# amplab/snap

Measured on AMD Instinct MI355X. Metric: aligned reads/sec (whole node), 150 bp single-end vs synthetic 3100 Mb genome (GRCh38 unavailable), seed=20, maxDist=8, higher is better.
Workload: dtype u8 bases / int32 DP / f64 match probability

## Files before the change

snap_amd/csrc/align_single.h:

```cpp
#pragma once
#include "dev_common.h"
#include "probe.h"
#include "lv.h"
#include "ag_win.h"
#include "se_help.h"
#include "adjust.h"
#include <stddef.h>
#include "../../include/snapgpu.h"

#define BUCKET 48
#define SENT_MIN 0xFC00u
#define WIN_PAD 128

struct AlignCfg {
    uint32_t max_hits, max_k, num_seeds, min_weight, extra_depth, use_ag;
    int32_t  match_reward, sub_penalty, gap_open, gap_extend, five_bonus, three_bonus;
    uint32_t alt_aware, emit_alt;
    int32_t  max_gap_alt;
    double   seed_coverage;
    uint32_t num_weight_lists;
    uint32_t RL;
    uint32_t kmax;
    uint32_t pool_size;
    uint32_t ht_size;
    uint64_t scratch_stride;
    uint32_t lds_per_wave;
    uint32_t ag_numvec_max;
    uint32_t ag_buffers;
    uint32_t ag_lds;
    uint32_t se_items_cap; uint64_t se_off;
    uint32_t stop_on_first_hit, explore_popular_seeds;
};

struct __attribute__((aligned(16))) Elem {
    uint64_t used;
    uint64_t scored;
    int64_t  base;
    int64_t  best_loc;
    double   match_prob;
    uint32_t weight;
    uint32_t lps;
    uint32_t best_score;
    int32_t  ag_score;
    int32_t  clip_before, clip_after, seed_offset;
    uint16_t wnext, wprev, hnext;
    uint8_t  dir;
    uint8_t  flags;
    uint32_t pad0;
    uint16_t cand_seed_offset[BUCKET];
};
static_assert(sizeof(Elem) == 176, "Elem layout");

struct ScoreSet {
    int32_t  best_score;
    int64_t  best_loc, best_orig_loc;
    int32_t  dir;
    int32_t  used_ag, clip_before, clip_after, ag_score, seed_offset;
    double   best_match_prob;
    double   p_all, p_best;
    __device__ __forceinline__ void init() {
        best_score = SNAPGPU_UnusedScoreValue; best_loc = SNAPGPU_InvalidGenomeLocation32;
        best_orig_loc = SNAPGPU_InvalidGenomeLocation32; dir = 0; used_ag = 0; clip_before = 0;
        clip_after = 0; ag_score = -1; seed_offset = 0; best_match_prob = 0.0; p_all = 0.0; p_best = 0.0;
    }
};

struct WaveCounters {
    uint64_t lookups, slots, hits, overflow_lists, lv, ag, lv_ref_bytes;
    uint64_t cyc_lookup, cyc_hits, cyc_lv, cyc_ag, cyc_total;
};
static __device__ __forceinline__ uint64_t wave_clock() { return __builtin_amdgcn_s_memtime(); }

static __device__ __forceinline__ int compute_mapq(const DevTables *tab, double p_all, double p_best, int popular_skipped) {
    if (p_all < p_best) p_all = p_best;
    double correctness = p_best / p_all;
    int base_mapq;
    if (correctness >= 1) {
        base_mapq = 70;
    } else {
        double x = 1 - correctness;
        int lo = 0, hi = 70;
        while (lo < hi) {
            int mid = (lo + hi + 1) >> 1;
            if (x <= tab->mapq_threshold[mid]) lo = mid; else hi = mid - 1;
        }
        base_mapq = lo;
    }
    int pen = popular_skipped - 10; if (pen < 0) pen = 0;
    base_mapq -= pen / 2;
    if (base_mapq < 0) base_mapq = 0;
    return (int)first_u32((uint32_t)base_mapq);
}

struct WaveShared {
    ScoreSet all, non_alt;
    ScoreSet ag_all, ag_non_alt;
    snapgpu_single_result primary, first_alt;
    WaveCounters cnt;
};

struct SecCfg {
    int32_t  om;
    int32_t  mpc;
    int64_t  omax;
    uint32_t cap;
    uint32_t adjust;
    uint64_t adj_off;
};

struct AlignerDirState { uint32_t dirkey; };
struct AlignerNoDirState {};
template <bool REGDIR> struct AlignerDirBase { using type = AlignerNoDirState; };
template <> struct AlignerDirBase<true> { using type = AlignerDirState; };

template <int AGC, bool SEC = false, bool EXACT = false, bool TIMED = false, bool PLANES = false, bool REGDIR = false>
struct Aligner : AlignerDirBase<REGDIR>::type {
    const DevIndex ix;
    GP<const DevTables> tab;
    const AlignCfg cfg;
    LP<uint8_t>  rd[2];
    LP<uint8_t>  ql[2];
    LP<uint8_t>  gw;
    LP<uint32_t> seed_used;
    LP<uint16_t> wl_next, wl_prev;
    LP<uint16_t> lv_tri;
    LP<int16_t>  ag_rows;
    LP<unsigned long long> rp;
    LP<unsigned long long> tp;
    int tp_org;
    LP<unsigned long long> lvp;
    uint32_t rd_plain;
    GP<uint16_t> heads;
    GP<Elem>     pool;
    GP<uint8_t>  ag_scratch;
    uint8_t  *ag_persist0, *ag_persist1;
    uint32_t ag_hw0, ag_hw1;
    uint32_t ag_epoch, ag_tag;
    struct LaneId { __device__ __forceinline__ operator int() const { return lane_id(); } };
    LaneId lane;
    int read_len;
    uint32_t n_used;
    uint32_t highest_used_weight_list;
    uint32_t wrap_count;
    uint32_t lps_unseen[2];
    uint32_t cur_round_lps[2];
    uint32_t n_seeds_applied[2];
    uint32_t popular_seeds_skipped;
    uint32_t ag_stale;
    uint32_t ag_replay;
    uint32_t ag_obj_used0, ag_obj_used1;
    uint32_t max_k;
    uint32_t ag_calls_unit;
    SEHelpSlot *se_slots; uint32_t se_n_slots; SESpec *se_spec; uint32_t se_spec_cap;
    uint32_t *se_ctl;
    uint32_t se_eager;
    uint32_t *se_items, *se_first;
    unsigned long long *se_diag;
    int se_slot; uint32_t se_n, se_tried, cur_read; SESpec *se_mine;
    GP<snapgpu_single_result> agc;
    uint32_t agc_cap, n_agc, agc_overflow;
    SecCfg sec_cfg;
    snapgpu_single_result *sec;
    uint32_t *sec_key, *sec_ord;
    uint32_t n_sec, n_sec_raw, sec_overflow;
    uint8_t *adj_scratch;
    LDS_AS WaveShared *ws_;
    __device__ __forceinline__ ScoreSet &all() const { return *(ScoreSet *)&ws_->all; }
    __device__ __forceinline__ ScoreSet &non_alt() const { return *(ScoreSet *)&ws_->non_alt; }
    __device__ __forceinline__ snapgpu_single_result &primary() const { return *(snapgpu_single_result *)&ws_->primary; }
    __device__ __forceinline__ snapgpu_single_result &first_alt() const { return *(snapgpu_single_result *)&ws_->first_alt; }
    __device__ __forceinline__ WaveCounters &cnt() const { return *(WaveCounters *)&ws_->cnt; }

    __device__ __forceinline__ Aligner(const DevIndex &ix_, const DevTables *tab_, const AlignCfg &cfg_, WaveShared *ws)
        : ix(ix_), tab(tab_), cfg(cfg_), tp_org(0), rd_plain(0), ag_hw0(0), ag_hw1(0), ag_epoch(0), ag_tag(0), read_len(0), popular_seeds_skipped(0),
          ag_stale(0), ag_replay(0), ag_obj_used0(0), ag_obj_used1(0), max_k(cfg_.max_k), ag_calls_unit(0),
          agc(nullptr), agc_cap(0), n_agc(0), agc_overflow(0), n_sec(0), n_sec_raw(0), sec_overflow(0),
          ws_((LDS_AS WaveShared *)ws) {}

    static __device__ __forceinline__ uint64_t clk() { if constexpr (TIMED) return wave_clock(); else return 0; }

    __device__ __forceinline__ void note_ag_call(int obj, uint32_t stale_steps) {
        ag_stale += stale_steps;
        const uint32_t used = obj == 0 ? ag_obj_used0 : ag_obj_used1;
        if (EXACT || used) ag_replay += stale_steps;
        if (obj == 0) ag_obj_used0 = 1; else ag_obj_used1 = 1;
    }

    __device__ __forceinline__ void new_read_images() {
        if constexpr (EXACT) {
            if (++ag_epoch == 16u) {
                if (ag_hw0) wave_zero16(ag_persist0, ((size_t)ag_hw0 + 15) & ~(size_t)15);
                if (ag_hw1) wave_zero16(ag_persist1, ((size_t)ag_hw1 + 15) & ~(size_t)15);
                ag_hw0 = ag_hw1 = 0; ag_epoch = 1u;
                WAVE_SYNC();
            }
            ag_tag = bt_tag_bits(ag_epoch);
        }
    }

    __device__ __forceinline__ void note_ag_extent(int obj, bool banded, int plen, int w, int tlen) {
        if constexpr (EXACT) {
            int nv, sl, ns;
            ag_dims(banded, plen, w > 126 ? 126 : (w < 0 ? 0 : w), &nv, &sl, &ns);
            uint32_t ext = (w >= 0 && tlen > 0) ? (uint32_t)tlen * (uint32_t)(ns * sl) : 0u;
            const uint32_t image = (uint32_t)ag_scratch_bytes(cfg.RL);
            if (ext > image) ext = image;
            if (obj == 0) ag_hw0 = ext > ag_hw0 ? ext : ag_hw0; else ag_hw1 = ext > ag_hw1 ? ext : ag_hw1;
        }
    }

    __device__ __forceinline__ bool is_alt(int64_t loc) const { return (uint64_t)loc >= ix.first_alt_location && loc >= 0; }

    __device__ __forceinline__ int score_limit(bool for_alt) const {
        int64_t inner;
        if (for_alt) {
            int64_t g = cfg.max_gap_alt < non_alt().best_score ? cfg.max_gap_alt : non_alt().best_score;
            int64_t b = (int64_t)non_alt().best_score - g;
            inner = all().best_score < b ? all().best_score : b;
        } else {
            int64_t a = (int64_t)all().best_score + cfg.max_gap_alt;
            inner = a < non_alt().best_score ? a : non_alt().best_score;
        }
        int64_t m = (int64_t)max_k < inner ? (int64_t)max_k : inner;
        int64_t v = (int64_t)cfg.extra_depth + m;
        return (int)(v < 126 ? v : 126);
    }

    __device__ __forceinline__ bool substring_ok(int64_t loc, int64_t len) const {
        if (!substring_in_range(loc, len)) return false;
        return substring_ok_known(loc, len, first_u32(((const G(uint8_t) *)ix.genome)[loc]) == 'n');
    }
    __device__ __forceinline__ bool substring_in_range(int64_t loc, int64_t len) const {
        int64_t nb = (int64_t)ix.n_bases;
        if (loc > nb || loc + len > nb + 1000) return false;
        if (loc < -(int64_t)ix.genome_pad + WIN_PAD) return false;
        return true;
    }
    __device__ __forceinline__ bool substring_ok_known(int64_t loc, int64_t len, bool first_is_pad) const {
        int64_t nb = (int64_t)ix.n_bases;
        if (len <= (int64_t)ix.chromosome_padding && !first_is_pad) return true;
        if (len == 0) return true;
        int lo = 0, hi = (int)ix.n_contigs - 1, found = -1;
        while (lo <= hi) {
            int mid = (lo + hi) >> 1;
            uint64_t b = first_u64(((const G(uint64_t) *)ix.contig_begin)[mid]);
            if ((int64_t)b <= loc) { found = mid; lo = mid + 1; } else { hi = mid - 1; }
        }
        if (found < 0) return false;
        int64_t cbeg = (int64_t)first_u64(((const G(uint64_t) *)ix.contig_begin)[found]);
        int64_t cend = found == (int)ix.n_contigs - 1 ? nb : (int64_t)first_u64(((const G(uint64_t) *)ix.contig_begin)[found + 1]);
        if (cend <= loc + len) return false;
        (void)cbeg;
        return true;
    }

    __device__ __forceinline__ uint16_t sent(uint32_t w) const { return (uint16_t)(0xFFFFu - w); }
    __device__ __forceinline__ uint16_t get_next(uint16_t i) const {
        return i >= SENT_MIN ? wl_next[0xFFFFu - i] : (uint16_t)first_u32(pool[i].wnext);
    }
    __device__ __forceinline__ uint16_t get_prev(uint16_t i) const {
        return i >= SENT_MIN ? wl_prev[0xFFFFu - i] : (uint16_t)first_u32(pool[i].wprev);
    }
    __device__ __forceinline__ void set_next(uint16_t i, uint16_t v) {
        if (lane == 0) { if (i >= SENT_MIN) wl_next[0xFFFFu - i] = v; else pool[i].wnext = v; }
        WAVE_SYNC();
    }
    __device__ __forceinline__ void set_prev(uint16_t i, uint16_t v) {
        if (lane == 0) { if (i >= SENT_MIN) wl_prev[0xFFFFu - i] = v; else pool[i].wprev = v; }
        WAVE_SYNC();
    }
    __device__ __forceinline__ void list_unlink(uint16_t e) {
        uint16_t n = get_next(e), p = get_prev(e);
        set_prev(n, p);
        set_next(p, n);
    }
    __device__ __forceinline__ void list_push_tail(uint32_t w, uint16_t e) {
        uint16_t s = sent(w);
        uint16_t tail = get_prev(s);
        if (lane == 0) { pool[e].wnext = s; pool[e].wprev = tail; }
        WAVE_SYNC();
        set_prev(s, e);
        set_next(tail, e);
    }

    __device__ __forceinline__ uint32_t head_slot(int64_t base, int dir) const {
        uint64_t k = ((uint64_t)base / BUCKET) * 2 + (uint64_t)dir;
        k *= 0x9E3779B97F4A7C15ull;
        return (uint32_t)(k >> 40) & (cfg.ht_size - 1);
    }
    static __device__ __forceinline__ uint32_t dir_key(int64_t base, int dir) { return (uint32_t)(((uint64_t)base / BUCKET) * 2 + (uint64_t)dir); }
#ifndef SNAPGPU_DIR_CAP
#define SNAPGPU_DIR_CAP 64
#endif
    static constexpr uint32_t DIR_CAP = SNAPGPU_DIR_CAP;
    __device__ __forceinline__ uint16_t find_element(int64_t loc, int dir) const {
        int64_t low = (int64_t)((uint64_t)loc % BUCKET);
        int64_t base = loc - low;
        if constexpr (REGDIR) {
            if (n_used <= DIR_CAP) {
                const unsigned long long m = BALLOT(this->dirkey == dir_key(base, dir));
                return m ? (uint16_t)__builtin_ctzll(m) : (uint16_t)0xFFFF;
            }
        }
        uint16_t h = (uint16_t)first_u32(heads[head_slot(base, dir)]);
        while (h != 0) {
            const uint32_t *ew = (const uint32_t *)&pool[h - 1];
            const uint32_t v = ew[lane == 0 ? 4 : (lane == 1 ? 5 : 18)];
            const int64_t b = (int64_t)(((uint64_t)(uint32_t)__builtin_amdgcn_readlane((int)v, 1) << 32) | (uint32_t)__builtin_amdgcn_readlane((int)v, 0));
            const uint32_t w18 = (uint32_t)__builtin_amdgcn_readlane((int)v, 2);
            if (b == base && (int)((w18 >> 16) & 0xffu) == dir) return (uint16_t)(h - 1);
            h = (uint16_t)(w18 & 0xffffu);
        }
        return 0xFFFF;
    }

    __device__ __forceinline__ void clear_candidates() {
        n_used = 0;
        highest_used_weight_list = 0;
        if constexpr (REGDIR) this->dirkey = 0xFFFFFFFFu;
        for (uint32_t i = lane; i < cfg.num_weight_lists; i += WAVE) {
            wl_next[i] = sent(i); wl_prev[i] = sent(i);
        }
        WAVE_SYNC();
    }

    __device__ __forceinline__ void release_candidates() {
        if (REGDIR && n_used <= DIR_CAP) return;
        for (uint32_t i = lane; i < n_used; i += WAVE) {
            heads[head_slot(pool[i].base, pool[i].dir)] = 0;
        }
        WAVE_SYNC();
    }

    __device__ __forceinline__ void increment_weight(uint16_t ei) {
        Elem *e = &pool[ei];
        uint32_t flags = first_u32(e->flags);
        if (flags & 1) return;
        uint32_t w = first_u32(e->weight);
        if (w >= cfg.num_weight_lists - 1) return;
        list_unlink(ei);
        w++;
        if (lane == 0) e->weight = w;
        WAVE_SYNC();
        if (w > highest_used_weight_list) highest_used_weight_list = w;
        list_push_tail(w, ei);
    }

    __device__ __forceinline__ void allocate_new_candidate(int64_t loc, int dir, uint32_t lps, int seed_offset) {
        int64_t low = (int64_t)((uint64_t)loc % BUCKET);
        int64_t base = loc - low;
        uint16_t ei = (uint16_t)n_used;
        n_used++;
        Elem *e = &pool[ei];
        uint32_t hs = head_slot(base, dir);
        uint16_t old_head = 0;
        bool hashed = true;
        if constexpr (REGDIR) {
            if (ei < DIR_CAP) { this->dirkey = lane == (int)ei ? dir_key(base, dir) : this->dirkey; hashed = false; }
            else if (ei == DIR_CAP) {
                for (uint32_t j = 0; j < DIR_CAP; j++) {
                    uint64_t k = (uint64_t)(uint32_t)__builtin_amdgcn_readlane((int)this->dirkey, (int)j) * 0x9E3779B97F4A7C15ull;
                    const uint32_t hj = (uint32_t)(k >> 40) & (cfg.ht_size - 1);
                    const uint16_t oh = (uint16_t)first_u32(heads[hj]);
                    if (lane == 0) { pool[j].hnext = oh; heads[hj] = (uint16_t)(j + 1); }
                    WAVE_SYNC();
                }
            }
        }
        if (hashed) old_head = (uint16_t)first_u32(heads[hs]);
        if (lane == 0) {
            e->used = 1ull << low;
            e->scored = 0;
            e->lps = lps;
            e->dir = (uint8_t)dir;
            e->weight = 1;
            e->base = base;
            e->best_score = SNAPGPU_UnusedScoreValue;
            e->flags = 0;
            e->match_prob = 0;
            e->clip_before = 0; e->clip_after = 0; e->ag_score = 0;
            e->best_loc = 0; e->seed_offset = 0;
            e->cand_seed_offset[low] = (uint16_t)seed_offset;
            e->hnext = old_head;
            if (hashed) heads[hs] = (uint16_t)(ei + 1);
        }
        WAVE_SYNC();
        list_push_tail(1, ei);
        if (highest_used_weight_list < 1) highest_used_weight_list = 1;
    }

    __device__ __forceinline__ void apply_hit(uint32_t hit, uint32_t offset, int dir) {
        int64_t loc = (int64_t)(uint32_t)(hit - offset);
        uint16_t ei = find_element(loc, dir);
        if (ei != 0xFFFF) {
            Elem *e = &pool[ei];
            uint32_t low = (uint32_t)((uint64_t)loc % BUCKET);
            uint64_t bit = 1ull << low;
            uint64_t used = first_u64(e->used);
            uint32_t flags = first_u32(e->flags);
            uint32_t new_flags = (flags & ~1u) | (((flags & 1u) && (used & bit)) ? 1u : 0u);
            if (lane == 0) {
                e->flags = (uint8_t)new_flags;
                e->used = used | bit;
                e->cand_seed_offset[low] = (uint16_t)offset;
            }
            WAVE_SYNC();
            increment_weight(ei);
        } else {
            bool cand_alt = cfg.alt_aware && is_alt(loc);
            const uint32_t lps_d = dir ? lps_unseen[1] : lps_unseen[0];
            if ((int64_t)lps_d <= (int64_t)score_limit(cand_alt)) {
                allocate_new_candidate(loc, dir, lps_d, (int)offset);
            }
        }
    }

    __device__ __forceinline__ void record_candidate(int dir, int64_t loc, int64_t orig_loc, int score, int used_ag, int clip_before,
                                                     int clip_after, int ag_score, double mp, int seed_offset) {
        if (agc == nullptr) return;
        if (n_agc >= agc_cap) { agc_overflow = 1; return; }
        snapgpu_single_result *r = &agc[n_agc];
        if (lane == 0) {
            r->direction = dir; r->location = loc; r->orig_location = orig_loc; r->mapq = 0; r->score = score;
            r->status = SNAPGPU_MultipleHits; r->clipping_for_read_adjustment = 0; r->used_affine_gap_scoring = used_ag;
            r->bases_clipped_before = clip_before; r->bases_clipped_after = clip_after; r->ag_score = ag_score;
            r->match_probability = mp; r->seed_offset = seed_offset; r->reserved = (uint32_t)score;
        }
        WAVE_SYNC();
        n_agc++;
    }

    __device__ __forceinline__ void record_secondary(int dir, int64_t loc, int64_t orig_loc, int score, int used_ag, int clip_before,
                                                     int clip_after, int ag_score, double mp, int seed_offset) {
        if (n_sec >= sec_cfg.cap) { sec_overflow = 1; return; }
        snapgpu_single_result *r = &sec[n_sec];
        if (lane == 0) {
            r->status = SNAPGPU_MultipleHits; r->direction = dir; r->location = loc; r->orig_location = orig_loc; r->score = score;
            r->score_prior_to_clipping = 0; r->mapq = 0; r->clipping_for_read_adjustment = 0; r->used_affine_gap_scoring = used_ag;
            r->bases_clipped_before = clip_before; r->bases_clipped_after = clip_after; r->ag_score = ag_score; r->supplementary = 0;
            r->seed_offset = seed_offset; r->match_probability = mp; r->probability_all_candidates = 0.0; r->popular_seeds_skipped = 0;
            r->reserved = 0;
        }
        WAVE_SYNC();
        n_sec++;
    }

    template <bool HAM>
    __device__ __forceinline__ bool update_best(ScoreSet &ss, int64_t loc, int64_t orig_loc, uint32_t score,
                                                int ag_score, double mp, const Elem *e, int e_dir,
                                                int e_used_ag, int e_clip_before, int e_clip_after, int e_seed_offset,
                                                double e_match_prob) {
        bool seen_new;
        if (cfg.use_ag) {
            seen_new = (ag_score > ss.ag_score) || (ss.ag_score == ag_score && mp > ss.p_best);
        } else {
            seen_new = (score < (uint32_t)ss.best_score) || (score == (uint32_t)ss.best_score && mp > ss.p_best);
        }
        if constexpr (SEC) {
            const uint32_t best = (uint32_t)ss.best_score;
            if (seen_new) {
                if (best >= score && (int)(best - score) <= sec_cfg.om) {
                    record_secondary(ss.dir, ss.best_loc, ss.best_orig_loc, ss.best_score, ss.used_ag, ss.clip_before, ss.clip_after,
                                     ss.ag_score, ss.best_match_prob, ss.seed_offset);
                }
            } else if ((int)(best - score) <= sec_cfg.om && score != (uint32_t)SNAPGPU_ScoreAboveLimit && best >= score) {
                record_secondary(e_dir, loc, orig_loc, (int)score, e_used_ag, e_clip_before, e_clip_after, ag_score, e_match_prob, e_seed_offset);
            }
        }
        if constexpr (HAM) {
            const uint32_t best = (uint32_t)ss.best_score;
            if (seen_new) {
                if (best >= score && (int)(best - score) <= (int)cfg.extra_depth) {
                    record_candidate(ss.dir, ss.best_loc, ss.best_orig_loc, ss.best_score, ss.used_ag, ss.clip_before, ss.clip_after,
                                     ss.ag_score, ss.best_match_prob, ss.seed_offset);
                    if (agc_overflow) return false;
                }
            } else if ((int)(best - score) <= (int)cfg.extra_depth && score != (uint32_t)SNAPGPU_ScoreAboveLimit && best >= score) {
                record_candidate(e_dir, loc, orig_loc, (int)score, e_used_ag, e_clip_before, e_clip_after, ag_score, e_match_prob, e_seed_offset);
            }
        }
        if (seen_new) {
            ss.best_score = (int32_t)score;
            ss.ag_score = ag_score;
            ss.p_best = mp;
            ss.best_loc = loc;
            ss.best_orig_loc = orig_loc;
            ss.dir = e_dir;
            ss.used_ag = e_used_ag;
            ss.clip_before = e_clip_before;
            ss.clip_after = e_clip_after;
            ss.seed_offset = e_seed_offset;
            ss.best_match_prob = e_match_prob;
        }
        (void)e;
        return seen_new;
    }

    __device__ __forceinline__ void fill_result(const ScoreSet &ss, snapgpu_single_result &r) const {
        r.ag_score = ss.ag_score;
        r.bases_clipped_after = ss.clip_after;
        r.bases_clipped_before = ss.clip_before;
        r.clipping_for_read_adjustment = 0;
        r.direction = ss.dir;
        r.location = ss.best_loc;
        r.orig_location = ss.best_orig_loc;
        r.mapq = compute_mapq(tab, ss.p_all, ss.p_best, (int)popular_seeds_skipped);
        r.score = ss.best_score;
        r.used_affine_gap_scoring = ss.used_ag;
        r.seed_offset = ss.seed_offset;
        r.match_probability = ss.best_match_prob;
        r.popular_seeds_skipped = popular_seeds_skipped;
        r.status = r.mapq >= 10 ? SNAPGPU_SingleHit : SNAPGPU_MultipleHits;
        r.probability_all_candidates = ss.p_all;
    }

    __device__ __forceinline__ int gapless_score(int st, const uint8_t *T, const uint8_t *P, const uint8_t *Q, int plen, int score_init,
                                                 int limit, int *n_edits, int *pattern_offset, double *mp, int *n_gapless) const {
        *mp = 1.0;
        if (limit < 0) { *n_edits = -1; *n_gapless = -1; return -1; }
        int sc = score_init, best = score_init, best_i = 0;
        for (int i = 0; i < plen; i++) {
            sc += (P[i * st] == T[i * st]) ? cfg.match_reward : -cfg.sub_penalty;
            if (sc > best) { best = sc; best_i = i; }
        }
        best = (int)first_u32((uint32_t)best); best_i = (int)first_u32((uint32_t)best_i);
        if (best > score_init) {
            int ne = 0, nm = 0;
            double p = 1.0;
            for (int i = 0; i <= best_i; i++) {
                if (P[i * st] != T[i * st]) { ne++; p *= tab->phred[Q[i * st]]; } else nm++;
            }
            p *= tab->perfect[nm];
            const int clipped = plen - (best_i + 1);
            *pattern_offset = clipped;
            ne = (int)first_u32((uint32_t)ne);
            *n_gapless = ne <= limit ? ne : -1;
            *n_edits = ne + clipped;
            p *= tab->indel[clipped];
            *mp = first_f64(p);
            return best;
        }
        *n_edits = -1; *n_gapless = -1;
        return -1;
    }

    template <class T> static __device__ __forceinline__ T *lds_ptr(T *p) {
#if defined(__HIP_DEVICE_COMPILE__) && !defined(SNAPGPU_WAVE_EMU)
        __builtin_assume(__builtin_amdgcn_is_shared((const void *)p));
#endif
        return p;
    }
    __device__ __forceinline__ void stage_window(int64_t loc) {
        uint8_t *const gw = this->gw;
        const int total = read_len + 2 * WIN_PAD;
        const G(uint8_t) *src = (const G(uint8_t) *)ix.genome + (loc - WIN_PAD);
        uintptr_t a = (uintptr_t)src;
        int head = (int)((4 - (a & 3)) & 3);
        if (head > total) head = total;
        if (lane < head) gw[lane] = src[lane];
        int words = (total - head) >> 2;
        const G(uint32_t) *s32 = (const G(uint32_t) *)(src + head);
        for (int w = lane; w < words; w += WAVE) {
            uint32_t v = s32[w];
            uint8_t *d = gw + head + 4 * w;
            d[0] = (uint8_t)v; d[1] = (uint8_t)(v >> 8); d[2] = (uint8_t)(v >> 16); d[3] = (uint8_t)(v >> 24);
        }
        int done = head + 4 * words;
        if (done + lane < total) gw[done + lane] = src[done + lane];
        WAVE_SYNC();
    }

    __device__ __forceinline__ void stage_planes(int64_t loc) {
        const int64_t bit0 = loc - WIN_PAD + (int64_t)ix.genome_pad;
        const int64_t blk0 = bit0 >> 6;
        tp_org = (int)(bit0 & 63) + WIN_PAD;
        const int nb = (int)text_plane_blocks(cfg.RL, WIN_PAD);
        for (int l = lane; l < 3 * nb; l += WAVE) {
            const int b = l / 3, pl = l - 3 * b;
            tp[pl * nb + b] = ix.planes[(blk0 + b) * 3 + pl];
        }
        WAVE_SYNC();
    }
    __device__ __forceinline__ void build_read_planes(int len) {
        const int rpw = (int)read_plane_words(cfg.RL);
        uint32_t not_plain = 0;
        for (int dir = 0; dir < 2; dir++) {
            for (int w = 0; w < rpw; w++) {
                const int i = w * 64 + lane;
                const uint8_t c = i < len ? rd[dir][i] : (uint8_t)0;
                const uint32_t v = base_value(c);
                const bool in = i < len, non = v > 3u, nn = c == 'N' || c == 'n';
                const unsigned long long p0 = BALLOT(in && (non ? c == 'n' : (v & 1u))), p1 = BALLOT(in && !non && (v & 2u));
                const unsigned long long pn = BALLOT(in && nn), po = BALLOT(in && non && !nn);
                if (lane == 0) {
                    unsigned long long *base = rp + (size_t)dir * 4 * rpw;
                    base[w] = p0; base[rpw + w] = p1; base[2 * rpw + w] = pn; base[3 * rpw + w] = po;
                }
                if (pn | po) not_plain |= 1u << dir;
            }
        }
        rd_plain = ~not_plain & 3u;
        WAVE_SYNC();
    }

    struct CandEval { uint32_t sc; double mp; int64_t loc; int used_ag, clip_before, clip_after, ag_score; uint32_t lv_sum_high;
                      int lv1, lv2; };
    template <bool HAM>
    __device__ __forceinline__ CandEval eval_candidate(int64_t loc, int e_dir, uint32_t e_lps, int cand_seed_offset, int limit_e, uint32_t best_all) {
        uint32_t lv_sum_high = 0;
        int lv1 = -1, lv2 = -2;
        uint32_t sc = (uint32_t)SNAPGPU_ScoreAboveLimit;
        double mp = 0.0;
        const int64_t glen = (int64_t)read_len + SNAPGPU_MAX_K;
        int used_ag = 0, clip_before = 0, clip_after = 0, ag_score = -1;

        const bool lv_planes = PLANES && !HAM && ix.planes != nullptr && limit_e <= 31;
        bool sub_ok = false;
        if (substring_in_range(loc, glen)) {
            bool first_is_pad;
            stage_window(loc);
            if (lv_planes) stage_planes(loc);
            first_is_pad = first_u32(gw[WIN_PAD]) == 'n';
            sub_ok = substring_ok_known(loc, glen, first_is_pad);
        }
        if (sub_ok) {
            const uint8_t *data = gw + WIN_PAD;
            const int seed_len = (int)ix.seed_len;
            const int seed_offset = cand_seed_offset;
            const int tail_start = seed_offset + seed_len;
            int ag1 = seed_len, ag2 = 0;
            int score1 = 0, score2 = 0;
            double mp1 = 1.0, mp2 = 1.0;
            int loc_offset = 0;
            const int text_len = read_len + SNAPGPU_MAX_K - tail_start;

            const uint8_t *rdd = e_dir ? rd[1] : rd[0], *qld = e_dir ? ql[1] : ql[0];
            int g1 = 0, g2 = 0;
            if constexpr (HAM) {
                if (tail_start != read_len) {
                    int po;
                    ag1 = gapless_score(+1, data + tail_start, rdd + tail_start, qld + tail_start, read_len - tail_start, read_len,
                                        limit_e, &score1, &po, &mp1, &g1);
                    ag1 += seed_len - read_len;
                }
                if (g1 != -1 && seed_offset != 0) {
                    int po = 0;
                    ag2 = gapless_score(-1, data + seed_offset - 1, rdd + seed_offset - 1, qld + seed_offset - 1, seed_offset, read_len,
                                        limit_e - g1, &score2, &po, &mp2, &g2);
                    ag2 -= read_len;
                    loc_offset = g2 != -1 ? po : 0;
                }
            }
            const uint64_t t_lv0 = clk();
            for (int half = 0; half < 2 && !HAM; half++) {
                if (half == 1 && score1 == -1) break;
                const int st = half == 0 ? 1 : -1;
                const int org = half == 0 ? tail_start : seed_offset - 1;
                const int plen = half == 0 ? read_len - tail_start : seed_offset;
                const int tlen = half == 0 ? text_len : seed_offset + SNAPGPU_MAX_K;
                const int lim = half == 0 ? limit_e : limit_e - score1;
                const LdsSeq P = lds_seq(ByteSeq{rdd + org, st}), Q = lds_seq(ByteSeq{qld + org, st}), T = lds_seq(ByteSeq{data + org, st});
                LvPlanes lp;
                if (lv_planes) {
                    const int rpw = (int)read_plane_words(cfg.RL);
                    const LDS_AS unsigned long long *rb = (const LDS_AS unsigned long long *)(unsigned long long *)rp + (e_dir ? 4 * rpw : 0);
                    const LDS_AS unsigned long long *tb = (const LDS_AS unsigned long long *)(unsigned long long *)tp;
                    lp.p0 = rb; lp.p1 = rb + rpw; lp.pn = rb + 2 * rpw; lp.po = rb + 3 * rpw;
                    const int tpb = (int)text_plane_blocks(cfg.RL, WIN_PAD);
                    lp.t0 = tb; lp.t1 = tb + tpb; lp.tn = tb + 2 * tpb;
                    lp.p_org = org; lp.t_org = tp_org + org; lp.st = st; lp.p_words = rpw; lp.t_words = tpb;
                    lp.work = (LDS_AS unsigned long long *)(unsigned long long *)lvp; lp.plain = ((rd_plain >> e_dir) & 1u) != 0;
                }
                LVResult r = lv_compute(P, Q, plen, T, tlen, lim, lv_tri, cfg.kmax, tab, cfg.RL, lv_planes ? &lp : nullptr);
                r.score = (int)first_u32((uint32_t)r.score); r.net_indel = (int)first_u32((uint32_t)r.net_indel);
                r.match_probability = first_f64(r.match_probability);
                if (half == 0) {
                    score1 = r.score; mp1 = r.match_probability;
                    ag1 = (seed_len + read_len - tail_start - score1) * cfg.match_reward - score1 * cfg.sub_penalty;
                    cnt().lv_ref_bytes += (uint64_t)plen + (uint64_t)(2 * (limit_e < 0 ? 0 : limit_e));
                } else {
                    score2 = r.score; mp2 = r.match_probability; loc_offset = r.net_indel;
                    ag2 = (seed_offset - score2) * cfg.match_reward - score2 * cfg.sub_penalty;
                    cnt().lv_ref_bytes += (uint64_t)plen;
                }
            }
            if (!HAM) cnt().lv++;
            cnt().cyc_lv += clk() - t_lv0;
            lv1 = score1; lv2 = score1 == -1 ? -2 : score2;

            if (!HAM && score1 != -1 && score2 != -1) {
                int max_k_same = cfg.gap_open / (cfg.sub_penalty - cfg.gap_extend);
                lv_sum_high = score1 + score2 > max_k_same ? 1u : 0u;
                if (cfg.use_ag && (lv_sum_high && e_lps <= best_all)) {
                    if (lv_planes) stage_window(loc);
                    score1 = 0; score2 = 0; ag1 = seed_len; ag2 = 0;
                    used_ag = 1;
                    cnt().ag++;
                    if (++ag_calls_unit == WAVE_PRIO_HEAVY_AFTER) wave_set_priority(1);
                    const uint64_t t_ag0 = clk();
                    AGParams agp{cfg.match_reward, cfg.sub_penalty, cfg.gap_open, cfg.gap_extend, cfg.five_bonus, cfg.three_bonus};
                    for (int half = 0; half < 2; half++) {
                        if (half == 0 && tail_start == read_len) continue;
                        if (half == 1 && (score1 == -1 || seed_offset == 0)) break;
                        const int st = half == 0 ? 1 : -1;
                        const int org = half == 0 ? tail_start : seed_offset - 1;
                        const int plen = half == 0 ? read_len - tail_start : seed_offset;
                        const int lim = half == 0 ? limit_e : limit_e - score1;
                        const int tlen = half == 0 ? text_len : seed_offset + lim;
                        const bool banded = plen >= 3 * (2 * lim + 1);
                        const LdsSeq P = lds_seq(ByteSeq{rdd + org, st}), Q = lds_seq(ByteSeq{qld + org, st}), T = lds_seq(ByteSeq{data + org, st});
                        note_ag_extent(half, banded, plen, lim, tlen);
                        AGResult a = ag_dispatch<AGC, EXACT>(banded, st, agp, P, Q, plen, T, tlen, lim, read_len, e_dir != 0,
                                                      false, ag_rows, EXACT ? (half == 0 ? ag_persist0 : ag_persist1) : (uint8_t *)ag_scratch, cfg.RL, tab, EXACT ? ag_tag : 0u);
                        a.ag_score = (int)first_u32((uint32_t)a.ag_score); a.n_edits = (int)first_u32((uint32_t)a.n_edits);
                        a.pattern_offset = (int)first_u32((uint32_t)a.pattern_offset); a.text_offset = (int)first_u32((uint32_t)a.text_offset);
                        a.stale_reads = (int)first_u32((uint32_t)a.stale_reads); a.match_probability = first_f64(a.match_probability);
                        note_ag_call(half, (uint32_t)a.stale_reads);
                        if (half == 0) {
                            ag1 = a.ag_score + (seed_len - read_len); clip_after = a.pattern_offset;
                            score1 = a.n_edits; mp1 = a.match_probability;
                        } else {
                            ag2 = a.ag_score - read_len; clip_before = a.pattern_offset;
                            score2 = a.n_edits; mp2 = a.match_probability; loc_offset = a.text_offset;
                        }
                    }
                    cnt().cyc_ag += clk() - t_ag0;
                }
            }

            bool found = HAM ? (g1 != -1 && g2 != -1) : (score1 != -1 && score2 != -1);
            if (found && loc_offset != 0 && !substring_ok(loc + loc_offset, glen)) found = false;
            if (found) {
                sc = (uint32_t)(score1 + score2);
                mp = mp1 * mp2 * tab->seed_prob;
                loc += loc_offset;
                ag_score = ag1 + ag2;
            } else {
                sc = (uint32_t)SNAPGPU_ScoreAboveLimit;
                ag_score = SNAPGPU_ScoreAboveLimit;
                mp = 0.0;
            }
        } else {
            mp = 0.0;
        }

        CandEval ce; ce.sc = sc; ce.mp = mp; ce.loc = loc; ce.used_ag = used_ag; ce.clip_before = clip_before; ce.clip_after = clip_after;
        ce.ag_score = ag_score; ce.lv_sum_high = lv_sum_high; ce.lv1 = lv1; ce.lv2 = lv2;
        return ce;
    }

    __device__ __forceinline__ bool se_wanted() const { return se_eager || XW::ld(se_ctl[1]) != 0u; }

    __device__ __forceinline__ void se_publish(uint32_t wl) {
        int s = -1;
        if (lane == 0) {
            const uint32_t start = (cur_read * 7u) % se_n_slots;
            for (uint32_t k = 0; k < se_n_slots; k++) {
                const uint32_t i = start + k < se_n_slots ? start + k : start + k - se_n_slots;
                if (XW::ld_lane(se_slots[i].state) != 0u) continue;
                if (atomicCAS(&se_slots[i].state, 0u, 3u) == 0u) { s = (int)i; break; }
            }
        }
        s = (int)first_u32((uint32_t)s);
        if (s < 0) { se_tried = 0x80000000u | 32u; return; }
        se_tried = 1;
        for (uint32_t i = (uint32_t)lane; i < n_used; i += WAVE) se_first[i] = 0xffffffffu;
        WAVE_SYNC();
        uint32_t n = 0;
        for (uint32_t w = wl; w >= 1 && n + BUCKET <= cfg.se_items_cap; w--) {
            uint16_t ei = get_next(sent(w));
            while (ei < SENT_MIN && n + BUCKET <= cfg.se_items_cap) {
                const uint32_t *ep = (const uint32_t *)&pool[ei];
                const uint32_t v = lane < 4 ? ep[lane] : (lane == 4 ? ep[17] : 0u);
                const uint64_t used = ((uint64_t)(uint32_t)__builtin_amdgcn_readlane((int)v, 1) << 32) | (uint32_t)__builtin_amdgcn_readlane((int)v, 0);
                const uint64_t scored = ((uint64_t)(uint32_t)__builtin_amdgcn_readlane((int)v, 3) << 32) | (uint32_t)__builtin_amdgcn_readlane((int)v, 2);
                const uint16_t nxt = (uint16_t)((uint32_t)__builtin_amdgcn_readlane((int)v, 4) & 0xffffu);
                const uint64_t m = used & ~scored;
                if (lane == 0) se_first[ei] = n;
                if (lane < BUCKET && ((m >> lane) & 1ull)) se_items[n + (uint32_t)__popcll(m & ((1ull << lane) - 1ull))] = ((uint32_t)ei << 6) | (uint32_t)lane;
                n += (uint32_t)__popcll(m);
                ei = nxt;
            }
        }
        WAVE_SYNC();
        if (n < SE_HELP_MIN_ITEMS || n > se_spec_cap) { if (lane == 0) atomicExch(&se_slots[s].state, 0u); return; }
        SEHelpSlot *slot = &se_slots[s];
        SESpec *spec = se_spec + (size_t)s * se_spec_cap;
        for (uint32_t t = (uint32_t)lane; t < n; t += WAVE) spec[t].state = 0u;
        WAVE_SYNC();
        if (lane == 0) {
            const uint32_t w0 = atomicExch(&slot->next, SE_HELP_LOOKAHEAD), w1 = atomicExch(&slot->helpers, 0u);
            if ((w0 ^ w1) == 0xFFFFFFF5u) atomicExch(&slot->helpers, 0u);
            XW::st(slot->read, cur_read); XW::st(slot->n, n); XW::st(slot->owner_pos, 0u);
            XW::st(slot->lim_alt, (int32_t)score_limit(true)); XW::st(slot->lim_non_alt, (int32_t)score_limit(false));
            XW::st(slot->best_all, (uint32_t)all().best_score);
            XW::st(*(uint64_t *)&slot->items, (uint64_t)(uintptr_t)se_items); XW::st(*(uint64_t *)&slot->pool, (uint64_t)(uintptr_t)(Elem *)pool);
            XW::st(*(uint64_t *)&slot->spec, (uint64_t)(uintptr_t)spec);
            XW::fence_release();
            atomicExch(&slot->state, 1u);
            atomicAdd(&se_ctl[2], 1u);
            if (se_diag) atomicAdd(&se_diag[1], 1ull << 32);
        }
        WAVE_SYNC();
        se_slot = s; se_n = n; se_mine = spec;
    }

    __device__ __forceinline__ bool se_take(uint16_t ei, int idx, uint64_t listed0, int limit_e, uint32_t e_lps, int64_t loc0, int cand_seed_offset, CandEval &ce) {
        const uint32_t t0 = first_u32(se_first[ei]);
        if (t0 == 0xffffffffu) return false;
        const uint32_t t = t0 + (uint32_t)__popcll(listed0 & ((1ull << idx) - 1ull));
        if (t >= se_n) return false;
        SEHelpSlot *slot = &se_slots[se_slot];
        SESpec *sp = &se_mine[t];
        if (lane == 0) XW::st(slot->owner_pos, t + 1u);
        const uint64_t t_w0 = wave_clock();
        for (;;) {
            uint32_t st = 0;
            if (lane == 0) st = atomicCAS(&sp->state, 0u, 1u);
            st = first_u32(st);
            if (st == 0u) return false;
            if (st == 2u) break;
            XW::nap();
            if (wave_clock() - t_w0 > 1200000000ull) {
                if (lane == 0 && se_diag) atomicAdd(&se_diag[0], 1ull);
                se_abandon();
                return false;
            }
        }
        const int lim = XW::ld(sp->limit);
        const uint32_t high = XW::ld(sp->lv_sum_high), best_then = XW::ld(sp->best_all);
        const uint32_t n_lv = XW::ld(sp->n_lv);
        uint32_t n_ag = XW::ld(sp->n_ag), stale = XW::ld(sp->stale);
        uint64_t bytes = XW::ld(sp->lv_ref_bytes);
        if (lim == limit_e) {
            if (high && ((e_lps <= best_then) != (e_lps <= (uint32_t)all().best_score))) { if (lane == 0 && se_diag) atomicAdd(&se_diag[-1], 1ull << 16); return false; }
            ce.sc = XW::ld(sp->sc); ce.mp = XW::ld(sp->mp); ce.loc = XW::ld(sp->loc); ce.used_ag = XW::ld(sp->used_ag);
            ce.clip_before = XW::ld(sp->clip_before); ce.clip_after = XW::ld(sp->clip_after); ce.ag_score = XW::ld(sp->ag_score);
        } else {
            if (lim < limit_e || n_lv == 0u) { if (lane == 0 && se_diag) atomicAdd(&se_diag[-1], 1ull); return false; }
            const int lv1 = XW::ld(sp->lv1), lv2 = XW::ld(sp->lv2);
            const int plen0 = read_len - (cand_seed_offset + (int)ix.seed_len), plen1 = cand_seed_offset;
            const bool half1_runs = lv1 >= 0 && lv1 <= limit_e;
            bytes = (uint64_t)plen0 + (uint64_t)(2 * (limit_e < 0 ? 0 : limit_e)) + (half1_runs ? (uint64_t)plen1 : 0ull);
            if (half1_runs && lv2 >= 0 && lv1 + lv2 <= limit_e) {
                if (n_ag != 0u || (high && e_lps <= (uint32_t)all().best_score)) {
                    if (lane == 0 && se_diag) atomicAdd(&se_diag[-1], 1ull << 16);
                    return false;
                }
                ce.sc = XW::ld(sp->sc); ce.mp = XW::ld(sp->mp); ce.loc = XW::ld(sp->loc); ce.used_ag = 0;
                ce.clip_before = 0; ce.clip_after = 0; ce.ag_score = XW::ld(sp->ag_score);
            } else {
                ce.sc = (uint32_t)SNAPGPU_ScoreAboveLimit; ce.mp = 0.0; ce.loc = loc0; ce.used_ag = 0; ce.clip_before = 0; ce.clip_after = 0;
                ce.ag_score = SNAPGPU_ScoreAboveLimit;
                n_ag = 0; stale = 0;
            }
        }
        ce.lv_sum_high = high; ce.lv1 = 0; ce.lv2 = 0;
        cnt().lv += n_lv; cnt().ag += n_ag; cnt().lv_ref_bytes += bytes;
        ag_stale += stale; ag_replay += stale;
        if (n_ag) { ag_obj_used0 = 1; ag_obj_used1 = 1; ag_calls_unit += n_ag; }
        if (lane == 0 && se_diag) atomicAdd(&se_diag[1], 1ull);
        return true;
    }

    __device__ __forceinline__ void se_abandon() {
        if (lane == 0) { atomicExch(&se_slots[se_slot].state, 4u); atomicSub(&se_ctl[2], 1u); }
        se_slot = -1;
    }

    __device__ __forceinline__ void se_close() {
        SEHelpSlot *slot = &se_slots[se_slot];
        uint32_t was = 0;
        if (lane == 0) { was = atomicExch(&slot->state, 2u); atomicSub(&se_ctl[2], 1u); }
        was = first_u32(was);
        bool gave_up = was != 1u;
        const uint64_t t0 = wave_clock();
        while (!gave_up) {
            if (XW::aload(&slot->helpers) == 0u) break;
            XW::nap();
            if (wave_clock() - t0 > 4800000000ull) { if (lane == 0 && se_diag) atomicAdd(&se_diag[0], 1ull << 16); gave_up = true; }
        }
        if (lane == 0) atomicExch(&slot->state, gave_up ? 4u : 0u);
        se_slot = -1;
    }

    __device__ __forceinline__ void se_help_slot(SEHelpSlot *slot) {
        const uint32_t n = XW::ld(slot->n);
        const int lim_alt = XW::ld(slot->lim_alt), lim_non_alt = XW::ld(slot->lim_non_alt);
        const uint32_t best = XW::ld(slot->best_all);
        const uint32_t *items = (const uint32_t *)(uintptr_t)XW::ld(*(const uint64_t *)&slot->items);
        const Elem *opool = (const Elem *)(uintptr_t)XW::ld(*(const uint64_t *)&slot->pool);
        SESpec *spec = (SESpec *)(uintptr_t)XW::ld(*(const uint64_t *)&slot->spec);
        for (uint32_t it = 0; it <= n; it++) {
            if (XW::aload(&slot->state) != 1u) break;
            uint32_t c0 = 0;
            if (lane == 0) c0 = atomicAdd(&slot->next, SE_HELP_CHUNK);
            c0 = first_u32(c0);
            if (c0 >= n) break;
            const uint32_t c1 = c0 + SE_HELP_CHUNK < n ? c0 + SE_HELP_CHUNK : n;
            for (uint32_t t = c0; t < c1; t++) {
                if (t < XW::ld(slot->owner_pos)) continue;
                uint32_t st = 1;
                if (lane == 0) st = atomicCAS(&spec[t].state, 0u, 1u);
                if (first_u32(st) != 0u) continue;
                if (XW::aload(&slot->state) != 1u) break;
                const uint32_t item = first_u32(items[t]);
                const uint32_t ei = item >> 6; const int idx = (int)(item & 63u);
                if (ei >= cfg.pool_size) continue;
                const uint32_t *ep = (const uint32_t *)&opool[ei];
                const uint32_t ew = lane < (int)(sizeof(Elem) / 4) ? ep[lane] : 0u;
                auto EW = [&](int i) -> uint32_t { return (uint32_t)__builtin_amdgcn_readlane((int)ew, i); };
                const int64_t e_base = (int64_t)(((uint64_t)EW(5) << 32) | EW(4));
                const int e_dir = (int)((EW(18) >> 16) & 0xffu);
                const uint32_t e_lps = EW(11);
                const int cso = (int)((EW(20 + (idx >> 1)) >> (16 * (idx & 1))) & 0xffffu);
                const int limit_e = (cfg.alt_aware && is_alt(e_base)) ? lim_alt : lim_non_alt;
                CandEval ce; ce.sc = 0; ce.mp = 0; ce.loc = 0; ce.used_ag = 0; ce.clip_before = 0; ce.clip_after = 0; ce.ag_score = 0; ce.lv_sum_high = 0;
                ce.lv1 = -1; ce.lv2 = -2;
                uint32_t d_lv = 0, d_ag = 0, stale = 0; uint64_t d_bytes = 0;
                int rec_limit = (int)0x80000000;
                if ((int64_t)e_lps <= (int64_t)limit_e && e_base >= 0 && (uint64_t)(e_base + idx) < (uint64_t)ix.n_bases && idx < 48 && cso >= 0 && cso <= read_len) {
                    const uint64_t lv0 = cnt().lv, ag0 = cnt().ag, b0 = cnt().lv_ref_bytes;
                    ag_stale = 0; ag_replay = 0; ag_obj_used0 = 1; ag_obj_used1 = 1;
                    ce = eval_candidate<false>(e_base + idx, e_dir, e_lps, cso, limit_e, best);
                    d_lv = (uint32_t)(cnt().lv - lv0); d_ag = (uint32_t)(cnt().ag - ag0); d_bytes = cnt().lv_ref_bytes - b0; stale = ag_stale;
                    cnt().lv = lv0; cnt().ag = ag0; cnt().lv_ref_bytes = b0;
                    WAVE_SYNC();
                    rec_limit = limit_e;
                }
                if (lane == 0) {
                    SESpec *sp = &spec[t];
                    XW::st(sp->limit, (int32_t)rec_limit); XW::st(sp->best_all, best); XW::st(sp->lv_sum_high, ce.lv_sum_high);
                    XW::st(sp->sc, ce.sc); XW::st(sp->ag_score, (int32_t)ce.ag_score); XW::st(sp->used_ag, (int32_t)ce.used_ag);
                    XW::st(sp->clip_before, (int32_t)ce.clip_before); XW::st(sp->clip_after, (int32_t)ce.clip_after);
                    XW::st(sp->n_lv, d_lv); XW::st(sp->n_ag, d_ag); XW::st(sp->stale, stale);
                    XW::st(sp->loc, ce.loc); XW::st(sp->mp, ce.mp); XW::st(sp->lv_ref_bytes, d_bytes);
                    XW::st(sp->lv1, (int32_t)ce.lv1); XW::st(sp->lv2, (int32_t)ce.lv2);
                    XW::stores_done();
                    atomicExch(&sp->state, 2u);
                    if (se_diag) atomicAdd(&se_diag[-1], 1ull << 32);
#if defined(SNAPGPU_WAVE_EMU)
                    if (getenv("SNAPGPU_DEBUG_SE_HELP")) fprintf(stderr, "HELPED read %u item %u limit %d sc %u n_ag %u\n", XW::ld(slot->read), t, rec_limit, ce.sc, d_ag);
#endif
                }
                WAVE_SYNC();
            }
        }
    }

    template <bool HAM>
    __device__ __forceinline__ bool score(bool force_result) {
        if (cur_round_lps[0] > lps_unseen[0]) lps_unseen[0] = cur_round_lps[0];
        if (cur_round_lps[1] > lps_unseen[1]) lps_unseen[1] = cur_round_lps[1];
        uint32_t wl = highest_used_weight_list;
        do {
            while (wl > 0 && get_next(sent(wl)) == sent(wl)) {
                wl--;
                highest_used_weight_list = wl;
            }
            int lim_t = score_limit(true), lim_f = score_limit(false);
            int lim_max = lim_t > lim_f ? lim_t : lim_f;
            uint32_t lps_min = lps_unseen[0] < lps_unseen[1] ? lps_unseen[0] : lps_unseen[1];
            if ((int64_t)lps_min > (int64_t)lim_max || force_result) {
                if (wl < cfg.min_weight) {
                    bool fin_all;
                    first_alt().status = SNAPGPU_NotFound;
                    if (!cfg.alt_aware || non_alt().best_score > all().best_score + cfg.max_gap_alt) {
                        fin_all = true;
                    } else {
                        fin_all = false;
                        if (cfg.emit_alt && all().best_score <= non_alt().best_score && all().best_loc != non_alt().best_loc) {
                            fill_result(all(), first_alt());
                        }
                    }
                    const int fin_best = fin_all ? all().best_score : non_alt().best_score;
                    primary().score = fin_best;
                    if ((uint32_t)fin_best <= max_k || (HAM && fin_best != SNAPGPU_UnusedScoreValue)) {
                        if (fin_all) fill_result(all(), primary()); else fill_result(non_alt(), primary());
                        primary().supplementary = 0;
                    } else {
                        primary().status = SNAPGPU_NotFound;
                        primary().mapq = 0;
                    }
                    return true;
                }
                force_result = true;
            } else if (wl == 0) {
                return false;
            }

            if constexpr (!EXACT && !HAM) {
                if (force_result && se_slots != nullptr && se_slot < 0) {
                    if (se_tried & 0x80000000u) { se_tried = (se_tried & 0x7fffffffu) > 1u ? se_tried - 1u : 0u; }
                    else if (!se_tried && se_wanted()) se_publish(wl);
                }
            }
            uint16_t ei = get_next(sent(wl));
            Elem *e = &pool[ei];
            const uint32_t ew = lane < (int)(sizeof(Elem) / 4) ? ((const uint32_t *)e)[lane] : 0u;
            auto EW = [&](int i) -> uint32_t { return (uint32_t)__builtin_amdgcn_readlane((int)ew, i); };
            static_assert(offsetof(Elem, wnext) == 68 && offsetof(Elem, base) == 16 && offsetof(Elem, match_prob) == 32 && offsetof(Elem, lps) == 44 &&
                          offsetof(Elem, best_score) == 48 && offsetof(Elem, hnext) == 72 && offsetof(Elem, dir) == 74 &&
                          offsetof(Elem, flags) == 75 && offsetof(Elem, cand_seed_offset) == 80, "Elem layout");
            int64_t e_base = (int64_t)(((uint64_t)EW(5) << 32) | EW(4));
            int e_dir = (int)((EW(18) >> 16) & 0xffu);
            uint32_t e_lps = EW(11);
            uint64_t e_scored = ((uint64_t)EW(3) << 32) | EW(2);
            uint32_t e_best_cur = EW(12);
            double e_mp_cur = __longlong_as_double((long long)(((uint64_t)EW(9) << 32) | EW(8)));
            uint32_t e_flags_cur = EW(18) >> 24;
            int limit_e = score_limit(cfg.alt_aware && is_alt(e_base));
            if ((int64_t)e_lps <= (int64_t)limit_e) {
                uint64_t mask = ((uint64_t)EW(1) << 32) | EW(0);
                const uint64_t listed0 = mask & ~e_scored;
                while (mask) {
                    int idx = __ffsll((long long)mask) - 1;
                    uint64_t bit = 1ull << idx;
                    mask &= ~bit;
                    uint64_t scored = e_scored;
                    if (scored & bit) continue;
                    bool any_nearby = scored != 0;
                    e_scored = scored | bit;
                    if (lane == 0) e->scored = e_scored;
                    WAVE_SYNC();

                    int64_t loc = e_base + idx;
                    const int64_t orig_loc = loc, elem_loc = loc;
                    bool loc_non_alt = !cfg.alt_aware || !is_alt(loc);

                    int cand_seed_offset = (int)((EW(20 + (idx >> 1)) >> (16 * (idx & 1))) & 0xffffu);
                    CandEval ce;
                    bool have = false;
                    if constexpr (!EXACT && !HAM) { if (se_slot >= 0) have = se_take(ei, idx, listed0, limit_e, e_lps, loc, cand_seed_offset, ce); }
                    if (!have) ce = eval_candidate<HAM>(loc, e_dir, e_lps, cand_seed_offset, limit_e, (uint32_t)all().best_score);
                    const uint32_t sc = ce.sc; const double mp = ce.mp; loc = ce.loc;
                    const int used_ag = ce.used_ag, clip_before = ce.clip_before, clip_after = ce.clip_after, ag_score = ce.ag_score;

                    uint32_t e_best = e_best_cur;
                    double e_mp = e_mp_cur;
                    if (any_nearby) {
                        if (HAM && mp <= e_mp) continue;
                        if (e_best < sc || (e_best == sc && mp <= e_mp)) continue;
                    }
                    const uint32_t e_flags = e_flags_cur;
                    e_flags_cur = (e_flags & 1u) | (used_ag ? 2u : 0u);
                    if (lane == 0) {
                        e->best_loc = loc;
                        e->flags = (uint8_t)e_flags_cur;
                        e->clip_before = clip_before;
                        e->clip_after = clip_after;
                        e->ag_score = ag_score;
                        e->seed_offset = cand_seed_offset;
                    }
                    WAVE_SYNC();

                    uint16_t ni = 0xFFFF;
                    if ((uint32_t)SNAPGPU_ScoreAboveLimit != sc && sc < 2) {
                        int64_t half = (int64_t)(((uint64_t)elem_loc % BUCKET) / (BUCKET / 2));
                        int64_t nearby_loc = elem_loc + (2 * half - 1) * (BUCKET / 2);
                        ni = find_element(nearby_loc, e_dir);
                    }
                    if (ni != 0xFFFF) {
                        Elem *ne = &pool[ni];
                        uint64_t n_scored = first_u64(ne->scored);
                        if (n_scored != 0) {
                            int64_t n_best_loc = (int64_t)first_u64((uint64_t)ne->best_loc);
                            int64_t dist = loc > n_best_loc ? loc - n_best_loc : n_best_loc - loc;
                            if (dist <= BUCKET) {
                                uint32_t n_best = first_u32(ne->best_score);
                                double n_mp = first_f64(ne->match_prob);
                                if (HAM && n_mp >= mp) continue;
                                if (n_best < sc || (n_best == sc && n_mp >= mp)) continue;
                                double v = all().p_all - n_mp; all().p_all = v > 0.0 ? v : 0.0;
                                if (loc_non_alt) { double u = non_alt().p_all - n_mp; non_alt().p_all = u > 0.0 ? u : 0.0; }
                                any_nearby = true;
                                if (lane == 0) ne->match_prob = 0;
                                WAVE_SYNC();
                            }
                        }
                    }

                    {
                        double v = all().p_all - e_mp; v = v > 0.0 ? v : 0.0; all().p_all = v + mp;
                        if (loc_non_alt) { double u = non_alt().p_all - e_mp; u = u > 0.0 ? u : 0.0; non_alt().p_all = u + mp; }
                    }
                    e_mp_cur = mp; e_best_cur = sc;
                    if (lane == 0) { e->match_prob = mp; e->best_score = sc; }
                    WAVE_SYNC();

                    update_best<HAM>(all(), loc, orig_loc, sc, ag_score, mp, e, e_dir, used_ag, clip_before, clip_after, cand_seed_offset, mp);
                    if (loc_non_alt) {
                        update_best<HAM>(non_alt(), loc, orig_loc, sc, ag_score, mp, e, e_dir, used_ag, clip_before, clip_after, cand_seed_offset, mp);
                    }
                    if (HAM && agc != nullptr && n_agc >= agc_cap) { agc_overflow = 1; return true; }

                    if (cfg.stop_on_first_hit && ((uint32_t)all().best_score <= max_k || (HAM && all().best_score != SNAPGPU_UnusedScoreValue))) {
                        if (cfg.alt_aware) fill_result(non_alt(), primary()); else fill_result(all(), primary());
                        primary().status = SNAPGPU_MultipleHits; primary().mapq = 0;
                        first_alt().status = SNAPGPU_NotFound;
                        WAVE_SYNC();
                        return true;
                    }
                    double p_chk = cfg.alt_aware ? non_alt().p_all : all().p_all;
                    if (!SEC && p_chk >= 4.9) {
                        if (cfg.alt_aware) fill_result(non_alt(), primary()); else fill_result(all(), primary());
                        first_alt().status = SNAPGPU_NotFound;
                        return true;
                    }
                }
            }

            {
                if (lane == 0) e->flags = (uint8_t)(e_flags_cur | 1u);
                WAVE_SYNC();
            }
            list_unlink(ei);
            if (lane == 0) { e->wnext = ei; e->wprev = ei; }
            WAVE_SYNC();
        } while (force_result);
        return false;
    }

    __device__ __forceinline__ void seed_set_used(uint32_t i) {
        if (lane == 0) seed_used[i >> 5] |= (1u << (i & 31));
        WAVE_SYNC();
    }
    __device__ __forceinline__ bool seed_is_used(uint32_t i) const { return (seed_used[i >> 5] >> (i & 31)) & 1u; }

    __device__ __forceinline__ void align_read(const uint8_t *g_bases, const uint8_t *g_quals, int len) {
        const uint64_t t_read0 = clk();
        ag_obj_used0 = ag_obj_used1 = 0;
        ag_calls_unit = 0;
        align_read_inner<false>(g_bases, g_quals, len);
        if (ag_calls_unit >= WAVE_PRIO_HEAVY_AFTER) wave_set_priority(0);
        cnt().cyc_total += clk() - t_read0;
    }
    __device__ __forceinline__ uint32_t load_read(const uint8_t *g_bases, const uint8_t *g_quals, int len) {
        uint32_t n_count = 0;
        for (int i0 = 0; i0 < len; i0 += WAVE) {
            int i = i0 + lane;
            uint8_t b = 0, q = 0;
            if (i < len) {
                b = g_bases[i]; q = g_quals[i];
                rd[0][i] = b; ql[0][i] = q;
                rd[1][len - 1 - i] = rc_base(b);
                ql[1][len - 1 - i] = q;
            }
            n_count += (uint32_t)__popcll(BALLOT(i < len && b == 'N'));
        }
        return n_count;
    }
    template <bool HAM>
    __device__ __forceinline__ void align_read_inner(const uint8_t *g_bases, const uint8_t *g_quals, int len) {
        read_len = len;
        if constexpr (SEC) { n_sec = 0; n_sec_raw = 0; sec_overflow = 0; }
        ag_stale = 0; ag_replay = 0; n_agc = 0; agc_overflow = 0;
        primary().status = SNAPGPU_NotFound; primary().direction = 0;
        primary().location = SNAPGPU_InvalidGenomeLocation32; primary().orig_location = 0;
        primary().score = SNAPGPU_UnusedScoreValue; primary().score_prior_to_clipping = 0; primary().mapq = 0;
        primary().clipping_for_read_adjustment = 0; primary().used_affine_gap_scoring = 0;
        primary().bases_clipped_before = 0; primary().bases_clipped_after = 0; primary().ag_score = 0;
        primary().supplementary = 0; primary().seed_offset = 0; primary().match_probability = 0.0;
        primary().probability_all_candidates = 0.0; primary().popular_seeds_skipped = 0; primary().reserved = 0;
        first_alt() = primary();
        first_alt().location = 0; first_alt().score = 0;

        const int seed_len = (int)ix.seed_len;
        if (len < seed_len || len > (int)cfg.RL) return;

        const uint32_t n_count = load_read(g_bases, g_quals, len);
        for (uint32_t i = lane; i < (cfg.RL + 31) / 32; i += WAVE) seed_used[i] = 0;
        WAVE_SYNC();
        if (n_count > max_k) return;
        if (PLANES && !HAM && ix.planes != nullptr) build_read_planes(len);

        if (n_count > 0) {
            int min_seed = 0;
            for (int i = 0; i < len; i++) {
                if (base_value(rd[0][i]) > 3) {
                    int limit = i + seed_len - 1 < len - 1 ? i + seed_len - 1 : len - 1;
                    int j0 = i - seed_len + 1; if (j0 < min_seed) j0 = min_seed;
                    for (int j = j0; j <= limit; j++) seed_set_used((uint32_t)j);
                    min_seed = limit + 1;
                    if (min_seed >= len) break;
                }
            }
        }

        uint32_t max_seeds_to_use = cfg.num_seeds != 0 ? cfg.num_seeds
                                  : (uint32_t)(int)(2 * cfg.seed_coverage * len / seed_len);
        clear_candidates();
        const uint32_t n_possible_seeds = (uint32_t)(len - seed_len + 1);
        uint32_t next_seed = 0;
        wrap_count = 0;
        lps_unseen[0] = lps_unseen[1] = 0;
        cur_round_lps[0] = cur_round_lps[1] = 0;
        all().init();
        non_alt().init();
        if (!cfg.alt_aware) non_alt().best_score = SNAPGPU_TooBigScoreValue;
        n_seeds_applied[0] = n_seeds_applied[1] = 0;
        popular_seeds_skipped = 0;
        se_tried = 0;

        while (true) {
            bool force = false, applied_either = false;
            if (n_seeds_applied[0] + n_seeds_applied[1] >= max_seeds_to_use) force = true;
            else if (next_seed >= n_possible_seeds && wrap_count + 1 >= (uint32_t)seed_len) { wrap_count++; force = true; }
            if (!force) do {
            if (next_seed >= n_possible_seeds) {
                wrap_count++;
                next_seed = tab->wrapped_seed[wrap_count];
                cur_round_lps[0] = cur_round_lps[1] = 0;
            }
            while (next_seed < n_possible_seeds && seed_is_used(next_seed)) next_seed++;
            if (next_seed >= n_possible_seeds) continue;
            seed_set_used(next_seed);

            SeedBits seed = pack_seed(rd[0] + next_seed, (uint32_t)seed_len);
            if (!seed.valid) continue;

            HitList hl[2];
            const uint64_t t_lk0 = clk();
            lookup_seed(ix, seed, hl);
            const uint64_t t_lk1 = clk();
            cnt().cyc_lookup += t_lk1 - t_lk0;
            cnt().lookups++;
            cnt().slots += hl[0].slots + hl[1].slots;

            for (int dir = 0; dir < 2; dir++) {
                const int64_t dir_n_hits = dir ? hl[1].n_hits : hl[0].n_hits;
                const uint32_t dir_singleton = dir ? hl[1].singleton : hl[0].singleton;
                const uint32_t *dir_hits = dir ? hl[1].hits : hl[0].hits;
                if (dir_n_hits > (int64_t)cfg.max_hits && !cfg.explore_popular_seeds) {
                    popular_seeds_skipped++;
                } else {
                    uint32_t offset = dir == 0 ? next_seed : (uint32_t)(len - seed_len) - next_seed;
                    int64_t limit = dir_n_hits < (int64_t)cfg.max_hits ? dir_n_hits : (int64_t)cfg.max_hits;
                    if (limit > 1) cnt().overflow_lists++;
                    cnt().hits += (uint64_t)limit;
                    for (int64_t c0 = 0; c0 < limit; c0 += WAVE) {
                        uint32_t mine = 0;
                        int64_t i = c0 + lane;
                        if (i < limit) mine = (dir_n_hits == 1) ? dir_singleton : dir_hits[i];
                        int n = (int)(limit - c0 < WAVE ? limit - c0 : WAVE);
                        for (int j = 0; j < n; j++) {
                            uint32_t h = first_u32((uint32_t)__shfl((int)mine, j));
                            apply_hit(h, offset, dir);
                        }
                    }
                    if (dir) { n_seeds_applied[1]++; cur_round_lps[1]++; } else { n_seeds_applied[0]++; cur_round_lps[0]++; }
                    applied_either = true;
                }
            }
            cnt().cyc_hits += clk() - t_lk1;
            next_seed += (uint32_t)seed_len;
            } while (0);
            if (force || applied_either) {
                if (score<HAM>(force) || force) break;
            }
        }
        if constexpr (!EXACT && !HAM) { if (se_slot >= 0) se_close(); }
        primary().score_prior_to_clipping = primary().score;
        primary().reserved = (ag_stale & 0x3fffffffu) | (ag_replay ? 0x40000000u : 0u);
        release_candidates();
        if constexpr (SEC) { n_sec_raw = n_sec; finalize_secondary(); }
    }

    __device__ __forceinline__ int contig_of(int64_t loc) const {
        int lo = 0, hi = (int)ix.n_contigs - 1;
        while (lo < hi) {
            int mid = (lo + hi + 1) >> 1;
            if ((int64_t)ix.contig_begin[mid] <= loc) lo = mid; else hi = mid - 1;
        }
        return lo;
    }
    __device__ __forceinline__ void sec_stable_sort(uint32_t n) {
        uint32_t *tmp = sec_key + sec_cfg.cap;
        for (uint32_t i0 = 0; i0 < n; i0 += WAVE) {
            const uint32_t i = i0 + (uint32_t)lane;
            if (i < n) {
                const uint32_t me = sec_ord[i], k = sec_key[me];
                uint32_t rank = 0;
                for (uint32_t j = 0; j < n; j++) {
                    const uint32_t kj = sec_key[sec_ord[j]];
                    rank += (kj < k || (kj == k && j < i)) ? 1u : 0u;
                }
                tmp[rank] = me;
            }
        }
        WAVE_SYNC(); __threadfence_block();
        for (uint32_t i = (uint32_t)lane; i < n; i += WAVE) sec_ord[i] = tmp[i];
        WAVE_SYNC(); __threadfence_block();
    }
    __device__ __forceinline__ void finalize_secondary() {
        int best = (int)first_u32((uint32_t)primary().score);
        if (sec_cfg.adjust) {
            const AdjustScratch asc = adjust_scratch_at(adj_scratch, cfg.RL);
            const AdjustIx aix = adjust_ix(ix);
            {
                const AdjustOut o = adjust_alignment(aix, rd[0], rd[1], read_len, (int)first_u32((uint32_t)primary().status), (int)first_u32((uint32_t)primary().direction),
                                                     (long long)first_u64((uint64_t)primary().location), best, SNAPGPU_InvalidGenomeLocation32, asc);
                primary().status = o.status; primary().location = o.location; primary().score = o.score; primary().clipping_for_read_adjustment = o.clipping;
                best = o.status != SNAPGPU_NotFound ? o.score : SNAPGPU_TooBigScoreValue;
            }
            WAVE_SYNC(); __threadfence_block();
            for (uint32_t i = 0; i < n_sec; i++) {
                snapgpu_single_result *r = &sec[i];
                const int sc0 = (int)first_u32((uint32_t)r->score);
                const AdjustOut o = adjust_alignment(aix, rd[0], rd[1], read_len, (int)first_u32((uint32_t)r->status), (int)first_u32((uint32_t)r->direction),
                                                     (long long)first_u64((uint64_t)r->location), sc0, SNAPGPU_InvalidGenomeLocation32, asc);
                if (lane == 0) {
                    r->score_prior_to_clipping = sc0;
                    r->status = o.status; r->location = o.location; r->score = o.score; r->clipping_for_read_adjustment = o.clipping;
                }
                if (o.status != SNAPGPU_NotFound && o.score < best) best = o.score;
            }
            WAVE_SYNC(); __threadfence_block();
        }
        uint32_t n = n_sec;
        if (n == 0) return;
        int worst = best + sec_cfg.om; if (worst > (int)max_k) worst = (int)max_k;
        for (uint32_t i = (uint32_t)lane; i < n; i += WAVE) { sec_ord[i] = i; sec_key[i] = (uint32_t)sec[i].score; }
        WAVE_SYNC(); __threadfence_block();
        if (lane == 0) {
            uint32_t i = 0;
            while (i < n) {
                if ((int)sec_key[sec_ord[i]] > worst) { sec_ord[i] = sec_ord[n - 1]; n--; }
                else i++;
            }
        }
        n = first_u32(n);
        WAVE_SYNC(); __threadfence_block();
        for (uint32_t i = (uint32_t)lane; i < n; i += WAVE) {
            snapgpu_single_result *r = &sec[sec_ord[i]];
            if (!sec_cfg.adjust) r->score_prior_to_clipping = r->score;
            r->supplementary = (cfg.alt_aware && is_alt(r->location)) ? 1 : 0;
        }
        WAVE_SYNC(); __threadfence_block();
        if (sec_cfg.mpc > 0 && primary().status != SNAPGPU_NotFound && n > 0) {
            const int primary_contig = contig_of(primary().location);
            for (uint32_t i = (uint32_t)lane; i < n; i += WAVE) {
                const uint32_t me = sec_ord[i];
                sec_key[me] = ((uint32_t)contig_of(sec[me].location) << 8) | (uint32_t)(sec[me].score & 0xff);
            }
            WAVE_SYNC(); __threadfence_block();
            uint32_t too_many = 0;
            for (uint32_t i0 = 0; i0 < n; i0 += WAVE) {
                const uint32_t i = i0 + (uint32_t)lane;
                bool over = false;
                if (i < n) {
                    const uint32_t c = sec_key[sec_ord[i]] >> 8;
                    int count = (int)c == primary_contig ? 1 : 0;
                    for (uint32_t j = 0; j < n; j++) count += (sec_key[sec_ord[j]] >> 8) == c ? 1 : 0;
                    over = count > sec_cfg.mpc;
                }
                too_many |= BALLOT(over) != 0 ? 1u : 0u;
            }
            if (too_many) {
                sec_stable_sort(n);
                if (lane == 0) {
                    int cur = -1, cur_count = 0; uint32_t dest = 0;
                    for (uint32_t src = 0; src < n; src++) {
                        const uint32_t me = sec_ord[src];
                        const int c = (int)(sec_key[me] >> 8);
                        if (c != cur) { cur = c; cur_count = c == primary_contig ? 1 : 0; }
                        cur_count++;
                        if (cur_count <= sec_cfg.mpc) sec_ord[dest++] = me;
                    }
                    n = dest;
                }
                n = first_u32(n);
                WAVE_SYNC(); __threadfence_block();
            }
        }
        if ((int64_t)n > sec_cfg.omax) {
            for (uint32_t i = (uint32_t)lane; i < n; i += WAVE) { const uint32_t me = sec_ord[i]; sec_key[me] = (uint32_t)sec[me].score; }
            WAVE_SYNC(); __threadfence_block();
            sec_stable_sort(n);
            n = (uint32_t)sec_cfg.omax;
        }
        n_sec = n;
    }

    __device__ __forceinline__ void score_location_ag(int dir, int64_t loc, int seed_offset, int limit, int *score, double *mp, int *offset,
                                                      int *clip_before, int *clip_after, int *ag_score) {
        const int64_t glen = (int64_t)read_len + SNAPGPU_MAX_K;
        *offset = 0;
        if (!substring_ok(loc, glen)) { *score = -1; *mp = 0; *ag_score = -1; return; }
        *clip_before = 0; *clip_after = 0;
        stage_window(loc);
        const uint8_t *data = gw + WIN_PAD;
        const int seed_len = (int)ix.seed_len;
        const int tail_start = seed_offset + seed_len;
        const uint8_t *rdd = dir ? rd[1] : rd[0], *qld = dir ? ql[1] : ql[0];
        int score1 = 0, score2 = 0, ag1 = seed_len, ag2 = 0;
        double mp1 = 1.0, mp2 = 1.0;
        AGParams agp{cfg.match_reward, cfg.sub_penalty, cfg.gap_open, cfg.gap_extend, cfg.five_bonus, cfg.three_bonus};
        for (int half = 0; half < 2; half++) {
            if (half == 0 && tail_start == read_len) continue;
            if (half == 1 && (score1 == -1 || seed_offset == 0)) break;
            const int st = half == 0 ? 1 : -1;
            const int org = half == 0 ? tail_start : seed_offset - 1;
            const int plen = half == 0 ? read_len - tail_start : seed_offset;
            const int lim = half == 0 ? limit : limit - score1;
            const int tlen = half == 0 ? (int)(glen - tail_start) : seed_offset + lim;
            const bool banded = plen >= 3 * (2 * lim + 1);
            const LdsSeq P = lds_seq(ByteSeq{rdd + org, st}), Q = lds_seq(ByteSeq{qld + org, st}), T = lds_seq(ByteSeq{data + org, st});
            note_ag_extent(half, banded, plen, lim, tlen);
            AGResult a = ag_dispatch<AGC, EXACT>(banded, st, agp, P, Q, plen, T, tlen, lim, read_len, dir != 0, half == 0, ag_rows,
                                                 EXACT ? (half == 0 ? ag_persist0 : ag_persist1) : (uint8_t *)ag_scratch, cfg.RL, tab, EXACT ? ag_tag : 0u);
            a.ag_score = (int)first_u32((uint32_t)a.ag_score); a.n_edits = (int)first_u32((uint32_t)a.n_edits);
            a.pattern_offset = (int)first_u32((uint32_t)a.pattern_offset); a.text_offset = (int)first_u32((uint32_t)a.text_offset);
            a.stale_reads = (int)first_u32((uint32_t)a.stale_reads); a.match_probability = first_f64(a.match_probability);
            note_ag_call(half, (uint32_t)a.stale_reads);
            if (half == 0) {
                ag1 = a.ag_score + (seed_len - read_len); *clip_after = a.pattern_offset; score1 = a.n_edits; mp1 = a.match_probability;
            } else {
                ag2 = a.ag_score - read_len; *clip_before = a.pattern_offset; score2 = a.n_edits; mp2 = a.match_probability; *offset = a.text_offset;
                if (score2 == -1) *offset = 0;
            }
        }
        if (score1 != -1 && score2 != -1) {
            *score = score1 + score2;
            *mp = mp1 * mp2 * tab->seed_prob_pow;
            *ag_score = ag1 + ag2;
        } else {
            *score = -1; *ag_score = -1; *mp = 0.0;
        }
    }

    __device__ __forceinline__ void set_from_result(ScoreSet &ss, const snapgpu_single_result &r) const {
        ss.best_score = r.score; ss.best_loc = r.location; ss.best_orig_loc = r.orig_location; ss.dir = r.direction;
        ss.used_ag = r.used_affine_gap_scoring; ss.clip_before = r.bases_clipped_before; ss.clip_after = r.bases_clipped_after;
        ss.ag_score = r.ag_score; ss.seed_offset = r.seed_offset; ss.best_match_prob = r.match_probability;
        ss.p_all = r.probability_all_candidates; ss.p_best = r.match_probability;
    }
    __device__ __forceinline__ bool set_update_from(ScoreSet &ss, int64_t loc, int64_t orig, int dir, int score, int used_ag, int cb, int ca,
                                                    int ag, int so, double mp) const {
        ss.p_all += mp;
        if (ag > ss.ag_score || (ag == ss.ag_score && mp > ss.best_match_prob)) {
            ss.best_score = score; ss.ag_score = ag; ss.best_match_prob = mp; ss.best_loc = loc; ss.best_orig_loc = orig; ss.dir = dir;
            ss.used_ag = used_ag; ss.clip_before = cb; ss.clip_after = ca; ss.seed_offset = so;
            return true;
        }
        return false;
    }
    static __device__ __forceinline__ void set_sub_all(ScoreSet &ss, double old) { double v = ss.p_all - old; ss.p_all = v > 0.0 ? v : 0.0; }

    __device__ __forceinline__ void align_affine_gap(ScoreSet &A, ScoreSet &N) {
        if (primary().status == SNAPGPU_NotFound) return;
        uint32_t n_count = 0;
        for (int i0 = 0; i0 < read_len; i0 += WAVE) {
            int i = i0 + lane;
            n_count += (uint32_t)__popcll(BALLOT(i < read_len && rd[0][i] == 'N'));
        }
        if (n_count > max_k) return;
        const int best_score = (int)first_u32((uint32_t)primary().score);
        int limit = SNAPGPU_MAX_K - 1, limit_alt = SNAPGPU_MAX_K - 1;
        int g_off = 0;
        bool skip = false;
        const double old_p = primary().match_probability;
        const double old_p_alt = first_alt().status != SNAPGPU_NotFound ? first_alt().match_probability : 0.0;
        const int max_k_same = cfg.gap_open / (cfg.sub_penalty - cfg.gap_extend);

        primary().used_affine_gap_scoring = 0;
        if (primary().score > max_k_same) {
            primary().used_affine_gap_scoring = 1;
            int sc, cb = primary().bases_clipped_before, ca = primary().bases_clipped_after, ag = primary().ag_score;
            double mp = primary().match_probability;
            score_location_ag(primary().direction, primary().orig_location, primary().seed_offset, limit, &sc, &mp, &g_off, &cb, &ca, &ag);
            primary().score = sc; primary().match_probability = mp; primary().bases_clipped_before = cb; primary().bases_clipped_after = ca; primary().ag_score = ag;
            if (sc != -1) primary().location = primary().orig_location + g_off; else primary().status = SNAPGPU_NotFound;
        } else {
            skip = true;
        }
        if (first_alt().status != SNAPGPU_NotFound && first_alt().score > max_k_same) {
            first_alt().used_affine_gap_scoring = 1;
            int sc, cb = first_alt().bases_clipped_before, ca = first_alt().bases_clipped_after, ag = first_alt().ag_score;
            double mp = first_alt().match_probability;
            score_location_ag(first_alt().direction, first_alt().orig_location, first_alt().seed_offset, limit_alt, &sc, &mp, &g_off, &cb, &ca, &ag);
            first_alt().score = sc; first_alt().match_probability = mp; first_alt().bases_clipped_before = cb; first_alt().bases_clipped_after = ca; first_alt().ag_score = ag;
            if (sc != -1) first_alt().location = first_alt().orig_location + g_off; else first_alt().status = SNAPGPU_NotFound;
        }
        if (primary().status == SNAPGPU_NotFound || primary().score > SNAPGPU_MAX_K - 1) {
            primary().location = SNAPGPU_InvalidGenomeLocation32; primary().mapq = 0; primary().score = -1; primary().status = SNAPGPU_NotFound;
            primary().clipping_for_read_adjustment = 0; primary().used_affine_gap_scoring = 0; primary().bases_clipped_before = 0;
            primary().bases_clipped_after = 0; primary().ag_score = -1; primary().seed_offset = 0; primary().match_probability = 0.0;
            first_alt().status = SNAPGPU_NotFound;
            return;
        }

        bool non_alt_aln = !cfg.alt_aware || !is_alt(primary().location);
        set_from_result(A, primary());
        bool alt_best = false;
        if (first_alt().status != SNAPGPU_NotFound) {
            alt_best = set_update_from(A, first_alt().location, first_alt().orig_location, first_alt().direction, first_alt().score,
                                       first_alt().used_affine_gap_scoring, first_alt().bases_clipped_before, first_alt().bases_clipped_after,
                                       first_alt().ag_score, first_alt().seed_offset, first_alt().match_probability);
        }
        if (non_alt_aln) set_from_result(N, primary()); else N.init();
        if (!skip) {
            const double new_p = primary().match_probability;
            if (alt_best) { set_sub_all(A, old_p_alt); A.p_best = first_alt().match_probability; A.p_all += first_alt().match_probability; }
            else          { set_sub_all(A, old_p); A.p_best = new_p; A.p_all += new_p; }
            if (non_alt_aln) { set_sub_all(N, old_p); N.p_best = new_p; N.p_all += new_p; }
        }

        if (n_agc > 0 && !skip) {
            limit = (int)((max_k < (uint32_t)best_score ? max_k : (uint32_t)best_score) + cfg.extra_depth);
            int last_score = -0x7fffffff, last_idx = -1;
            for (uint32_t done_n = 0; done_n < n_agc; done_n++) {
                int bi = -1, bs = 0x7fffffff;
                for (uint32_t j0 = 0; j0 < n_agc; j0 += WAVE) {
                    uint32_t j = j0 + (uint32_t)lane;
                    int sj = j < n_agc ? (int)agc[j].reserved : 0x7fffffff;
                    bool ok = j < n_agc && (sj > last_score || (sj == last_score && (int)j > last_idx));
                    int key = ok ? sj : 0x7fffffff;
                    for (int o = 32; o >= 1; o >>= 1) {
                        int ok2 = __shfl_xor(key, o), oj = __shfl_xor((int)j, o);
                        if (ok2 < key || (ok2 == key && oj < (int)j)) { key = ok2; j = (uint32_t)oj; }
                    }
                    key = (int)first_u32((uint32_t)key); j = first_u32(j);
                    if (key < bs) { bs = key; bi = (int)j; }
                }
                last_score = bs; last_idx = bi;
                snapgpu_single_result *c = &agc[bi];
                const int64_t c_loc = (int64_t)first_u64((uint64_t)c->location), c_orig = (int64_t)first_u64((uint64_t)c->orig_location);
                const int c_dir = (int)first_u32((uint32_t)c->direction), c_so = (int)first_u32((uint32_t)c->seed_offset);
                const bool c_non_alt = !cfg.alt_aware || !is_alt(c_loc);
                const double c_old_p = first_f64(c->match_probability);
                int sc, cb = (int)first_u32((uint32_t)c->bases_clipped_before), ca = (int)first_u32((uint32_t)c->bases_clipped_after);
                int ag = (int)first_u32((uint32_t)c->ag_score);
                double mp = c_old_p;
                score_location_ag(c_dir, c_orig, c_so, limit, &sc, &mp, &g_off, &cb, &ca, &ag);
                sc = (int)first_u32((uint32_t)sc);
                if (sc != -1 && sc <= SNAPGPU_MAX_K - 1) {
                    const int64_t new_loc = c_orig + g_off;
                    if (primary().location == new_loc) continue;
                    set_sub_all(A, c_old_p);
                    set_update_from(A, new_loc, c_orig, c_dir, sc, 1, cb, ca, ag, c_so, mp);
                    if (c_non_alt) { set_sub_all(N, c_old_p); set_update_from(N, new_loc, c_orig, c_dir, sc, 1, cb, ca, ag, c_so, mp); }
                    limit = score_limit(cfg.alt_aware && !c_non_alt);
                }
            }
        }

        const bool emit_all = !cfg.alt_aware || N.best_score > A.best_score + cfg.max_gap_alt;
        const uint32_t pop = primary().popular_seeds_skipped, pop_alt = first_alt().popular_seeds_skipped;
        const uint32_t saved_pop = popular_seeds_skipped;
        popular_seeds_skipped = pop;
        if (emit_all) fill_result(A, primary()); else fill_result(N, primary());
        if (cfg.alt_aware && !emit_all && A.best_loc != N.best_loc) {
            popular_seeds_skipped = pop_alt;
            fill_result(A, first_alt());
            first_alt().supplementary = 1;
        } else {
            first_alt().status = SNAPGPU_NotFound;
        }
        popular_seeds_skipped = saved_pop;
    }
};
```

snap_amd/csrc/kernel_common.h:

```cpp
#pragma once
#include "align_single.h"

struct AlignArgs {
    DevIndex ix;
    AlignCfg cfg;
    const DevTables *tab;
    uint8_t *scratch;
    const uint8_t *bases, *quals;
    const uint64_t *offsets;
    uint32_t n_reads;
    snapgpu_single_result *primary, *first_alt;
    uint32_t *work_counter;
    unsigned long long *counters;
    SecCfg sec_cfg;
    uint8_t *sec_scratch;
    uint64_t sec_stride_bytes;
    snapgpu_single_result *secondary;
    uint32_t sec_out_stride;
    uint32_t *n_secondary;
    uint32_t *flag_list, *flag_count;
    const uint32_t *remap, *n_remap;
    uint32_t is_replay;
    uint8_t *persist; uint64_t persist_stride;
    const uint32_t *order;
    unsigned long long *dbg; uint32_t dbg_slots;
    SEHelpSlot *se_slots; uint32_t se_n_slots; SESpec *se_spec; uint32_t se_spec_cap; uint32_t *se_ctl; uint32_t se_eager;
    uint32_t se_keep;
    const int32_t *front_clip, *data_len; const uint8_t *skip;
};

extern "C" {
void snapgpu_launch_single_sec_3(const AlignArgs *a, uint32_t blocks, size_t lds_bytes, hipStream_t s);
void snapgpu_launch_single_sec_4(const AlignArgs *a, uint32_t blocks, size_t lds_bytes, hipStream_t s);
void snapgpu_launch_single_sec_6(const AlignArgs *a, uint32_t blocks, size_t lds_bytes, hipStream_t s);
void snapgpu_launch_single_sec_0(const AlignArgs *a, uint32_t blocks, size_t lds_bytes, hipStream_t s);
void snapgpu_launch_single_exact_3(const AlignArgs *a, int sec, uint32_t blocks, size_t lds_bytes, hipStream_t s);
void snapgpu_launch_single_exact_0(const AlignArgs *a, int sec, uint32_t blocks, size_t lds_bytes, hipStream_t s);
void snapgpu_launch_single_exact_4(const AlignArgs *a, int sec, uint32_t blocks, size_t lds_bytes, hipStream_t s);
void snapgpu_launch_single_exact_6(const AlignArgs *a, int sec, uint32_t blocks, size_t lds_bytes, hipStream_t s);
void snapgpu_launch_single_exact_3_timed(const AlignArgs *a, uint32_t blocks, size_t lds_bytes, hipStream_t s);
void snapgpu_launch_single_3_timed(const AlignArgs *a, uint32_t blocks, size_t lds_bytes, hipStream_t s);
void snapgpu_launch_single_planes_3(const AlignArgs *a, uint32_t blocks, size_t lds_bytes, hipStream_t s);
void snapgpu_launch_single_planes_4(const AlignArgs *a, uint32_t blocks, size_t lds_bytes, hipStream_t s);
void snapgpu_launch_single_planes_6(const AlignArgs *a, uint32_t blocks, size_t lds_bytes, hipStream_t s);
void snapgpu_launch_single_planes_0(const AlignArgs *a, uint32_t blocks, size_t lds_bytes, hipStream_t s);
void snapgpu_launch_single_exact_planes_3(const AlignArgs *a, uint32_t blocks, size_t lds_bytes, hipStream_t s);
void snapgpu_launch_single_exact_planes_0(const AlignArgs *a, uint32_t blocks, size_t lds_bytes, hipStream_t s);
}

static __device__ __forceinline__ uint32_t align_up(uint32_t v, uint32_t a) { return (v + a - 1) & ~(a - 1); }

struct LdsLayout {
    uint32_t rd0, rd1, ql0, ql1, gw, seed_used, wl_next, wl_prev, lv, ag, shared, rp, tp, lvp, total;
};

static __host__ __device__ __forceinline__ LdsLayout lds_layout(uint32_t RL, uint32_t num_weight_lists, uint32_t kmax, uint32_t ag_lds) {
    LdsLayout L; uint32_t o = 0;
    L.rd0 = o; o += RL; L.rd1 = o; o += RL; L.ql0 = o; o += RL; L.ql1 = o; o += RL;
    L.gw = o; o += (RL + 2 * WIN_PAD + 15) & ~15u;
    L.seed_used = o; o += (((RL + 31) / 32) * 4 + 15) & ~15u;
    L.wl_next = o; o += (num_weight_lists * 2 + 15) & ~15u;
    L.wl_prev = o; o += (num_weight_lists * 2 + 15) & ~15u;
    L.lv = o; o += (lv_lds_bytes(kmax, RL) + 15) & ~15u;
    L.ag = o; o += (ag_lds + 15) & ~15u;
    L.shared = o; o += ((uint32_t)sizeof(WaveShared) + 15) & ~15u;
    L.rp = o; o += (2 * 4 * read_plane_words(RL) * 8 + 15) & ~15u;
    L.tp = o; o += (3 * text_plane_blocks(RL, WIN_PAD) * 8 + 15) & ~15u;
    L.lvp = o; o += (lv_plane_work_words(RL) * 8 + 15) & ~15u;
    L.total = o;
    return L;
}
```

snap_amd/csrc/paired_dev.h:

```cpp
#pragma once
#include "align_single.h"
#include "kernel_common.h"
#include "paired.h"
#include "paired_args.h"
#include <new>

template <int AGC, bool SEC = false, bool EXACT = false>
struct DevPL {
    typedef LP<DevPL> SelfPtr;
    LP<Aligner<AGC, SEC, EXACT>> al;
    uint8_t *ag_persist0, *ag_persist1;
    uint32_t ag_hw0, ag_hw1;
    uint32_t ag_epoch, ag_tag;
    static const bool HELP = !EXACT;
    static const bool ALWAYS_COUNT_STALE = EXACT;
    G(PEHelpSlot) *help; uint32_t n_help; G(PEHelpSpec) *help_spec; uint32_t help_spec_cap;
    const G(uint32_t) *help_idle; bool help_eager;
    uint32_t cur_pair; int my_slot;
    G(unsigned long long) *diag;
    template <class P> static __device__ __forceinline__ uint32_t aload(P *p) { return first_u32(lane_id() == 0 ? atomicCAS(p, 0xFFFFFFF5u, 0xFFFFFFF5u) : 0u); }
    template <class T, class W> static __device__ __forceinline__ void spec_st(T &x, W v_in) {
        typedef typename strip_as<T>::type V;
        const V v = (V)v_in;
#ifdef SNAPGPU_WAVE_EMU
// ... 199 lines not shown
#pragma unroll
                for (int j = 0; j < W; j++) c.win[j] = v[j];
                c.wbase = (int32_t)lo;
            }
            WAVE_SYNC();
        }
    }
    __device__ __forceinline__ void hs_stage(HSCursor &c, bool want, uint32_t lo, uint32_t hi) {
        const bool need = want && hi >= lo && !c.single && (c.wbase < 0 || lo < (uint32_t)c.wbase || hi >= (uint32_t)c.wbase + hs_w);
        if (hs_w == 16u) hs_stage_w<16>(c, need, lo); else hs_stage_w<8>(c, need, lo);
    }
    static __device__ __forceinline__ uint32_t hs_get(const HSCursor &c, uint32_t i) { return c.single ? c.singleton : c.win[i - (uint32_t)c.wbase]; }
    static __device__ __forceinline__ int wave_argmax32(bool ok, uint32_t v, uint32_t *best) {
        uint32_t m = ok ? v : 0u;
        for (int o = 16; o >= 1; o >>= 1) { const uint32_t t = (uint32_t)__shfl_xor((int)m, o); m = t > m ? t : m; }
        m = first_u32(m);
        const uint64_t who = BALLOT(ok && v == m);
        *best = m;
        return who ? __ffsll((long long)who) - 1 : -1;
    }
    __device__ __forceinline__ bool hs_first(HSCursor &c, int64_t *loc, uint32_t *seed_offset) {
        bool ok = c.act && c.nh > 0u;
        hs_stage(c, ok, 0u, c.nh > 1u ? 1u : 0u);
        const uint32_t v = ok ? hs_get(c, 0u) - c.so : 0u;
        ok = ok && v > 0u;
        uint32_t best;
        const int w = wave_argmax32(ok, v, &best);
        *loc = 0;
        if (w < 0) return true;
        *loc = (int64_t)best;
        *seed_offset = (uint32_t)__builtin_amdgcn_readlane((int)c.so, w);
        c.recent = best;
        return false;
    }
    __device__ __forceinline__ bool hs_next_lower(HSCursor &c, int64_t *loc, uint32_t *seed_offset) {
        bool live = c.act && c.cur != c.nh;
        hs_stage(c, live, c.cur > 0u ? c.cur - 1u : 0u, c.cur + 1u < c.nh ? c.cur + 1u : c.cur);
        uint32_t hv = live ? hs_get(c, c.cur) : 0u;
        if (live && hv - c.so == c.recent) {
            c.cur++;
            live = c.cur != c.nh;
            if (live) hv = hs_get(c, c.cur);
        }
        const bool ok = live && hv >= c.so && hv - c.so > 0u;
        uint32_t best;
        const int w = wave_argmax32(ok, hv - c.so, &best);
        if (w < 0) return false;
        *loc = (int64_t)best;
        *seed_offset = (uint32_t)__builtin_amdgcn_readlane((int)c.so, w);
        c.recent = best;
        return true;
    }
    __device__ __forceinline__ bool hs_next_le(HSCursor &c, int64_t max_loc, int64_t *loc, uint32_t *seed_offset) {
        const int64_t max_this = max_loc + c.so;
        const uint32_t wcap = hs_w;
        auto peek = [&](int64_t i) -> int64_t {
            if (c.single) return (int64_t)c.singleton;
            if (c.wbase >= 0 && i >= (int64_t)c.wbase && i < (int64_t)c.wbase + (int64_t)wcap) return (int64_t)c.win[i - c.wbase];
            return (int64_t)c.hits[i];
        };
        int64_t lo = c.act ? (int64_t)c.cur : 0, hi = c.act ? (int64_t)c.nh - 1 : -1;
        if (c.act && !c.single && c.wbase >= 0) {
            const int64_t wend = ((int64_t)c.wbase + (int64_t)wcap < (int64_t)c.nh ? (int64_t)c.wbase + (int64_t)wcap : (int64_t)c.nh) - 1;
            if (wend >= lo && (int64_t)c.win[wend - c.wbase] <= max_this) hi = wend;
        }
        bool found = false;
        uint32_t v = 0;
        while (BALLOT(lo <= hi && !found)) {
            if (lo <= hi && !found) {
                const int64_t probe = (lo + hi) / 2;
                const int64_t ph = peek(probe);
                if (ph <= max_this && (probe == 0 || peek(probe - 1) > max_this)) {
                    found = true; v = (uint32_t)ph - c.so;
                    c.cur = (uint32_t)probe;
                } else if (ph > max_this) lo = probe + 1; else hi = probe - 1;
            }
        }
        if (c.act && !found) c.cur = c.nh;
        uint32_t best;
        const int w = wave_argmax32(found && v > 0u, v, &best);
        if (w < 0) return false;
        *loc = (int64_t)best;
        *seed_offset = (uint32_t)__builtin_amdgcn_readlane((int)c.so, w);
        c.recent = best;
        return true;
    }
    __device__ __forceinline__ uint32_t hs_best_possible(HSCursor &c, uint32_t *exhausted) {
        const int64_t target = (int64_t)c.recent + c.so;
        hs_stage(c, c.act && c.nh > 0u, c.cur > 0u ? c.cur - 1u : 0u, c.cur < c.nh ? c.cur : c.nh - 1u);
        bool close = false;
        if (c.act) {
            if (c.cur != c.nh) { const int64_t a = (int64_t)hs_get(c, c.cur); const int64_t d = a > target ? a - target : target - a; close = d <= PE_MERGE_DIST; }
            if (!close && c.cur != 0u) { const int64_t a = (int64_t)hs_get(c, c.cur - 1u); const int64_t d = a > target ? a - target : target - a; close = d <= PE_MERGE_DIST; }
        }
        uint32_t best = 0;
        for (int d = 0; d <= c.cd; d++) {
            uint32_t m = ld(exhausted[d]) + (uint32_t)__popcll(BALLOT(c.act && !close && c.wd == (uint32_t)d));
            if (m > best) best = m;
        }
        return best;
    }

    template <class R> __device__ __forceinline__ void hint_indels(R *r, uint32_t first, uint32_t n, int K) {
        const int lane = lane_id();
        r += first;
        uint32_t carry_t = 0;
        for (uint32_t base = 0; base < n; base += WAVE) {
            const uint32_t i = base + (uint32_t)lane;
            const bool act = i < n;
            const int64_t li = act ? (int64_t)r[i].loc : 0;
            uint32_t t = i, b = i;
            for (uint32_t step = 1; step < (uint32_t)K + 1u; step++) {
                const bool fw = act && t == i + step - 1u && i + step < n;
                const bool bw = act && b == i - step + 1u && i >= step;
                if (!BALLOT(fw || bw)) break;
                if (fw && li - (int64_t)r[i + step].loc < (int64_t)K) t = i + step;
                if (bw && (int64_t)r[i - step].loc - li < (int64_t)K) b = i - step;
            }
            uint32_t prev_t = (uint32_t)__shfl_up((int)t, 1);
            if (lane == 0) prev_t = carry_t;
            carry_t = (uint32_t)__builtin_amdgcn_readlane((int)t, WAVE - 1);
            int64_t big = 0;
            if (act && b < i) big = (int64_t)r[b].loc - li;
            if (act && t > i && t > prev_t) { const int64_t d = li - (int64_t)r[t].loc; big = d > big ? d : big; }
            if (act && big > 0) r[i].big_indel = (decltype(r[i].big_indel))big;
            WAVE_SYNC();
        }
    }

    __device__ __forceinline__ bool lookup(const uint8_t *text, PEHits out[2]) {
        SeedBits seed = pack_seed(text, al->ix.seed_len);
        if (!seed.valid) return false;
        HitList hl[2];
        lookup_seed(al->ix, seed, hl);
        out[0].hits = (const G(uint32_t) *)hl[0].hits; out[0].n_hits = hl[0].n_hits; out[0].singleton = hl[0].singleton;
        out[1].hits = (const G(uint32_t) *)hl[1].hits; out[1].n_hits = hl[1].n_hits; out[1].singleton = hl[1].singleton;
        al->cnt().lookups++;
        al->cnt().slots += hl[0].slots + hl[1].slots;
        return true;
    }
    __device__ __forceinline__ uint32_t wrapped_seed(uint32_t wrap) const { return tab->wrapped_seed[wrap]; }
    __device__ __forceinline__ uint32_t count_n(const uint8_t *b, int len) const {
        uint32_t n = 0;
        const int lane = lane_id();
        for (int i0 = 0; i0 < len; i0 += WAVE) {
            int i = i0 + lane;
            n += (uint32_t)__popcll(BALLOT(i < len && b[i] == 'N'));
        }
        return n;
    }
    __device__ __forceinline__ const uint8_t *window(int64_t loc, int read_len) {
        al->read_len = read_len;
        al->stage_window(loc);
        uint8_t *g = al->gw;
        return g + WIN_PAD;
    }
    __device__ __forceinline__ bool is_alt(int64_t loc) const { return al->is_alt(loc); }
    __device__ __forceinline__ bool substring_ok(int64_t loc, int64_t len) const { return al->substring_ok(loc, len); }
    __device__ __forceinline__ int mapq(double p_all, double p_best, int popular) const { return compute_mapq(tab, p_all, p_best, popular); }
    __device__ __forceinline__ double seed_prob() const { return tab->seed_prob; }
    __device__ __forceinline__ double phred(uint8_t q) const { return tab->phred[q]; }
    __device__ __forceinline__ double indel(int n) const { return tab->indel[n]; }
    __device__ __forceinline__ double perfect(int n) const { return tab->perfect[n]; }

    __device__ __forceinline__ LVOut lv(int st, const uint8_t *P, const uint8_t *Q, int plen, const uint8_t *T, int tlen, int k) {
        const LdsSeq Ps = lds_seq(ByteSeq{P, st}), Qs = lds_seq(ByteSeq{Q, st}), Ts = lds_seq(ByteSeq{T, st});
        LVResult r = k <= (int)al->cfg.kmax ? lv_compute(Ps, Qs, plen, Ts, tlen, k, al->lv_tri, al->cfg.kmax, tab, al->cfg.RL)
                                            : lv_compute<false>(Ps, Qs, plen, Ts, tlen, k, lv_big, kmax_lv, tab, al->cfg.RL);
        LVOut o;
        o.score = i32(r.score); o.mp = f64(r.match_probability); o.net_indel = i32(r.net_indel);
        o.total_indels = i32(r.total_indels); o.text_span = i32(r.text_span);
        return o;
    }
    __device__ __forceinline__ AGOut ag(bool banded, int st, const uint8_t *P, const uint8_t *Q, int plen, const uint8_t *T, int tlen, int lim,
                                        int read_len, bool is_rc, int use_clip) {
        const LdsSeq Ps = lds_seq(ByteSeq{P, st}), Qs = lds_seq(ByteSeq{Q, st}), Ts = lds_seq(ByteSeq{T, st});
        if constexpr (EXACT) {
            int nv, sl, ns;
            ag_dims(banded, plen, lim > 126 ? 126 : (lim < 0 ? 0 : lim), &nv, &sl, &ns);
            uint32_t ext = (lim >= 0 && tlen > 0) ? (uint32_t)tlen * (uint32_t)(ns * sl) : 0u;
            const uint32_t image = (uint32_t)ag_scratch_bytes(al->cfg.RL);
            if (ext > image) ext = image;
            if (st == 1) ag_hw0 = ext > ag_hw0 ? ext : ag_hw0; else ag_hw1 = ext > ag_hw1 ? ext : ag_hw1;
        }
        if (++al->ag_calls_unit == WAVE_PRIO_HEAVY_AFTER * 8) wave_set_priority(1);
        AGResult a = ag_dispatch<AGC, EXACT>(banded, st, agp, Ps, Qs, plen, Ts, tlen, lim, read_len, is_rc, use_clip, al->ag_rows,
                                             EXACT ? (st == 1 ? ag_persist0 : ag_persist1) : (uint8_t *)al->ag_scratch, al->cfg.RL, tab, EXACT ? ag_tag : 0u);
        AGOut o;
        o.ag_score = i32(a.ag_score); o.text_offset = i32(a.text_offset); o.pattern_offset = i32(a.pattern_offset);
        o.n_edits = i32(a.n_edits); o.mp = f64(a.match_probability); o.stale = i32(a.stale_reads);
        return o;
    }
    __device__ __forceinline__ void sort_candidates(const G(snapgpu_paired_result) *c, uint32_t n, G(uint32_t) *order) {
        const int lane = lane_id();
        uint32_t *base = (uint32_t *)(uint16_t *)al->lv_tri;
        uint32_t *hist = base;
        for (int k = lane; k < 512; k += WAVE) hist[k] = 0;
        WAVE_SYNC();
        for (uint32_t j0 = 0; j0 < n; j0 += WAVE) {
            uint32_t j = j0 + (uint32_t)lane;
            if (j < n) atomicAdd(&hist[c[j].reserved & 511u], 1u);
        }
        WAVE_SYNC();
        uint32_t loc[8], sum = 0;
        for (int t = 0; t < 8; t++) { loc[t] = hist[lane * 8 + t]; sum += loc[t]; }
        uint32_t incl = sum;
        for (int o = 1; o < WAVE; o <<= 1) { uint32_t v = (uint32_t)__shfl_up((int)incl, o); if (lane >= o) incl += v; }
        uint32_t run = incl - sum;
        WAVE_SYNC();
        for (int t = 0; t < 8; t++) { hist[lane * 8 + t] = run; run += loc[t]; }
        WAVE_SYNC();
        for (uint32_t j0 = 0; j0 < n; j0 += WAVE) {
            uint32_t j = j0 + (uint32_t)lane;
            const bool act = j < n;
            const uint32_t key = act ? (c[j].reserved & 511u) : 0xffffffffu;
            uint64_t todo = BALLOT(act);
            while (todo) {
                const int leader = __ffsll((long long)todo) - 1;
                const uint32_t k = (uint32_t)__builtin_amdgcn_readlane((int)key, leader);
                const uint64_t same = BALLOT(act && key == k);
                const uint32_t b = base[k];
                if (act && key == k) order[b + (uint32_t)__popcll(same & ((1ull << lane) - 1ull))] = j;
                WAVE_SYNC();
                if (lane == 0) base[k] = b + (uint32_t)__popcll(same);
                WAVE_SYNC();
                todo &= ~same;
            }
        }
        WAVE_SYNC();
    }
    __device__ __forceinline__ uint32_t align_single(int r, int max_k, bool hamming, snapgpu_single_result &res, snapgpu_single_result &alt,
                                                     bool want_secondary, G(snapgpu_single_result) *sec_out, uint32_t sec_room, uint32_t room32) {
        (void)want_secondary; (void)room32;
        al->max_k = (uint32_t)max_k;
        if (!hamming) {
            al->template align_read_inner<false>(g_bases[r], g_quals[r], g_len[r]);
        } else {
            al->template align_read_inner<true>(g_bases[r], g_quals[r], g_len[r]);
            if (!al->agc_overflow) al->align_affine_gap(ws->ag_all, ws->ag_non_alt);
            al->primary().reserved = (al->ag_stale & 0x3fffffffu) | (al->ag_replay ? 0x40000000u : 0u);
        }
        WAVE_SYNC();
        res = al->primary();
        alt = al->first_alt();
        if (al->agc_overflow) res.reserved |= 0x80000000u;
        WAVE_SYNC();
        if constexpr (SEC) {
            if (al->sec_overflow) res.reserved |= 0x80000000u;
            const uint32_t n = al->n_sec;
            const uint32_t n_out = n < sec_room ? n : sec_room;
            const int lane = lane_id();
            const int nd = (int)(sizeof(snapgpu_single_result) / 4);
            for (uint32_t k0 = 0; k0 < n_out; k0 += 2) {
                const uint32_t k = k0 + (uint32_t)(lane >> 5);
                const int w = lane & 31;
                if (k < n_out && w < nd) ((G(uint32_t) *)&sec_out[k])[w] = ((const uint32_t *)&al->sec[al->sec_ord[k]])[w];
            }
            WAVE_SYNC();
            return n;
        } else {
            (void)sec_out; (void)sec_room;
            return 0;
        }
    }
    __device__ __forceinline__ uint32_t single_raw_secondary() const {
        if constexpr (SEC) return al->n_sec_raw; else return 0;
    }
};

template <int AGC, bool SEC, bool EXACT = false, bool CLIP = false>
__global__ __launch_bounds__(256, SNAPGPU_PAIRED_WAVES_PER_SIMD(AGC)) void k_align_paired(PairedArgs a)
{
    extern __shared__ __attribute__((aligned(16))) uint8_t lds[];
    const int lane = lane_id();
    const int wave_in_block = __builtin_amdgcn_readfirstlane((int)(threadIdx.x >> 6));
    const uint32_t wave_slot = blockIdx.x * (blockDim.x >> 6) + (uint32_t)wave_in_block;
    const LdsLayout SL = lds_layout(a.scfg.RL, a.scfg.num_weight_lists, a.scfg.kmax, a.scfg.ag_lds);
    const PairedLds PLd = paired_lds_layout(SL.total, a.scfg.RL, a.pcfg.max_seeds);
    uint8_t *my = lds + (size_t)wave_in_block * PLd.total;
    uint8_t *sc = a.scratch + (size_t)wave_slot * a.stride;

    WaveShared *ws = (WaveShared *)(my + SL.shared);
    typedef Aligner<AGC, SEC, EXACT> AL_T; typedef DevPL<AGC, SEC, EXACT> PL_T; typedef PairedCore<PL_T> CORE_T;
    constexpr uint32_t AL_SZ = ((uint32_t)sizeof(AL_T) + 15u) & ~15u, PL_SZ = ((uint32_t)sizeof(PL_T) + 15u) & ~15u;
    static_assert(AL_SZ + PL_SZ + sizeof(CORE_T) <= PE_FRAME_BYTES, "the wave's frame does not fit PE_FRAME_BYTES");
    uint8_t *frame = my + PLd.frame;
    AL_T &al = *new (frame) AL_T(a.ix, a.tab, a.scfg, ws);
    al.rd[0] = my + SL.rd0; al.rd[1] = my + SL.rd1;
    al.ql[0] = my + SL.ql0; al.ql[1] = my + SL.ql1;
    al.gw = my + SL.gw;
    al.seed_used = (uint32_t *)(my + SL.seed_used);
    al.wl_next = (uint16_t *)(my + SL.wl_next);
    al.wl_prev = (uint16_t *)(my + SL.wl_prev);
    al.lv_tri = (uint16_t *)(my + SL.lv);
    al.ag_rows = (int16_t *)(my + SL.ag);
    al.rp = (unsigned long long *)(my + SL.rp); al.tp = (unsigned long long *)(my + SL.tp); al.lvp = (unsigned long long *)(my + SL.lvp);
    al.heads = (uint16_t *)sc;
    al.pool = (Elem *)(sc + (size_t)a.scfg.ht_size * 2);
    al.ag_scratch = sc + (size_t)a.scfg.ht_size * 2 + (size_t)a.scfg.pool_size * sizeof(Elem);
    al.agc = a.single_agc_cap ? (snapgpu_single_result *)(sc + a.off_single_agc) : nullptr;
    al.agc_cap = a.single_agc_cap;
    al.cnt() = WaveCounters{0, 0, 0, 0, 0, 0, 0, 0, 0, 0, 0, 0};
    al.ag_calls_unit = 0;
    al.se_slots = nullptr; al.se_n_slots = 0; al.se_spec = nullptr; al.se_spec_cap = 0; al.se_ctl = nullptr; al.se_eager = 0; al.se_diag = nullptr;
    al.se_items = nullptr; al.se_first = nullptr; al.se_slot = -1; al.se_n = 0; al.se_tried = 0; al.cur_read = 0; al.se_mine = nullptr;

    if constexpr (SEC) {
        al.sec_cfg = a.ssec_cfg;
        al.sec = (snapgpu_single_result *)(sc + a.off_ssec);
        al.sec_key = (uint32_t *)(sc + a.off_ssec + (size_t)a.ssec_cfg.cap * sizeof(snapgpu_single_result));
        al.sec_ord = al.sec_key + 2 * (size_t)a.ssec_cfg.cap;
        al.n_sec = 0; al.n_sec_raw = 0; al.sec_overflow = 0;
    }
    PL_T &pl = *new (frame + AL_SZ) PL_T;
    pl.al = &al; pl.tab = a.tab; pl.ws = ws; pl.kmax_lv = a.kmax_lv; pl.lv_big = (uint16_t *)(sc + a.off_lv_big);
    al.ag_persist0 = al.ag_persist1 = pl.ag_persist0 = pl.ag_persist1 = nullptr;
    al.ag_hw0 = al.ag_hw1 = pl.ag_hw0 = pl.ag_hw1 = 0;
    pl.ag_epoch = 0; pl.ag_tag = 0;
    pl.help = EXACT ? nullptr : (G(PEHelpSlot) *)a.help; pl.n_help = a.n_help; pl.help_spec = (G(PEHelpSpec) *)a.help_spec; pl.help_spec_cap = a.help_spec_cap;
    pl.help_idle = a.help_done ? (const G(uint32_t) *)(a.help_done + 1) : nullptr; pl.help_eager = a.help_eager != 0;
    pl.cur_pair = 0; pl.my_slot = -1; pl.diag = (G(unsigned long long) *)(a.counters + 13);
    pl.hs_w = 8u * PE_MRING + 2u * a.pcfg.max_seeds * 16u * 4u <= lv_lds_bytes(a.scfg.kmax, a.scfg.RL) ? 16u : 8u;
    if constexpr (EXACT) {
        uint8_t *pb = a.persist + (size_t)wave_slot * a.persist_stride;
        const size_t q = (size_t)(a.persist_stride / 4);
        pl.ag_persist0 = pb; pl.ag_persist1 = pb + q; al.ag_persist0 = pb + 2 * q; al.ag_persist1 = pb + 3 * q;
    }
    pl.agp = AGParams{a.scfg.match_reward, a.scfg.sub_penalty, a.scfg.gap_open, a.scfg.gap_extend, a.scfg.five_bonus, a.scfg.three_bonus};

    CORE_T &core = *new (frame + AL_SZ + PL_SZ) CORE_T(pl, a.pcfg);
    core.help_min = a.help_min;
    core.lk = (PELookup *)(my + PLd.lk);
    core.exhausted = (uint32_t *)(my + PLd.exhausted);
    core.miss = (uint32_t *)(my + PLd.miss);
    core.hs = (PEHitSetHdr *)(my + PLd.hs);
    core.list_head = (int32_t *)(my + PLd.list_head);
    core.seed_used = (uint32_t *)(my + PLd.seed_used);
    core.sh = (PEShared *)(my + PLd.sh);
    core.mring = (uint32_t *)(my + SL.lv);
    core.cand = (G(PECand) *)(sc + a.off_cand);
    core.mate[0] = (G(PEMate) *)(sc + a.off_mate0);
    core.mate[1] = (G(PEMate) *)(sc + a.off_mate1);
    core.anchor = (G(PEAnchor) *)(sc + a.off_anchor);
    core.agc = (G(snapgpu_paired_result) *)(sc + a.off_agc);
    core.agc_order = (G(uint32_t) *)(sc + a.off_agc_order);
    core.sec = nullptr; core.sec_ord = nullptr; core.sec_key = nullptr; core.n_sec = 0;
    core.ssec_out = nullptr; core.ssec_stride = 0; core.n_ssec[0] = core.n_ssec[1] = 0; core.ref_dep = 0;
    if constexpr (SEC) {
        core.sec = (G(snapgpu_paired_result) *)(sc + a.off_sec);
        core.sec_ord = (G(uint32_t) *)(sc + a.off_sec_ord);
        core.sec_key = (G(uint32_t) *)(sc + a.off_sec_key);
    }
    core.S()->cnt = PECounters{0, 0, 0, 0, 0, 0, 0, 0, 0, 0, 0, 0};
    uint8_t *prd = my + PLd.rd, *pql = my + PLd.ql;
    const uint32_t RL = a.scfg.RL;
    uint64_t n_done = 0;

    const uint32_t n_total = a.remap ? first_u32(*a.n_remap) : a.n_pairs;
    auto load_pair = [&](uint32_t i) {
        for (int r = 0; r < 2; r++) {
            uint64_t b = first_u64(a.offsets[2 * (size_t)i + r]), e = first_u64(a.offsets[2 * (size_t)i + r + 1]);
            if constexpr (CLIP) { b += (uint64_t)first_u32((uint32_t)a.front_clip[2 * (size_t)i + r]); e = b + (uint64_t)first_u32((uint32_t)a.data_len[2 * (size_t)i + r]); }
            int len = (int)(e - b);
            if (len < 0 || len > (int)RL) len = 0;
            uint8_t *f = prd + (2 * r) * RL, *rc = prd + (2 * r + 1) * RL, *qf = pql + (2 * r) * RL, *qr = pql + (2 * r + 1) * RL;
            for (int j0 = 0; j0 < len; j0 += WAVE) {
                int j = j0 + lane;
                if (j < len) {
                    uint8_t bb = a.bases[b + j], qq = a.quals[b + j];
                    f[j] = bb; qf[j] = qq;
                    rc[len - 1 - j] = rc_base(bb); qr[len - 1 - j] = qq;
                }
            }
            core.rd[r][0] = f; core.rd[r][1] = rc; core.ql[r][0] = qf; core.ql[r][1] = qr;
            core.read_len[r] = len;
            pl.g_bases[r] = a.bases + b; pl.g_quals[r] = a.quals + b; pl.g_len[r] = len;
        }
        WAVE_SYNC();
    };
    while (true) {
        uint32_t i = 0;
        if (lane == 0) i = atomicAdd(a.work_counter, 1u);
        i = first_u32(i);
        if (i >= n_total) break;
        if (a.remap) i = first_u32(a.remap[i]);
        if (CLIP && first_u32((uint32_t)a.skip[i]) != 0u) {
            const int nd = (int)(sizeof(snapgpu_paired_result) / 4);
            if (lane < nd) { ((uint32_t *)&a.primary[i])[lane] = 0u; if (a.first_alt) ((uint32_t *)&a.first_alt[i])[lane] = 0u; }
            WAVE_SYNC();
            if (lane < 2) {
                a.primary[i].status[lane] = SNAPGPU_NotFound; a.primary[i].location[lane] = SNAPGPU_InvalidGenomeLocation32; a.primary[i].score[lane] = -1;
                if (a.first_alt) { a.first_alt[i].status[lane] = SNAPGPU_NotFound; a.first_alt[i].location[lane] = SNAPGPU_InvalidGenomeLocation32; a.first_alt[i].score[lane] = -1; }
            }
            if (!EXACT && a.help_done != nullptr && lane == 0) atomicAdd(a.help_done, 1u);
            continue;
        }
        if constexpr (EXACT) {
            if (++pl.ag_epoch == 16u) {
                if (pl.ag_hw0) wave_zero16(pl.ag_persist0, ((size_t)pl.ag_hw0 + 15) & ~(size_t)15);
                if (pl.ag_hw1) wave_zero16(pl.ag_persist1, ((size_t)pl.ag_hw1 + 15) & ~(size_t)15);
                if (al.ag_hw0) wave_zero16(al.ag_persist0, ((size_t)al.ag_hw0 + 15) & ~(size_t)15);
                if (al.ag_hw1) wave_zero16(al.ag_persist1, ((size_t)al.ag_hw1 + 15) & ~(size_t)15);
                pl.ag_hw0 = pl.ag_hw1 = al.ag_hw0 = al.ag_hw1 = 0; pl.ag_epoch = 1u;
                WAVE_SYNC();
            }
            pl.ag_tag = al.ag_tag = bt_tag_bits(pl.ag_epoch);
        }
        load_pair(i);
        pl.cur_pair = i;
        if (al.ag_calls_unit >= WAVE_PRIO_HEAVY_AFTER * 8) wave_set_priority(0);
        al.ag_calls_unit = 0;
        al.ag_obj_used0 = al.ag_obj_used1 = 0;
        {
            uint32_t *z0 = (uint32_t *)&core.S()->res, *z1 = (uint32_t *)&core.S()->alt;
            const int nd = (int)(sizeof(snapgpu_paired_result) / 4);
            if (lane < nd) { z0[lane] = 0; z1[lane] = 0; }
        }
        WAVE_SYNC();
        if constexpr (SEC) {
            core.ssec_out = a.ssec_out_stride ? (G(snapgpu_single_result) *)(a.single_secondary + (size_t)i * a.ssec_out_stride) : nullptr;
            core.ssec_stride = a.ssec_out_stride;
        }
        core.align_pair(a.max_k_paired, a.max_k_single);
        core.S()->res.flags = (core.overflow ? SNAPGPU_PAIR_POOL_OVERFLOW : 0) | (core.ref_dep ? SNAPGPU_PAIR_REF_BUFFER_DEPENDENT : 0) |
                             ((EXACT || core.stale_later || (a.dbg_flag_every != 0u && i % a.dbg_flag_every == 0u)) ? SNAPGPU_PAIR_EXACT_REPLAY : 0);
        WAVE_SYNC();
        if constexpr (SEC) {
            const uint32_t n_sec = core.overflow ? 0u : core.n_sec;
            if (lane == 0) {
                a.n_secondary[i] = n_sec;
                a.n_single_secondary[2 * (size_t)i] = core.overflow ? 0u : core.n_ssec[0];
                a.n_single_secondary[2 * (size_t)i + 1] = core.overflow ? 0u : core.n_ssec[1];
            }
            const uint32_t n_out = n_sec < a.sec_out_stride ? n_sec : a.sec_out_stride;
            const int nd = (int)(sizeof(snapgpu_paired_result) / 4);
            for (uint32_t k = 0; k < n_out; k++) {
                const G(uint32_t) *src = (const G(uint32_t) *)core.secondary(k);
                uint32_t *dst = (uint32_t *)&a.secondary[(size_t)i * a.sec_out_stride + k];
                if (lane < nd) dst[lane] = src[lane];
            }
            WAVE_SYNC();
        }
        {
            const uint32_t *src = (const uint32_t *)&core.S()->res, *src2 = (const uint32_t *)&core.S()->alt;
            uint32_t *dst = (uint32_t *)&a.primary[i];
            const int nd = (int)(sizeof(snapgpu_paired_result) / 4);
            if (lane < nd) dst[lane] = src[lane];
            if (a.first_alt) { uint32_t *dst2 = (uint32_t *)&a.first_alt[i]; if (lane < nd) dst2[lane] = src2[lane]; }
        }
        WAVE_SYNC();
        n_done++;
        if (!EXACT && a.help_done != nullptr && lane == 0) atomicAdd(a.help_done, 1u);
    }
    if constexpr (!EXACT) {
        if (a.help != nullptr && a.help_done != nullptr) {
            if (lane == 0) atomicAdd(a.help_done + 1, 1u);
            const uint64_t t_idle0 = wave_clock();
            for (uint32_t round = 0;; round++) {
                if ((round & 7u) == 0u) {
                    const uint32_t dn = DevPL<AGC, SEC, EXACT>::aload(a.help_done);
                    if (dn >= n_total) break;
                    if (wave_clock() - t_idle0 > 24000000000ull) {
                        if (lane == 0) { atomicAdd(&a.counters[14], 1ull << 32); a.counters[15] = 0x3000000000000000ull | ((unsigned long long)n_total << 32) | dn; }
                        break;
                    }
                }
                bool any = false;
                for (uint32_t s = 0; s < a.n_help; s++) {
                    G(PEHelpSlot) *slot = (G(PEHelpSlot) *)&a.help[s];
                    if (DevPL<AGC, SEC, EXACT>::aload(&slot->pair) >= a.n_pairs) continue;
                    if (DevPL<AGC, SEC, EXACT>::aload(&slot->state) != 1u) continue;
                    if (DevPL<AGC, SEC, EXACT>::aload(&slot->next) >= DevPL<AGC, SEC, EXACT>::aload(&slot->n)) continue;
                    uint32_t before = 0;
                    if (lane == 0) before = atomicAdd(&slot->helpers, 1u);
                    before = first_u32(before);
                    if (before < 0x7fffffffu && DevPL<AGC, SEC, EXACT>::aload(&slot->state) == 1u) {
                        DevPL<AGC, SEC, EXACT>::fence_acquire();
                        load_pair(DevPL<AGC, SEC, EXACT>::aload(&slot->pair));
                        pl.help_work(core, slot);
                        any = true;
                    }
                    if (lane == 0) atomicSub(&slot->helpers, 1u);
                }
#ifdef SNAPGPU_WAVE_EMU
                if (!getenv("SNAPGPU_EMU_HELP_SPIN")) break;
#endif
                if (!any) { DevPL<AGC, SEC, EXACT>::nap(); DevPL<AGC, SEC, EXACT>::nap(); }
            }
        }
    }
    if constexpr (EXACT) {
        if (pl.ag_hw0) wave_zero16(pl.ag_persist0, ((size_t)pl.ag_hw0 + 15) & ~(size_t)15);
        if (pl.ag_hw1) wave_zero16(pl.ag_persist1, ((size_t)pl.ag_hw1 + 15) & ~(size_t)15);
        if (al.ag_hw0) wave_zero16(al.ag_persist0, ((size_t)al.ag_hw0 + 15) & ~(size_t)15);
        if (al.ag_hw1) wave_zero16(al.ag_persist1, ((size_t)al.ag_hw1 + 15) & ~(size_t)15);
    }
    if (lane == 0 && !(EXACT && a.is_replay)) {
        if (!a.is_replay) atomicAdd(&a.counters[0], (unsigned long long)(2 * n_done));
        atomicAdd(&a.counters[1], (unsigned long long)al.cnt().lookups);
        atomicAdd(&a.counters[2], (unsigned long long)al.cnt().slots);
        atomicAdd(&a.counters[3], (unsigned long long)(al.cnt().hits + core.S()->cnt.hits));
        atomicAdd(&a.counters[4], (unsigned long long)(al.cnt().overflow_lists + core.S()->cnt.overflow_lists));
        atomicAdd(&a.counters[5], (unsigned long long)(al.cnt().lv + core.S()->cnt.lv));
        atomicAdd(&a.counters[6], (unsigned long long)(al.cnt().ag + core.S()->cnt.ag));
        atomicAdd(&a.counters[7], (unsigned long long)(al.cnt().lv_ref_bytes + core.S()->cnt.lv_ref_bytes));
        atomicAdd(&a.counters[8], (unsigned long long)core.S()->cnt.cyc_lookup);
        atomicAdd(&a.counters[9], (unsigned long long)core.S()->cnt.cyc_intersect);
        atomicAdd(&a.counters[10], (unsigned long long)core.S()->cnt.cyc_lv);
        atomicAdd(&a.counters[11], (unsigned long long)core.S()->cnt.cyc_ag);
        atomicAdd(&a.counters[12], (unsigned long long)core.S()->cnt.cyc_total);
        atomicAdd(&a.counters[13], (unsigned long long)core.S()->cnt.cyc_single);
    }
}

template <int UNUSED>
__global__ void k_collect_flagged(snapgpu_paired_result *primary, uint32_t n, uint32_t *list, uint32_t *count, int stale)
{
    uint32_t i = blockIdx.x * blockDim.x + threadIdx.x;
    if (i >= n) return;
    const uint32_t fl = primary[i].flags;
    const bool ov = (fl & SNAPGPU_PAIR_POOL_OVERFLOW) != 0;
    if (stale ? (!ov && (fl & SNAPGPU_PAIR_EXACT_REPLAY) != 0) : ov) list[atomicAdd(count, 1u)] = i;
}
```

snap_amd/csrc/single_kernel.h:

```cpp
#pragma once
#include "kernel_common.h"

#ifndef SNAPGPU_WAVES_PER_SIMD
#define SNAPGPU_WAVES_PER_SIMD(AGC) ((AGC) == 3 ? 6 : 4)
#endif
template <int AGC, bool SEC, bool EXACT = false, bool TIMED = false, bool PLANES = false>
__global__ __launch_bounds__(256, SNAPGPU_WAVES_PER_SIMD(AGC)) void k_align_single(AlignArgs a)
{
    extern __shared__ __attribute__((aligned(16))) uint8_t lds[];
    const int lane = lane_id();
    const int wave_in_block = __builtin_amdgcn_readfirstlane((int)(threadIdx.x >> 6));
    const uint32_t wave_slot = blockIdx.x * (blockDim.x >> 6) + (uint32_t)wave_in_block;
    const LdsLayout L = lds_layout(a.cfg.RL, a.cfg.num_weight_lists, a.cfg.kmax, a.cfg.ag_lds);
    uint8_t *my = lds + (size_t)wave_in_block * L.total;

    WaveShared *ws = (WaveShared *)(my + L.shared);
#if !defined(SNAPGPU_REGDIR)
    Aligner<AGC, SEC, EXACT, TIMED, PLANES> al(a.ix, a.tab, a.cfg, ws);
#else
    Aligner<AGC, SEC, EXACT, TIMED, PLANES, true> al(a.ix, a.tab, a.cfg, ws);
#endif
    al.rd[0] = my + L.rd0; al.rd[1] = my + L.rd1;
    al.ql[0] = my + L.ql0; al.ql[1] = my + L.ql1;
    al.gw = my + L.gw;
    al.seed_used = (uint32_t *)(my + L.seed_used);
    al.wl_next = (uint16_t *)(my + L.wl_next);
    al.wl_prev = (uint16_t *)(my + L.wl_prev);
    al.lv_tri = (uint16_t *)(my + L.lv);
    al.ag_rows = (int16_t *)(my + L.ag);
    al.rp = (unsigned long long *)(my + L.rp); al.tp = (unsigned long long *)(my + L.tp); al.lvp = (unsigned long long *)(my + L.lvp);
    uint8_t *sc = a.scratch + (size_t)wave_slot * a.cfg.scratch_stride;
    al.heads = (uint16_t *)sc;
    al.pool = (Elem *)(sc + (size_t)a.cfg.ht_size * 2);
    al.ag_scratch = sc + (size_t)a.cfg.ht_size * 2 + (size_t)a.cfg.pool_size * sizeof(Elem);
    al.ag_persist0 = al.ag_persist1 = nullptr; al.ag_hw0 = al.ag_hw1 = 0;
    if constexpr (EXACT) {
        al.ag_persist0 = a.persist + (size_t)wave_slot * a.persist_stride;
        al.ag_persist1 = al.ag_persist0 + a.persist_stride / 2;
    }
    if constexpr (SEC) {
        uint8_t *ss = a.sec_scratch + (size_t)wave_slot * a.sec_stride_bytes;
        al.sec_cfg = a.sec_cfg;
        al.sec = (snapgpu_single_result *)ss;
        al.sec_key = (uint32_t *)(ss + (size_t)a.sec_cfg.cap * sizeof(snapgpu_single_result));
        al.sec_ord = al.sec_key + 2 * (size_t)a.sec_cfg.cap;
        al.n_sec = 0;
        al.adj_scratch = a.sec_cfg.adjust ? ss + a.sec_cfg.adj_off : nullptr;
    }
    al.cnt() = WaveCounters{0, 0, 0, 0, 0, 0, 0, 0, 0, 0, 0, 0};
    uint64_t n_done = 0;
    const bool se_on = !EXACT && a.se_slots != nullptr && a.cfg.se_items_cap != 0;
    al.se_slots = se_on ? a.se_slots : nullptr; al.se_n_slots = a.se_n_slots; al.se_spec = a.se_spec; al.se_spec_cap = a.se_spec_cap;
    al.se_ctl = a.se_ctl; al.se_eager = a.se_eager; al.se_diag = a.counters + 14;
    al.se_items = (uint32_t *)(sc + a.cfg.se_off); al.se_first = al.se_items + a.cfg.se_items_cap;
    al.se_slot = -1; al.se_n = 0; al.se_tried = 0; al.cur_read = 0; al.se_mine = nullptr;

    const uint32_t n_total = a.remap ? first_u32(*a.n_remap) : a.n_reads;
    unsigned long long dbg_worst = 0;
    if constexpr (TIMED) { if (a.dbg && lane == 0 && wave_slot < a.dbg_slots) a.dbg[64 + wave_slot] = wave_clock(); }
    while (true) {
        uint32_t i = 0;
        if (lane == 0) i = atomicAdd(a.work_counter, 1u);
        i = first_u32(i);
        if (i >= n_total) break;
        if (a.remap) i = first_u32(a.remap[i]);
        else if (a.order) i = first_u32(a.order[i]);
        al.new_read_images();
        al.cur_read = i;
        uint64_t b = first_u64(a.offsets[i]), e = first_u64(a.offsets[i + 1]);
        if (a.front_clip) {
            b += (uint64_t)first_u32((uint32_t)a.front_clip[i]); e = b + (uint64_t)first_u32((uint32_t)a.data_len[i]);
            if (a.skip && first_u32((uint32_t)a.skip[i]) != 0u) {
                const int nd = (int)(sizeof(snapgpu_single_result) / 4);
                if (lane < nd) { ((uint32_t *)&a.primary[i])[lane] = 0u; if (a.first_alt) ((uint32_t *)&a.first_alt[i])[lane] = 0u; }
                WAVE_SYNC();
                if (lane == 0) { a.primary[i].status = SNAPGPU_NotFound; a.primary[i].location = SNAPGPU_InvalidGenomeLocation32; a.primary[i].score = -1; }
                if (se_on && lane == 0) atomicAdd(&a.se_ctl[0], 1u);
                continue;
            }
        }
        const uint64_t dbg_t0 = TIMED ? wave_clock() : 0; const uint64_t dbg_ag0 = al.cnt().ag;
        al.align_read(a.bases + b, a.quals + b, (int)(e - b));
        WAVE_SYNC();
#if defined(SNAPGPU_TEST_BREAK_PARITY)
        if (i % 997u == 7u && lane == 0) ws->primary.mapq ^= 1;
        WAVE_SYNC();
#endif
        if constexpr (TIMED) {
            if (a.dbg) {
                const unsigned long long cyc = wave_clock() - dbg_t0, nag = al.cnt().ag - dbg_ag0;
                if (lane == 0) atomicAdd(&a.dbg[63 - __clzll((long long)(cyc | 1ull))], 1ull);
                const unsigned long long packed = (cyc << 24) | (nag > 0xffffffull ? 0xffffffull : nag);
                if (packed > dbg_worst) dbg_worst = packed;
            }
        }
        if constexpr (!EXACT) {
            if (a.flag_list && (ws->primary.reserved & 0x40000000u) && lane == 0) a.flag_list[atomicAdd(a.flag_count, 1u)] = i;
        }
        if (EXACT && lane == 0) ws->primary.reserved |= 0x80000000u;
        WAVE_SYNC();
        {
            const uint32_t *src = (const uint32_t *)&ws->primary;
            uint32_t *dst = (uint32_t *)&a.primary[i];
            const int nd = (int)(sizeof(snapgpu_single_result) / 4);
            if (lane < nd) dst[lane] = src[lane];
            if (a.first_alt) {
                const uint32_t *src2 = (const uint32_t *)&ws->first_alt;
                uint32_t *dst2 = (uint32_t *)&a.first_alt[i];
                if (lane < nd) dst2[lane] = src2[lane];
            }
        }
        WAVE_SYNC();
        if constexpr (SEC) {
            const uint32_t n_sec = al.n_sec;
            if (lane == 0) a.n_secondary[i] = al.sec_overflow ? 0xFFFFFFFFu : n_sec;
            const uint32_t n_out = n_sec < a.sec_out_stride ? n_sec : a.sec_out_stride;
            const int nd = (int)(sizeof(snapgpu_single_result) / 4);
            for (uint32_t k0 = 0; k0 < n_out; k0 += 2) {
                const uint32_t k = k0 + (uint32_t)(lane >> 5);
                const int w = lane & 31;
                if (k < n_out && w < nd) {
                    const uint32_t *src = (const uint32_t *)&al.sec[al.sec_ord[k]];
                    uint32_t *dst = (uint32_t *)&a.secondary[(size_t)i * a.sec_out_stride + k];
                    dst[w] = src[w];
                }
            }
            WAVE_SYNC();
        }
        n_done++;
        if (se_on && lane == 0) atomicAdd(&a.se_ctl[0], 1u);
    }
    if constexpr (!EXACT) {
        if (se_on && (a.se_keep <= 1u || wave_slot % a.se_keep == 0u)) {
            if (lane == 0) atomicAdd(&a.se_ctl[1], 1u);
            const uint64_t t_idle0 = wave_clock();
            for (uint32_t round = 0;; round++) {
                if (XW::ld(a.se_ctl[0]) >= n_total) break;
                if ((round & 63u) == 0u && wave_clock() - t_idle0 > 48000000000ull) {
                    if (lane == 0) atomicAdd(&a.counters[14], 1ull << 32);
                    break;
                }
                bool any = false;
                if (XW::ld(a.se_ctl[2]) != 0u) {
                    const uint32_t s_first = (wave_slot * 13u + round * 7u) % a.se_n_slots;
                    for (uint32_t k = 0; k < a.se_n_slots && !any; k++) {
                        const uint32_t s = s_first + k < a.se_n_slots ? s_first + k : s_first + k - a.se_n_slots;
                        SEHelpSlot *slot = &a.se_slots[s];
                        if (XW::ld(slot->state) != 1u) continue;
                        if (XW::ld(slot->next) >= XW::ld(slot->n)) continue;
                        if (XW::ld(slot->helpers) >= SE_HELP_MAX_HELPERS) continue;
                        uint32_t before = 0;
                        if (lane == 0) before = atomicAdd(&slot->helpers, 1u);
                        before = first_u32(before);
                        if (before < SE_HELP_MAX_HELPERS && XW::aload(&slot->state) == 1u) {
                            XW::fence_acquire();
                            const uint32_t r = XW::ld(slot->read);
                            if (r < a.n_reads) {
                                uint64_t rb = first_u64(a.offsets[r]), re = first_u64(a.offsets[r + 1]);
                                if (a.front_clip) { rb += (uint64_t)first_u32((uint32_t)a.front_clip[r]); re = rb + (uint64_t)first_u32((uint32_t)a.data_len[r]); }
                                const int len = (int)(re - rb);
                                if (len >= (int)a.ix.seed_len && len <= (int)a.cfg.RL) {
                                    al.read_len = len;
                                    (void)al.load_read(a.bases + rb, a.quals + rb, len);
                                    WAVE_SYNC();
                                    if (PLANES && a.ix.planes != nullptr) al.build_read_planes(len);
                                    al.se_help_slot(slot);
                                    any = true;
                                }
                            }
                        }
                        if (lane == 0) atomicSub(&slot->helpers, 1u);
                    }
                }
#ifdef SNAPGPU_WAVE_EMU
                if (!getenv("SNAPGPU_EMU_HELP_SPIN")) break;
#endif
                if (!any) { for (int z = 0; z < 8; z++) XW::nap(); }
            }
        }
    }
    if constexpr (TIMED) {
        if (a.dbg && lane == 0 && wave_slot < a.dbg_slots) { a.dbg[64 + a.dbg_slots + wave_slot] = wave_clock(); a.dbg[64 + 2 * a.dbg_slots + wave_slot] = dbg_worst; }
    }
    if constexpr (EXACT) {
        if (al.ag_hw0) wave_zero16(al.ag_persist0, ((size_t)al.ag_hw0 + 15) & ~(size_t)15);
        if (al.ag_hw1) wave_zero16(al.ag_persist1, ((size_t)al.ag_hw1 + 15) & ~(size_t)15);
    }
    if (lane == 0 && !a.is_replay) {
        atomicAdd(&a.counters[0], (unsigned long long)n_done);
        atomicAdd(&a.counters[1], (unsigned long long)al.cnt().lookups);
        atomicAdd(&a.counters[2], (unsigned long long)al.cnt().slots);
        atomicAdd(&a.counters[3], (unsigned long long)al.cnt().hits);
        atomicAdd(&a.counters[4], (unsigned long long)al.cnt().overflow_lists);
        atomicAdd(&a.counters[5], (unsigned long long)al.cnt().lv);
        atomicAdd(&a.counters[6], (unsigned long long)al.cnt().ag);
        atomicAdd(&a.counters[7], (unsigned long long)al.cnt().lv_ref_bytes);
        atomicAdd(&a.counters[8], (unsigned long long)al.cnt().cyc_lookup);
        atomicAdd(&a.counters[9], (unsigned long long)al.cnt().cyc_hits);
        atomicAdd(&a.counters[10], (unsigned long long)al.cnt().cyc_lv);
        atomicAdd(&a.counters[11], (unsigned long long)al.cnt().cyc_ag);
        atomicAdd(&a.counters[12], (unsigned long long)al.cnt().cyc_total);
    }
}
```

snap_amd/csrc/snapgpu.hip:

```cpp
#include <hip/hip_runtime.h>
#include <math.h>
#include <stdio.h>
#include <stdlib.h>
#include <string.h>
#include <string>
#include <vector>
#include <deque>
#include <mutex>
#include <chrono>
#include <atomic>
#include <memory>
#include <thread>
#include <fcntl.h>
#include <unistd.h>
#include <sys/stat.h>

#include "../../include/snapgpu.h"
#include "dev_common.h"
#include "probe.h"
#include "lv.h"
#include "ag_win.h"
#include "align_single.h"
#include "kernel_common.h"
#include "single_kernel.h"
// ... 396 lines not shown
        double dlo = 1e-300, dhi = 1.0;
        memcpy(&lo, &dlo, 8); memcpy(&hi, &dhi, 8);
        while (hi - lo > 1) {
            uint64_t mid = lo + (hi - lo) / 2;
            double x; memcpy(&x, &mid, 8);
            int f = (int)(-10 * log10(x));
            if (f >= m) lo = mid; else hi = mid;
        }
        double x; memcpy(&x, &lo, 8);
        t.mapq_threshold[m] = x;
    }
    t.mapq_threshold[71] = 0.0;

    memset(t.wrapped_seed, 0, sizeof(t.wrapped_seed));
    if (seed_len >= 2 && seed_len <= 32) {
        std::vector<unsigned> offsets(seed_len, 0);
        std::deque<std::pair<unsigned, unsigned>> work;
        work.push_back({1u, seed_len - 1});
        unsigned filled = 1;
        while (!work.empty()) {
            auto it = work.front(); work.pop_front();
            unsigned sel = (it.first + it.second) / 2;
            offsets[sel] = filled++;
            if (it.second > sel) work.push_back({sel + 1, it.second});
            if (it.first < sel) work.push_back({it.first, sel - 1});
        }
        for (unsigned i = 0; i < seed_len; i++) t.wrapped_seed[i] = offsets[i];
    }
}

static uint32_t next_pow2(uint32_t v) { uint32_t p = 1; while (p < v) p <<= 1; return p; }

extern "C" void snapgpu_destroy(snapgpu_ctx *ctx) {
    if (!ctx) return;
    if (ctx->device >= 0) (void)hipSetDevice(ctx->device);
    if (ctx->owns_index) {
        if (ctx->d_hash) (void)hipFree(ctx->d_hash);
        if (ctx->d_overflow) (void)hipFree(ctx->d_overflow);
        if (ctx->d_genome_padded) (void)hipFree(ctx->d_genome_padded);
    }
    if (ctx->owns_buckets) {
        if (ctx->d_bucket_blob) (void)hipFree(ctx->d_bucket_blob);
        if (ctx->d_bucket_offset) (void)hipFree(ctx->d_bucket_offset);
        if (ctx->d_n_buckets) (void)hipFree(ctx->d_n_buckets);
    }
    if (ctx->d_sec_scratch) (void)hipFree(ctx->d_sec_scratch);
    if (ctx->d_table_offset) (void)hipFree(ctx->d_table_offset);
    if (ctx->d_table_size) (void)hipFree(ctx->d_table_size);
    if (ctx->d_contig_begin) (void)hipFree(ctx->d_contig_begin);
    if (ctx->d_proj) (void)hipFree(ctx->d_proj);
    if (ctx->d_tab) (void)hipFree(ctx->d_tab);
    if (ctx->d_scratch) (void)hipFree(ctx->d_scratch);
    if (ctx->d_pscratch) (void)hipFree(ctx->d_pscratch);
    if (ctx->d_pscratch_big) (void)hipFree(ctx->d_pscratch_big);
    if (ctx->d_pscratch_sec) (void)hipFree(ctx->d_pscratch_sec);
    if (ctx->d_pscratch_sec_big) (void)hipFree(ctx->d_pscratch_sec_big);
    if (ctx->d_flag_list) (void)hipFree(ctx->d_flag_list);
    if (ctx->d_exact_persist) (void)hipFree(ctx->d_exact_persist);
    if (ctx->d_pexact_persist) (void)hipFree(ctx->d_pexact_persist);
    if (ctx->d_help) (void)hipFree(ctx->d_help);
    if (ctx->d_help_spec) (void)hipFree(ctx->d_help_spec);
    if (ctx->feeders) ctx->feeders->fetch_sub(1);
    if (ctx->d_dbg) (void)hipFree(ctx->d_dbg);
    if (ctx->d_se_slots) (void)hipFree(ctx->d_se_slots);
    if (ctx->d_se_spec) (void)hipFree(ctx->d_se_spec);
    if (ctx->d_se_ctl) (void)hipFree(ctx->d_se_ctl);
    if (ctx->d_planes && ctx->owns_planes) (void)hipFree(ctx->d_planes);
    if (ctx->d_order) (void)hipFree(ctx->d_order);
    if (ctx->d_wbucket) (void)hipFree(ctx->d_wbucket);
    if (ctx->d_whist) (void)hipFree(ctx->d_whist);
    ctx->pool.free_all();
    if (ctx->d_work) (void)hipFree(ctx->d_work);
    if (ctx->d_counters) (void)hipFree(ctx->d_counters);
    if (ctx->ev0) (void)hipEventDestroy(ctx->ev0);
    if (ctx->ev1) (void)hipEventDestroy(ctx->ev1);
    if (ctx->stream) (void)hipStreamDestroy(ctx->stream);
    delete ctx;
}

static bool lv_planes_wanted() {
    const char *e = getenv("SNAPGPU_LV_PLANES");
    return !getenv("SNAPGPU_NO_PLANES") && e && atoi(e) != 0;
}

static int build_planes(snapgpu_ctx *ctx)
{
    if (!lv_planes_wanted()) return SNAPGPU_OK;
    const uint64_t n_bytes = ctx->ix.n_bases + 2 * (uint64_t)ctx->ix.genome_pad;
    const uint64_t n_blocks = (n_bytes + 63) / 64 + 32;
    if (!ctx->d_planes) {
        ctx->plane_bytes = n_blocks * 24;
        HIPCHK(ctx, hipMalloc((void **)&ctx->d_planes, (size_t)ctx->plane_bytes), SNAPGPU_E_NOMEM);
        ctx->owns_planes = true;
    }
    hipLaunchKernelGGL(k_genome_planes, dim3((unsigned)ctx->num_cus * 8), dim3(256), 0, ctx->stream, (const uint8_t *)ctx->d_genome_padded, n_bytes, n_blocks, ctx->d_planes);
    HIPCHK(ctx, hipGetLastError(), SNAPGPU_E_LAUNCH);
    HIPCHK(ctx, hipStreamSynchronize(ctx->stream), SNAPGPU_E_LAUNCH);
    ctx->ix.planes = ctx->d_planes;
    return SNAPGPU_OK;
}

static int build_buckets(snapgpu_ctx *ctx)
{
    DevIndex &ix = ctx->ix;
    if (ix.large || ix.entry_bytes != 8 || ix.key_bytes > 4 || getenv("SNAPGPU_NO_BUCKETS")) return SNAPGPU_OK;
    const uint32_t nt = ix.n_hash_tables;
    std::vector<uint64_t> nb(nt), boff(nt);
    uint64_t total = 0;
    for (uint32_t t = 0; t < nt; t++) { nb[t] = bucket_count_for(ctx->h_table_size[t]); boff[t] = total * BUCKET_BYTES; total += nb[t]; }
    if (!ctx->d_bucket_blob) {
        ctx->bucket_bytes = total * BUCKET_BYTES;
        HIPCHK(ctx, hipMalloc(&ctx->d_bucket_blob, (size_t)ctx->bucket_bytes + 64), SNAPGPU_E_NOMEM);
        HIPCHK(ctx, hipMalloc(&ctx->d_bucket_offset, (size_t)nt * 8), SNAPGPU_E_NOMEM);
        HIPCHK(ctx, hipMalloc(&ctx->d_n_buckets, (size_t)nt * 8), SNAPGPU_E_NOMEM);
        HIPCHK(ctx, hipMemcpy(ctx->d_bucket_offset, boff.data(), (size_t)nt * 8, hipMemcpyHostToDevice), SNAPGPU_E_NODEVICE);
        HIPCHK(ctx, hipMemcpy(ctx->d_n_buckets, nb.data(), (size_t)nt * 8, hipMemcpyHostToDevice), SNAPGPU_E_NODEVICE);
    }
    const uint32_t key_mask = ix.key_bytes >= 4 ? 0xffffffffu : ((1u << (8 * ix.key_bytes)) - 1u);
    hipLaunchKernelGGL(k_bucket_init, dim3((unsigned)ctx->num_cus * 8), dim3(256), 0, ctx->stream, (uint32_t *)ctx->d_bucket_blob, total);
    for (uint32_t t = 0; t < nt; t++) {
        if (ctx->h_table_size[t] == 0) continue;
        hipLaunchKernelGGL(k_bucket_build, dim3((unsigned)ctx->num_cus * 4), dim3(256), 0, ctx->stream,
                           (const uint32_t *)((const uint8_t *)ctx->d_hash + ctx->h_table_offset[t]), ctx->h_table_size[t], key_mask,
                           (uint32_t *)((uint8_t *)ctx->d_bucket_blob + boff[t]), nb[t]);
    }
    HIPCHK(ctx, hipGetLastError(), SNAPGPU_E_LAUNCH);
    HIPCHK(ctx, hipStreamSynchronize(ctx->stream), SNAPGPU_E_LAUNCH);
    ix.bucket_blob = (const uint8_t *)ctx->d_bucket_blob;
    ix.bucket_offset = (const uint64_t *)ctx->d_bucket_offset;
    ix.n_buckets = (const uint64_t *)ctx->d_n_buckets;
    return SNAPGPU_OK;
}

extern "C" int snapgpu_create(const snapgpu_index_view *idx, const snapgpu_params *p, int device, snapgpu_ctx **out)
{
    if (!idx || !p || !out) return fail(nullptr, SNAPGPU_E_INVALID, "snapgpu_create: null argument");
    *out = nullptr;
    if (idx->location_size != 4)
        return fail(nullptr, SNAPGPU_E_UNSUPPORTED, "index uses 64-bit genome locations; only the 32-bit lookup path (seed >= 20) is implemented");
    if (idx->seed_len < 2 || idx->seed_len > 32) return fail(nullptr, SNAPGPU_E_INVALID, "seed length out of range");
    if (idx->key_bytes < 2 || idx->key_bytes > 8) return fail(nullptr, SNAPGPU_E_INVALID, "hash key size out of range");
    if (idx->genome_pad < 1000) return fail(nullptr, SNAPGPU_E_INVALID, "genome_pad must be >= 1000");
    if (p->max_read_len < idx->seed_len || p->max_read_len > 1000)
        return fail(nullptr, SNAPGPU_E_INVALID, "max_read_len must be in [seed_len, 1000] (MAX_READ_LENGTH, Read.h:49)");
    if (p->sub_penalty <= p->gap_extend_penalty) return fail(nullptr, SNAPGPU_E_INVALID, "sub_penalty must exceed gap_extend_penalty");
    if (p->sub_penalty > p->gap_open_penalty + p->gap_extend_penalty)
        return fail(nullptr, SNAPGPU_E_INVALID, "subPenalty > gapOpen + gapExtend (BaseAligner.cpp:141)");

    int ndev = 0;
    if (hipGetDeviceCount(&ndev) != hipSuccess || ndev <= 0)
        return fail(nullptr, SNAPGPU_E_NODEVICE, "no HIP device available (this library has no CPU path)");
    if (device < 0 || device >= ndev) return fail(nullptr, SNAPGPU_E_NODEVICE, "device index out of range");

    snapgpu_ctx *ctx = new snapgpu_ctx();
    ctx->device = device;
    ctx->params = *p;
#define CRCHK(call, code) do { hipError_t _e = (call); if (_e != hipSuccess) { \
        fail(nullptr, code, std::string(#call) + ": " + hipGetErrorString(_e)); snapgpu_destroy(ctx); return code; } } while (0)
    CRCHK(hipSetDevice(device), SNAPGPU_E_NODEVICE);
    hipDeviceProp_t prop;
    CRCHK(hipGetDeviceProperties(&prop, device), SNAPGPU_E_NODEVICE);
    ctx->num_cus = prop.multiProcessorCount;
    CRCHK(hipStreamCreateWithFlags(&ctx->stream, hipStreamNonBlocking), SNAPGPU_E_NODEVICE);
    CRCHK(hipEventCreate(&ctx->ev0), SNAPGPU_E_NODEVICE);
    CRCHK(hipEventCreate(&ctx->ev1), SNAPGPU_E_NODEVICE);

    DevIndex &ix = ctx->ix;
    ix.n_bases = idx->n_bases; ix.overflow_size = idx->overflow_table_size;
    ix.first_alt_location = idx->first_alt_location; ix.n_contigs = idx->n_contigs;
    ix.seed_len = idx->seed_len; ix.key_bytes = idx->key_bytes; ix.large = idx->large_hash_table ? 1 : 0;
    ix.entry_bytes = 4 * (ix.large ? 2 : 1) + ix.key_bytes; ix.n_hash_tables = idx->n_hash_tables;
    ix.chromosome_padding = idx->chromosome_padding; ix.genome_pad = idx->genome_pad;
    const size_t genome_total = (size_t)idx->n_bases + 2 * (size_t)idx->genome_pad;
    const size_t overflow_words = idx->overflow_table_size ? (size_t)idx->overflow_table_size : 1;
    if (idx->on_device) {
        ctx->owns_index = false;
        ctx->d_hash = (void *)idx->hash_blob;
        ctx->d_overflow = (void *)idx->overflow;
        ctx->d_genome_padded = (void *)(idx->genome - idx->genome_pad);
    } else {
        CRCHK(hipMalloc(&ctx->d_hash, (size_t)idx->hash_blob_bytes + 16), SNAPGPU_E_NOMEM);
        CRCHK(hipMalloc(&ctx->d_overflow, overflow_words * 4 + 16), SNAPGPU_E_NOMEM);
        CRCHK(hipMalloc(&ctx->d_genome_padded, genome_total + 16), SNAPGPU_E_NOMEM);
        if (idx->hash_blob) CRCHK(hipMemcpy(ctx->d_hash, idx->hash_blob, (size_t)idx->hash_blob_bytes, hipMemcpyHostToDevice), SNAPGPU_E_NODEVICE);
        if (idx->overflow) CRCHK(hipMemcpy(ctx->d_overflow, idx->overflow, overflow_words * 4, hipMemcpyHostToDevice), SNAPGPU_E_NODEVICE);
        if (idx->genome) CRCHK(hipMemcpy(ctx->d_genome_padded, idx->genome - idx->genome_pad, genome_total, hipMemcpyHostToDevice), SNAPGPU_E_NODEVICE);
    }
    ix.hash_blob = (const uint8_t *)ctx->d_hash;
    ix.overflow = (const uint32_t *)ctx->d_overflow;
    ix.genome = (const uint8_t *)ctx->d_genome_padded + idx->genome_pad;
    CRCHK(hipMalloc(&ctx->d_table_offset, (size_t)idx->n_hash_tables * 8), SNAPGPU_E_NOMEM);
    CRCHK(hipMalloc(&ctx->d_table_size, (size_t)idx->n_hash_tables * 8), SNAPGPU_E_NOMEM);
    CRCHK(hipMemcpy(ctx->d_table_offset, idx->table_offset, (size_t)idx->n_hash_tables * 8, hipMemcpyHostToDevice), SNAPGPU_E_NODEVICE);
    CRCHK(hipMemcpy(ctx->d_table_size, idx->table_size, (size_t)idx->n_hash_tables * 8, hipMemcpyHostToDevice), SNAPGPU_E_NODEVICE);
    size_t nc = idx->n_contigs ? idx->n_contigs : 1;
    CRCHK(hipMalloc(&ctx->d_contig_begin, nc * 8), SNAPGPU_E_NOMEM);
    if (idx->n_contigs) CRCHK(hipMemcpy(ctx->d_contig_begin, idx->contig_begin, (size_t)idx->n_contigs * 8, hipMemcpyHostToDevice), SNAPGPU_E_NODEVICE);
    ix.table_offset = (const uint64_t *)ctx->d_table_offset;
    ix.table_size = (const uint64_t *)ctx->d_table_size;
    ix.contig_begin = (const uint64_t *)ctx->d_contig_begin;
    ix.bucket_blob = nullptr; ix.bucket_offset = nullptr; ix.n_buckets = nullptr; ix.planes = nullptr;
    {
        const size_t n = idx->n_contigs;
        const uint32_t n_ops = (idx->contig_cigar_start && idx->cigar_ops && n) ? idx->contig_cigar_start[n] : 0;
        std::vector<uint8_t> img(n * 8 + (n + 1) * 4 + ((size_t)n_ops + 1) * 4 + n + 16, 0);
        uint64_t *pb = (uint64_t *)img.data();
        uint32_t *cs = (uint32_t *)(img.data() + n * 8);
        uint32_t *ops = cs + (n + 1);
        uint8_t *rc = (uint8_t *)(ops + (size_t)n_ops + 1);
        for (size_t i = 0; i < n; i++) {
            pb[i] = idx->contig_proj_begin ? idx->contig_proj_begin[i] : 0;
            rc[i] = idx->contig_proj_rc ? idx->contig_proj_rc[i] : 0;
            cs[i] = n_ops ? idx->contig_cigar_start[i] : 0;
        }
        cs[n] = n_ops;
        for (uint32_t i = 0; i < n_ops; i++) ops[i] = idx->cigar_ops[i];
        CRCHK(hipMalloc(&ctx->d_proj, img.size()), SNAPGPU_E_NOMEM);
        CRCHK(hipMemcpy(ctx->d_proj, img.data(), img.size(), hipMemcpyHostToDevice), SNAPGPU_E_NODEVICE);
        uint8_t *d = (uint8_t *)ctx->d_proj;
        ctx->proj.contig_begin = (const uint64_t *)ctx->d_contig_begin;
        ctx->proj.proj_begin = (const uint64_t *)d;
        ctx->proj.cigar_start = (const uint32_t *)(d + n * 8);
        ctx->proj.cigar_ops = ctx->proj.cigar_start + (n + 1);
        ctx->proj.proj_rc = (const uint8_t *)(ctx->proj.cigar_ops + (size_t)n_ops + 1);
        ctx->proj.n_contigs = idx->n_contigs;
    }

    {
        ctx->view_meta = *idx;
        const size_t n = idx->n_contigs;
        ctx->h_table_offset.assign(idx->table_offset, idx->table_offset + idx->n_hash_tables);
        ctx->h_table_size.assign(idx->table_size, idx->table_size + idx->n_hash_tables);
        if (n) ctx->h_contig_begin.assign(idx->contig_begin, idx->contig_begin + n);
        if (idx->contig_proj_begin && n) ctx->h_proj_begin.assign(idx->contig_proj_begin, idx->contig_proj_begin + n);
        if (idx->contig_proj_rc && n) ctx->h_proj_rc.assign(idx->contig_proj_rc, idx->contig_proj_rc + n);
        if (idx->contig_cigar_start && idx->cigar_ops && n) {
            ctx->h_cigar_start.assign(idx->contig_cigar_start, idx->contig_cigar_start + n + 1);
            ctx->h_cigar_ops.assign(idx->cigar_ops, idx->cigar_ops + idx->contig_cigar_start[n]);
        }
        ctx->view_meta.hash_blob = nullptr; ctx->view_meta.overflow = nullptr; ctx->view_meta.genome = nullptr;
        ctx->view_meta.table_offset = nullptr; ctx->view_meta.table_size = nullptr; ctx->view_meta.contig_begin = nullptr;
        ctx->view_meta.contig_proj_begin = nullptr; ctx->view_meta.contig_proj_rc = nullptr; ctx->view_meta.contig_cigar_start = nullptr;
        ctx->view_meta.cigar_ops = nullptr;
    }

    if (g_share_buckets_from && g_share_buckets_from->d_bucket_blob && idx->on_device && !getenv("SNAPGPU_NO_BUCKETS")) {
        ctx->owns_buckets = false;
        ctx->d_bucket_blob = g_share_buckets_from->d_bucket_blob; ctx->d_bucket_offset = g_share_buckets_from->d_bucket_offset;
        ctx->d_n_buckets = g_share_buckets_from->d_n_buckets; ctx->bucket_bytes = g_share_buckets_from->bucket_bytes;
        ix.bucket_blob = (const uint8_t *)ctx->d_bucket_blob; ix.bucket_offset = (const uint64_t *)ctx->d_bucket_offset;
        ix.n_buckets = (const uint64_t *)ctx->d_n_buckets;
    } else if (idx->on_device || idx->hash_blob != nullptr) {
        const int brc = build_buckets(ctx);
        if (brc != SNAPGPU_OK) { snapgpu_destroy(ctx); return brc; }
    }
    if (g_share_buckets_from && g_share_buckets_from->d_planes && idx->on_device && lv_planes_wanted()) {
        ctx->d_planes = g_share_buckets_from->d_planes; ctx->owns_planes = false; ctx->plane_bytes = g_share_buckets_from->plane_bytes;
        ix.planes = ctx->d_planes;
    } else if (idx->on_device || idx->genome != nullptr) {
        const int prc = build_planes(ctx);
        if (prc != SNAPGPU_OK) { snapgpu_destroy(ctx); return prc; }
    }

    build_tables(ctx->h_tab, idx->seed_len);
    CRCHK(hipMalloc((void **)&ctx->d_tab, sizeof(DevTables)), SNAPGPU_E_NOMEM);
    CRCHK(hipMemcpy(ctx->d_tab, &ctx->h_tab, sizeof(DevTables), hipMemcpyHostToDevice), SNAPGPU_E_NODEVICE);

    AlignCfg &c = ctx->cfg;
    c.max_hits = p->max_hits; c.max_k = p->max_k; c.num_seeds = p->num_seeds;
    c.min_weight = p->min_weight_to_check < 1 ? 1 : p->min_weight_to_check;
    c.extra_depth = p->extra_search_depth; c.use_ag = p->use_affine_gap ? 1 : 0; c.ag_buffers = c.use_ag;
    c.match_reward = (int)p->match_reward; c.sub_penalty = (int)p->sub_penalty;
    c.gap_open = (int)p->gap_open_penalty; c.gap_extend = (int)p->gap_extend_penalty;
    c.five_bonus = (int)p->five_prime_end_bonus; c.three_bonus = (int)p->three_prime_end_bonus;
    c.alt_aware = p->alt_awareness ? 1 : 0; c.emit_alt = p->emit_alt_alignments ? 1 : 0;
    c.max_gap_alt = p->max_score_gap_to_prefer_non_alt; c.seed_coverage = p->seed_coverage;
    uint32_t max_seeds_ctor = p->num_seeds != 0 ? p->num_seeds : (uint32_t)(int)(p->seed_coverage * 1000 / idx->seed_len);
    c.num_weight_lists = max_seeds_ctor + 1;
    if (c.num_weight_lists < 2 || c.num_weight_lists > 0x3FF) { snapgpu_destroy(ctx); return fail(nullptr, SNAPGPU_E_UNSUPPORTED, "number of seeds out of the supported range [1, 1022]"); }
    c.RL = (p->max_read_len + 15) & ~15u;
    uint32_t kmax = p->max_k + p->extra_search_depth; if (kmax > 126) kmax = 126;
    c.kmax = kmax;
    uint64_t pool = (uint64_t)p->max_hits * max_seeds_ctor;
    if (pool < 64) pool = 64;
    if (pool > 60000) { snapgpu_destroy(ctx); return fail(nullptr, SNAPGPU_E_UNSUPPORTED, "max_hits * num_seeds > 60000 candidate buckets per read is not supported"); }
    c.pool_size = (uint32_t)pool;
    c.ht_size = next_pow2((uint32_t)pool * 2);
    c.ag_numvec_max = (c.RL + 7) / 8;
    {
        int need = ag_max_positions((int)p->max_read_len - (int)idx->seed_len, (int)kmax);
        ctx->ag_variant = need <= 192 ? 3 : need <= 256 ? 4 : need <= 384 ? 6 : 0;
        if (getenv("SNAPGPU_AG_LDS")) ctx->ag_variant = 0;
    }
    size_t ag_bytes = c.ag_buffers ? ag_scratch_bytes(c.RL) : 0;
    if (const char *e = getenv("SNAPGPU_SINGLE_HELP")) { ctx->single_help_forced = atoi(e) != 0 ? 1 : 0; ctx->single_help = ctx->single_help_forced != 0; }
    if (g_share_buckets_from && g_share_buckets_from->feeders && idx->on_device) { ctx->feeders = g_share_buckets_from->feeders; ctx->feeders->fetch_add(1); }
    else ctx->feeders = std::make_shared<std::atomic<int>>(1);
    if (const char *e = getenv("SNAPGPU_SINGLE_HELP_EAGER")) ctx->single_help_eager = atoi(e) != 0;
    if (const char *e = getenv("SNAPGPU_SINGLE_HELP_KEEP")) { int v = atoi(e); if (v >= 1 && v <= 64) ctx->single_help_keep = (uint32_t)v; }
    c.se_items_cap = ctx->single_help ? SE_HELP_ITEMS_CAP : 0u;
    c.se_off = ((size_t)c.ht_size * 2 + (size_t)c.pool_size * sizeof(Elem) + ag_bytes + 255) & ~(size_t)255;
    c.scratch_stride = (c.se_off + ((size_t)c.se_items_cap + (c.se_items_cap ? c.pool_size : 0u)) * 4 + 255) & ~(size_t)255;
    c.ag_lds = !c.ag_buffers ? 0u : (ctx->ag_variant == 3 ? ag_lds_bytes_reg(c.RL, 3) : ag_lds_bytes(c.RL));
    LdsLayout L = lds_layout(c.RL, c.num_weight_lists, c.kmax, c.ag_lds);
    c.lds_per_wave = L.total;

    int waves_per_cu = ctx->ag_variant == 3 ? 24 : 16;
    if (const char *e = getenv("SNAPGPU_WAVES_PER_CU")) { int v = atoi(e); if (v >= 1 && v <= 32) waves_per_cu = v; }
    while (waves_per_cu > 1 && (size_t)waves_per_cu * L.total > 160 * 1024) waves_per_cu--;
    if ((size_t)4 * L.total > 160 * 1024) { snapgpu_destroy(ctx); return fail(nullptr, SNAPGPU_E_UNSUPPORTED, "per-read LDS state exceeds 40 KiB per wave (max_read_len / num_seeds / max_k too large)"); }
    ctx->n_wave_slots = (uint32_t)ctx->num_cus * (uint32_t)waves_per_cu;
    ctx->n_wave_slots = (ctx->n_wave_slots + 3) & ~3u;
    size_t scratch_total = (size_t)ctx->n_wave_slots * c.scratch_stride;
    CRCHK(hipMalloc((void **)&ctx->d_scratch, scratch_total), SNAPGPU_E_NOMEM);
    CRCHK(hipMemsetAsync(ctx->d_scratch, 0, scratch_total, ctx->stream), SNAPGPU_E_NODEVICE);
    if (c.use_ag) {
        ctx->always_exact = ctx->ag_variant == 3;
        ctx->exact_slots = ctx->always_exact ? ctx->n_wave_slots : (ctx->n_wave_slots < 64 ? ctx->n_wave_slots : 64);
        ctx->exact_persist_stride = 2 * (uint64_t)((ag_bytes + 255) & ~(size_t)255);
        CRCHK(hipMalloc((void **)&ctx->d_exact_persist, (size_t)ctx->exact_slots * ctx->exact_persist_stride), SNAPGPU_E_NOMEM);
        CRCHK(hipMemsetAsync(ctx->d_exact_persist, 0, (size_t)ctx->exact_slots * ctx->exact_persist_stride, ctx->stream), SNAPGPU_E_NODEVICE);
    }
    if (const char *e = getenv("SNAPGPU_SINGLE_HEAVY_FIRST")) ctx->single_heavy_first = atoi(e) != 0 ? 1 : 0;
    if (const char *e = getenv("SNAPGPU_PHASE_TIMERS")) ctx->phase_timers = atoi(e) != 0;
    if (ctx->single_help) {
        ctx->se_spec_cap = c.se_items_cap;
        CRCHK(hipMalloc((void **)&ctx->d_se_slots, SE_HELP_SLOTS * sizeof(SEHelpSlot)), SNAPGPU_E_NOMEM);
        CRCHK(hipMalloc((void **)&ctx->d_se_spec, (size_t)SE_HELP_SLOTS * ctx->se_spec_cap * sizeof(SESpec)), SNAPGPU_E_NOMEM);
        CRCHK(hipMalloc((void **)&ctx->d_se_ctl, 256), SNAPGPU_E_NOMEM);
    }
    CRCHK(hipMalloc((void **)&ctx->d_work, 256), SNAPGPU_E_NOMEM);
    CRCHK(hipMemsetAsync(ctx->d_work, 0, 256, ctx->stream), SNAPGPU_E_NODEVICE);
    CRCHK(hipMalloc((void **)&ctx->d_counters, sizeof(snapgpu_counters)), SNAPGPU_E_NOMEM);
    CRCHK(hipMemsetAsync(ctx->d_counters, 0, sizeof(snapgpu_counters), ctx->stream), SNAPGPU_E_NODEVICE);
    CRCHK(hipStreamSynchronize(ctx->stream), SNAPGPU_E_NODEVICE);
#undef CRCHK
    *out = ctx;
    return SNAPGPU_OK;
}

extern "C" int snapgpu_device_count(void) {
    int n = 0;
    if (hipGetDeviceCount(&n) != hipSuccess) return 0;
    return n;
}

extern "C" int snapgpu_create_replica(const snapgpu_ctx *src, int device, int share_index, snapgpu_ctx **out)
{
    return snapgpu_create_replica_with_params(src, device, share_index, nullptr, out);
}

extern "C" int snapgpu_create_replica_with_params(const snapgpu_ctx *src, int device, int share_index, const snapgpu_params *p, snapgpu_ctx **out)
{
    if (!src || !out) return fail(nullptr, SNAPGPU_E_INVALID, "snapgpu_create_replica: null argument");
    *out = nullptr;
    if (share_index && device != src->device) return fail(nullptr, SNAPGPU_E_INVALID, "snapgpu_create_replica: index blobs can only be shared on the device that holds them");
    snapgpu_index_view v = src->view_meta;
    v.table_offset = src->h_table_offset.data(); v.table_size = src->h_table_size.data();
    v.contig_begin = src->h_contig_begin.empty() ? nullptr : src->h_contig_begin.data();
    v.contig_proj_begin = src->h_proj_begin.empty() ? nullptr : src->h_proj_begin.data();
    v.contig_proj_rc = src->h_proj_rc.empty() ? nullptr : src->h_proj_rc.data();
    v.contig_cigar_start = src->h_cigar_start.empty() ? nullptr : src->h_cigar_start.data();
    v.cigar_ops = src->h_cigar_ops.empty() ? nullptr : src->h_cigar_ops.data();
    if (share_index) {
        v.on_device = 1;
        v.hash_blob = (const uint8_t *)src->d_hash; v.overflow = (const uint32_t *)src->d_overflow;
        v.genome = (const uint8_t *)src->d_genome_padded + src->view_meta.genome_pad;
    } else {
        v.on_device = 0;
        v.hash_blob = nullptr; v.overflow = nullptr; v.genome = nullptr;
    }
    g_share_buckets_from = share_index ? src : nullptr;
    const int rc = snapgpu_create(&v, p ? p : &src->params, device, out);
    g_share_buckets_from = nullptr;
    return rc;
}

#include <dlfcn.h>
typedef struct ncclComm *ncclComm_t;
typedef int ncclResult_t;
typedef int ncclDataType_t;
static const ncclResult_t ncclSuccess = 0;
static const ncclDataType_t ncclUint8 = 1;
struct RcclApi {
    void *h = nullptr;
    ncclResult_t (*CommInitAll)(ncclComm_t *, int, const int *) = nullptr;
    ncclResult_t (*CommDestroy)(ncclComm_t) = nullptr;
    ncclResult_t (*GroupStart)() = nullptr;
    ncclResult_t (*GroupEnd)() = nullptr;
    ncclResult_t (*Broadcast)(const void *, void *, size_t, ncclDataType_t, int, ncclComm_t, hipStream_t) = nullptr;
    const char *(*GetErrorString)(ncclResult_t) = nullptr;
    bool load(std::string &why) {
        if (h) return true;
        for (const char *name : {"librccl.so.1", "librccl.so", "/opt/rocm/lib/librccl.so.1"}) { h = dlopen(name, RTLD_NOW | RTLD_LOCAL); if (h) break; }
        if (!h) { why = std::string("dlopen(librccl): ") + dlerror(); return false; }
        CommInitAll = (decltype(CommInitAll))dlsym(h, "ncclCommInitAll"); CommDestroy = (decltype(CommDestroy))dlsym(h, "ncclCommDestroy");
        GroupStart = (decltype(GroupStart))dlsym(h, "ncclGroupStart"); GroupEnd = (decltype(GroupEnd))dlsym(h, "ncclGroupEnd");
        Broadcast = (decltype(Broadcast))dlsym(h, "ncclBroadcast"); GetErrorString = (decltype(GetErrorString))dlsym(h, "ncclGetErrorString");
        if (!CommInitAll || !CommDestroy || !GroupStart || !GroupEnd || !Broadcast || !GetErrorString) { why = "librccl lacks an expected symbol"; return false; }
        return true;
    }
};
static RcclApi g_rccl;
static std::once_flag g_rccl_once; static bool g_rccl_ok = false; static std::string g_rccl_why;

extern "C" int snapgpu_broadcast_index(snapgpu_ctx **ctxs, int n)
{
    if (!ctxs || n < 1) return fail(nullptr, SNAPGPU_E_INVALID, "snapgpu_broadcast_index: bad argument");
    for (int i = 0; i < n; i++) if (!ctxs[i]) return fail(nullptr, SNAPGPU_E_INVALID, "snapgpu_broadcast_index: null context");
    snapgpu_ctx *root = ctxs[0];
    const size_t hash_bytes = (size_t)root->view_meta.hash_blob_bytes;
    const size_t ovf_bytes = (size_t)(root->view_meta.overflow_table_size ? root->view_meta.overflow_table_size : 1) * 4;
    const size_t gen_bytes = (size_t)root->view_meta.n_bases + 2 * (size_t)root->view_meta.genome_pad;
    for (int i = 1; i < n; i++) {
        const snapgpu_index_view &a = root->view_meta, &b = ctxs[i]->view_meta;
        if (a.hash_blob_bytes != b.hash_blob_bytes || a.overflow_table_size != b.overflow_table_size || a.n_bases != b.n_bases ||
            a.genome_pad != b.genome_pad || a.seed_len != b.seed_len || a.n_hash_tables != b.n_hash_tables)
            return fail(root, SNAPGPU_E_INVALID, "snapgpu_broadcast_index: context " + std::to_string(i) + " was not created over the same index (snapgpu_create_replica)");
        if (!ctxs[i]->owns_index) return fail(root, SNAPGPU_E_INVALID, "snapgpu_broadcast_index: context " + std::to_string(i) + " shares another context's blobs");
        for (int j = 0; j < i; j++) if (ctxs[j]->device == ctxs[i]->device) return fail(root, SNAPGPU_E_INVALID, "snapgpu_broadcast_index: two contexts on one device");
    }
    if (n == 1) return SNAPGPU_OK;
    std::call_once(g_rccl_once, [] { g_rccl_ok = g_rccl.load(g_rccl_why); });
    if (!g_rccl_ok) return fail(root, SNAPGPU_E_UNSUPPORTED, "snapgpu_broadcast_index: RCCL is not available (" + g_rccl_why + ")");
    std::vector<int> devs((size_t)n);
    struct Comms {
        std::vector<ncclComm_t> v;
        ~Comms() { for (auto c : v) if (c) g_rccl.CommDestroy(c); }
    } comms_owner; comms_owner.v.assign((size_t)n, nullptr);
    std::vector<ncclComm_t> &comms = comms_owner.v;
    for (int i = 0; i < n; i++) devs[(size_t)i] = ctxs[i]->device;
#define NCCLCHK(call) do { ncclResult_t _r = (call); if (_r != ncclSuccess) { \
        std::string m = std::string(#call) + ": " + g_rccl.GetErrorString(_r); return fail(root, SNAPGPU_E_LAUNCH, m); } } while (0)
    NCCLCHK(g_rccl.CommInitAll(comms.data(), n, devs.data()));
    struct Blob { void *snapgpu_ctx::*p; size_t bytes; };
    const Blob blobs[3] = {{&snapgpu_ctx::d_hash, hash_bytes}, {&snapgpu_ctx::d_overflow, ovf_bytes}, {&snapgpu_ctx::d_genome_padded, gen_bytes}};
    for (const Blob &b : blobs) {
        NCCLCHK(g_rccl.GroupStart());
        for (int i = 0; i < n; i++) {
            HIPCHK(root, hipSetDevice(ctxs[i]->device), SNAPGPU_E_NODEVICE);
            NCCLCHK(g_rccl.Broadcast(ctxs[i]->*(b.p), ctxs[i]->*(b.p), b.bytes, ncclUint8, 0, comms[(size_t)i], ctxs[i]->stream));
        }
        NCCLCHK(g_rccl.GroupEnd());
    }
    for (int i = 0; i < n; i++) {
        HIPCHK(root, hipSetDevice(ctxs[i]->device), SNAPGPU_E_NODEVICE);
        HIPCHK(root, hipStreamSynchronize(ctxs[i]->stream), SNAPGPU_E_LAUNCH);
    }
    for (auto &c : comms) { if (c) g_rccl.CommDestroy(c); c = nullptr; }
#undef NCCLCHK
    for (int i = 1; i < n; i++) {
        HIPCHK(root, hipSetDevice(ctxs[i]->device), SNAPGPU_E_NODEVICE);
        const int brc = build_buckets(ctxs[i]);
        if (brc != SNAPGPU_OK) return brc;
        const int prc = build_planes(ctxs[i]);
        if (prc != SNAPGPU_OK) return prc;
    }
    return SNAPGPU_OK;
}

static bool read_file(const std::string &path, std::vector<uint8_t> &out, std::string &err) {
    FILE *f = fopen(path.c_str(), "rb");
    if (!f) { err = "cannot open " + path; return false; }
    fseek(f, 0, SEEK_END); long long n = ftell(f); fseek(f, 0, SEEK_SET);
    out.resize((size_t)n);
    size_t got = n ? fread(out.data(), 1, (size_t)n, f) : 0;
    fclose(f);
    if ((long long)got != n) { err = "short read on " + path; return false; }
    return true;
}

struct LoadJob {
    int fd; uint64_t file_off; uint8_t *dev; uint64_t bytes;
    uint32_t src_entry = 1, dst_entry = 1, loc_size = 0, value_count = 0; bool slots = false;
};

static const char *narrow_entries(const LoadJob &j, uint8_t *buf, uint64_t n)
{
    const uint64_t all_ones = j.loc_size == 8 ? ~0ull : ((1ull << (8 * j.loc_size)) - 1ull);
    const uint32_t key_bytes = j.src_entry - j.loc_size * j.value_count;
    for (uint64_t e = 0; e < n; e++) {
        const uint8_t *src = buf + e * j.src_entry;
        uint8_t *dst = buf + e * j.dst_entry;
        uint32_t w[2];
        for (uint32_t k = 0; k < j.value_count; k++) {
            uint64_t v = 0; memcpy(&v, src + (size_t)k * j.loc_size, j.loc_size);
            if (!j.slots) {
                if (v > 0xffffffffull) return "OverflowTable entry does not fit 32 bits";
                w[k] = (uint32_t)v;
            }
            else if (v == all_ones) w[k] = 0xffffffffu;
            else if (v == all_ones - 1) w[k] = 0xfffffffeu;
            else if (v < 0xfffffffeull) w[k] = (uint32_t)v;
            else return "hash table value does not fit 32 bits";
        }
        memmove(dst + 4 * j.value_count, src + (size_t)j.loc_size * j.value_count, key_bytes);
        memcpy(dst, w, 4 * j.value_count);
    }
    return nullptr;
}

static int stream_files_to_device(const std::vector<LoadJob> &jobs, int device, std::string &err)
{
    const uint64_t PIECE = 64ull << 20;
    struct Slice { const LoadJob *j; uint64_t off, n; };
    std::vector<Slice> slices;
    for (const LoadJob &j : jobs) {
        const uint64_t step = PIECE / j.src_entry * j.src_entry;
        for (uint64_t o = 0; o < j.bytes; o += step) slices.push_back(Slice{&j, o, j.bytes - o < step ? j.bytes - o : step});
    }
    int n_threads = 12;
    if (const char *e = getenv("SNAPGPU_LOAD_THREADS")) { const int v = atoi(e); if (v >= 1 && v <= 64) n_threads = v; }
    uint64_t total_bytes = 0, largest = 0;
    for (const Slice &sl : slices) { total_bytes += sl.n; if (sl.n > largest) largest = sl.n; }
    {
        const uint64_t by_size = (total_bytes + PIECE - 1) / PIECE;
        if ((uint64_t)n_threads > by_size) n_threads = (int)(by_size ? by_size : 1);
    }
    const size_t piece_bytes = (size_t)(((largest ? largest : 1) + 4095) & ~(uint64_t)4095);
    const bool want_pin = !(getenv("SNAPGPU_LOAD_PIN") && atoi(getenv("SNAPGPU_LOAD_PIN")) == 0);
    std::atomic<size_t> next{0};
    std::atomic<int> failed{SNAPGPU_OK};
    std::mutex err_mu;
    auto stop = [&](int code, const char *msg) { std::lock_guard<std::mutex> g(err_mu); if (failed.load() == SNAPGPU_OK) { err = msg; failed = code; } };
    auto worker = [&]() {
        if (hipSetDevice(device) != hipSuccess) { stop(SNAPGPU_E_INVALID, "hipSetDevice failed while loading the index directory"); return; }
        void *buf = nullptr;
        hipStream_t st = nullptr;
        bool pinned = false;
        if (posix_memalign(&buf, 4096, piece_bytes) != 0 || !buf) { stop(SNAPGPU_E_INVALID, "out of host memory while loading the index directory"); return; }
        pinned = want_pin && hipHostRegister(buf, piece_bytes, 0) == hipSuccess;
        if (hipStreamCreateWithFlags(&st, hipStreamNonBlocking) != hipSuccess) {
            stop(SNAPGPU_E_INVALID, "hipStreamCreateWithFlags failed while loading the index directory");
            if (pinned) (void)hipHostUnregister(buf);
            free(buf); return;
        }
        while (failed.load() == SNAPGPU_OK) {
            const size_t k = next.fetch_add(1);
            if (k >= slices.size()) break;
            const Slice &s = slices[k];
            const LoadJob &j = *s.j;
            uint64_t got = 0;
            while (got < s.n) {
                const ssize_t r = pread(j.fd, (uint8_t *)buf + got, (size_t)(s.n - got), (off_t)(j.file_off + s.off + got));
                if (r <= 0) break;
                got += (uint64_t)r;
            }
            if (got < s.n) { stop(SNAPGPU_E_INVALID, "short read while loading the index directory"); break; }
            const uint64_t n_entries = s.n / j.src_entry;
            if (j.src_entry != j.dst_entry) {
                if (const char *msg = narrow_entries(j, (uint8_t *)buf, n_entries)) { stop(SNAPGPU_E_UNSUPPORTED, msg); break; }
            }
            if (hipMemcpyAsync(j.dev + s.off / j.src_entry * j.dst_entry, buf, (size_t)(n_entries * j.dst_entry), hipMemcpyHostToDevice, st) != hipSuccess ||
                hipStreamSynchronize(st) != hipSuccess) {
                stop(SNAPGPU_E_INVALID, "host-to-device copy failed while loading the index directory"); break;
            }
        }
        (void)hipStreamDestroy(st);
        if (pinned) (void)hipHostUnregister(buf);
        free(buf);
    };
    std::vector<std::thread> th;
    for (int t = 0; t < n_threads; t++) th.emplace_back(worker);
    for (auto &t : th) t.join();
    return failed.load();
}

extern "C" int snapgpu_create_from_directory(const char *index_dir, const snapgpu_params *p, int device, snapgpu_ctx **out)
{
    if (!index_dir || !p || !out) return fail(nullptr, SNAPGPU_E_INVALID, "snapgpu_create_from_directory: null argument");
    const std::string dir(index_dir);
    std::string err;
    std::vector<uint8_t> hdr;
    if (!read_file(dir + "/GenomeIndex", hdr, err)) return fail(nullptr, SNAPGPU_E_INVALID, err);
    hdr.push_back(0);
    int major = 0, minor = 0, n_tables = 0, seed_len = 0, padding = 0, key_bytes = 0, small = 0, loc_size = 0;
    long long overflow_size = 0, hash_file_size = 0;
    if (sscanf((const char *)hdr.data(), "%d %d %d %lld %d %d %d %lld %d %d", &major, &minor, &n_tables, &overflow_size, &seed_len,
               &padding, &key_bytes, &hash_file_size, &small, &loc_size) != 10 || n_tables < 0)
        return fail(nullptr, SNAPGPU_E_INVALID, "malformed GenomeIndex header");
    if (major != 7) return fail(nullptr, SNAPGPU_E_UNSUPPORTED, "index major version is not 7 (GenomeIndex.h:170)");
    if (loc_size < 4 || loc_size > 8) return fail(nullptr, SNAPGPU_E_INVALID, "GenomeIndex header: location size out of range");
    const bool wide = loc_size > 4;
    struct Fd { int fd = -1; ~Fd() { if (fd >= 0) close(fd); } } fg, fo, fh;
    fg.fd = open((dir + "/Genome").c_str(), O_RDONLY); fo.fd = open((dir + "/OverflowTable").c_str(), O_RDONLY); fh.fd = open((dir + "/GenomeIndexHash").c_str(), O_RDONLY);
    if (fg.fd < 0 || fo.fd < 0 || fh.fd < 0) return fail(nullptr, SNAPGPU_E_INVALID, "cannot open the files of " + dir);
    auto size_of = [](int fd) -> long long { struct stat sb; return fstat(fd, &sb) == 0 ? (long long)sb.st_size : -1; };
    const long long gen_size = size_of(fg.fd), ovf_size = size_of(fo.fd), hash_size = size_of(fh.fd);
    if (ovf_size != overflow_size * (wide ? 8 : 4)) return fail(nullptr, SNAPGPU_E_INVALID, "OverflowTable size does not match the header");

    std::vector<uint8_t> head;
    size_t pos = 0;
    long long n_bases = 0; int n_contigs = 0, gflags = 0;
    std::vector<uint64_t> contig_begin, proj_begin; std::vector<uint8_t> proj_rc; std::vector<uint32_t> cigar_start, cigar_ops;
    uint64_t first_alt = ~0ull >> 2;
    for (size_t want = 1u << 20;; want *= 4) {
        const size_t n = (long long)want < gen_size ? want : (size_t)gen_size;
        head.resize(n);
        size_t got = 0;
        while (got < n) { const ssize_t r = pread(fg.fd, head.data() + got, n - got, (off_t)got); if (r <= 0) return fail(nullptr, SNAPGPU_E_INVALID, "short read on Genome"); got += (size_t)r; }
        pos = 0;
        bool complete = true;
        auto next_line = [&](std::string &line) -> bool {
            size_t e = pos; while (e < head.size() && head[e] != '\n') e++;
            if (e >= head.size()) return false;
            line.assign((const char *)head.data() + pos, e - pos); pos = e + 1; return true;
        };
        std::string line;
        if (!next_line(line)) { if ((long long)n == gen_size) return fail(nullptr, SNAPGPU_E_INVALID, "malformed Genome header"); continue; }
        if (sscanf(line.c_str(), "%lld %d %d", &n_bases, &n_contigs, &gflags) < 2 || n_contigs < 0) return fail(nullptr, SNAPGPU_E_INVALID, "malformed Genome header");
        contig_begin.assign((size_t)n_contigs, 0); proj_begin.assign((size_t)n_contigs, 0); proj_rc.assign((size_t)n_contigs, 0);
        cigar_start.assign((size_t)n_contigs + 1, 0); cigar_ops.clear(); first_alt = ~0ull >> 2;
        for (int i = 0; i < n_contigs; i++) {
            long long begin = 0, pbegin = 0; int cflags = 0, orig = 0, pflags = 0, name_len = 0, cigar_len = 0, consumed = 0;
            if (!next_line(line)) { complete = false; break; }
// ... 1670 lines not shown
```

Baseline: 14.49 million.

## Place per-wave Aligner object in LDS and drop register directory path

The Aligner state object is now placement-new'ed into a per-wave LDS frame (768 bytes added to the LDS layout) instead of living in registers or scratch. The single-end-help fields move into a templated base that exists only in non-exact kernels. The experimental REGDIR ballot-based directory is removed. The aim is to relieve register pressure and scratch spills by keeping uniform wave state in LDS. The cost is LDS traffic on every field access, and the larger LDS footprint may reduce waves per CU.

After: 15.56 million (median of 6 runs). 7.4% higher.

```diff
diff --git a/snap_amd/csrc/align_single.h b/snap_amd/csrc/align_single.h
--- a/snap_amd/csrc/align_single.h
+++ b/snap_amd/csrc/align_single.h
@@ -108,13 +108,20 @@
     uint64_t adj_off;
 };
 
-struct AlignerDirState { uint32_t dirkey; };
-struct AlignerNoDirState {};
-template <bool REGDIR> struct AlignerDirBase { using type = AlignerNoDirState; };
-template <> struct AlignerDirBase<true> { using type = AlignerDirState; };
-
-template <int AGC, bool SEC = false, bool EXACT = false, bool TIMED = false, bool PLANES = false, bool REGDIR = false>
-struct Aligner : AlignerDirBase<REGDIR>::type {
+struct AlignerHelpState {
+    SEHelpSlot *se_slots; uint32_t se_n_slots; SESpec *se_spec; uint32_t se_spec_cap;
+    uint32_t *se_ctl;
+    uint32_t se_eager;
+    uint32_t *se_items, *se_first;
+    unsigned long long *se_diag;
+    int se_slot; uint32_t se_n, se_tried, cur_read; SESpec *se_mine;
+};
+struct AlignerNoHelpState {};
+template <bool HELP> struct AlignerHelpBase { using type = AlignerNoHelpState; };
+template <> struct AlignerHelpBase<true> { using type = AlignerHelpState; };
+
+template <int AGC, bool SEC = false, bool EXACT = false, bool TIMED = false, bool PLANES = false, bool HELP = false>
+struct Aligner : AlignerHelpBase<HELP>::type {
     const DevIndex ix;
     GP<const DevTables> tab;
     const AlignCfg cfg;
@@ -151,12 +158,6 @@
     uint32_t ag_obj_used0, ag_obj_used1;
     uint32_t max_k;
     uint32_t ag_calls_unit;
-    SEHelpSlot *se_slots; uint32_t se_n_slots; SESpec *se_spec; uint32_t se_spec_cap;
-    uint32_t *se_ctl;
-    uint32_t se_eager;
-    uint32_t *se_items, *se_first;
-    unsigned long long *se_diag;
-    int se_slot; uint32_t se_n, se_tried, cur_read; SESpec *se_mine;
     GP<snapgpu_single_result> agc;
     uint32_t agc_cap, n_agc, agc_overflow;
     SecCfg sec_cfg;
@@ -288,20 +289,9 @@
         k *= 0x9E3779B97F4A7C15ull;
         return (uint32_t)(k >> 40) & (cfg.ht_size - 1);
     }
-    static __device__ __forceinline__ uint32_t dir_key(int64_t base, int dir) { return (uint32_t)(((uint64_t)base / BUCKET) * 2 + (uint64_t)dir); }
-#ifndef SNAPGPU_DIR_CAP
-#define SNAPGPU_DIR_CAP 64
-#endif
-    static constexpr uint32_t DIR_CAP = SNAPGPU_DIR_CAP;
     __device__ __forceinline__ uint16_t find_element(int64_t loc, int dir) const {
         int64_t low = (int64_t)((uint64_t)loc % BUCKET);
         int64_t base = loc - low;
-        if constexpr (REGDIR) {
-            if (n_used <= DIR_CAP) {
-                const unsigned long long m = BALLOT(this->dirkey == dir_key(base, dir));
-                return m ? (uint16_t)__builtin_ctzll(m) : (uint16_t)0xFFFF;
-            }
-        }
         uint16_t h = (uint16_t)first_u32(heads[head_slot(base, dir)]);
         while (h != 0) {
             const uint32_t *ew = (const uint32_t *)&pool[h - 1];
@@ -317,7 +307,6 @@
     __device__ __forceinline__ void clear_candidates() {
         n_used = 0;
         highest_used_weight_list = 0;
-        if constexpr (REGDIR) this->dirkey = 0xFFFFFFFFu;
         for (uint32_t i = lane; i < cfg.num_weight_lists; i += WAVE) {
             wl_next[i] = sent(i); wl_prev[i] = sent(i);
         }
@@ -325,7 +314,6 @@
     }
 
     __device__ __forceinline__ void release_candidates() {
-        if (REGDIR && n_used <= DIR_CAP) return;
         for (uint32_t i = lane; i < n_used; i += WAVE) {
             heads[head_slot(pool[i].base, pool[i].dir)] = 0;
         }
@@ -353,21 +341,7 @@
         n_used++;
         Elem *e = &pool[ei];
         uint32_t hs = head_slot(base, dir);
-        uint16_t old_head = 0;
-        bool hashed = true;
-        if constexpr (REGDIR) {
-            if (ei < DIR_CAP) { this->dirkey = lane == (int)ei ? dir_key(base, dir) : this->dirkey; hashed = false; }
-            else if (ei == DIR_CAP) {
-                for (uint32_t j = 0; j < DIR_CAP; j++) {
-                    uint64_t k = (uint64_t)(uint32_t)__builtin_amdgcn_readlane((int)this->dirkey, (int)j) * 0x9E3779B97F4A7C15ull;
-                    const uint32_t hj = (uint32_t)(k >> 40) & (cfg.ht_size - 1);
-                    const uint16_t oh = (uint16_t)first_u32(heads[hj]);
-                    if (lane == 0) { pool[j].hnext = oh; heads[hj] = (uint16_t)(j + 1); }
-                    WAVE_SYNC();
-                }
-            }
-        }
-        if (hashed) old_head = (uint16_t)first_u32(heads[hs]);
+        uint16_t old_head = (uint16_t)first_u32(heads[hs]);
         if (lane == 0) {
             e->used = 1ull << low;
             e->scored = 0;
@@ -382,7 +356,7 @@
             e->best_loc = 0; e->seed_offset = 0;
             e->cand_seed_offset[low] = (uint16_t)seed_offset;
             e->hnext = old_head;
-            if (hashed) heads[hs] = (uint16_t)(ei + 1);
+            heads[hs] = (uint16_t)(ei + 1);
         }
         WAVE_SYNC();
         list_push_tail(1, ei);
@@ -749,22 +723,22 @@
         return ce;
     }
 
-    __device__ __forceinline__ bool se_wanted() const { return se_eager || XW::ld(se_ctl[1]) != 0u; }
+    __device__ __forceinline__ bool se_wanted() const { return this->se_eager || XW::ld(this->se_ctl[1]) != 0u; }
 
     __device__ __forceinline__ void se_publish(uint32_t wl) {
         int s = -1;
         if (lane == 0) {
-            const uint32_t start = (cur_read * 7u) % se_n_slots;
-            for (uint32_t k = 0; k < se_n_slots; k++) {
-                const uint32_t i = start + k < se_n_slots ? start + k : start + k - se_n_slots;
-                if (XW::ld_lane(se_slots[i].state) != 0u) continue;
-                if (atomicCAS(&se_slots[i].state, 0u, 3u) == 0u) { s = (int)i; break; }
+            const uint32_t start = (this->cur_read * 7u) % this->se_n_slots;
+            for (uint32_t k = 0; k < this->se_n_slots; k++) {
+                const uint32_t i = start + k < this->se_n_slots ? start + k : start + k - this->se_n_slots;
+                if (XW::ld_lane(this->se_slots[i].state) != 0u) continue;
+                if (atomicCAS(&this->se_slots[i].state, 0u, 3u) == 0u) { s = (int)i; break; }
             }
         }
         s = (int)first_u32((uint32_t)s);
-        if (s < 0) { se_tried = 0x80000000u | 32u; return; }
-        se_tried = 1;
-        for (uint32_t i = (uint32_t)lane; i < n_used; i += WAVE) se_first[i] = 0xffffffffu;
+        if (s < 0) { this->se_tried = 0x80000000u | 32u; return; }
+        this->se_tried = 1;
+        for (uint32_t i = (uint32_t)lane; i < n_used; i += WAVE) this->se_first[i] = 0xffffffffu;
         WAVE_SYNC();
         uint32_t n = 0;
         for (uint32_t w = wl; w >= 1 && n + BUCKET <= cfg.se_items_cap; w--) {
@@ -776,42 +750,42 @@
                 const uint64_t scored = ((uint64_t)(uint32_t)__builtin_amdgcn_readlane((int)v, 3) << 32) | (uint32_t)__builtin_amdgcn_readlane((int)v, 2);
                 const uint16_t nxt = (uint16_t)((uint32_t)__builtin_amdgcn_readlane((int)v, 4) & 0xffffu);
                 const uint64_t m = used & ~scored;
-                if (lane == 0) se_first[ei] = n;
-                if (lane < BUCKET && ((m >> lane) & 1ull)) se_items[n + (uint32_t)__popcll(m & ((1ull << lane) - 1ull))] = ((uint32_t)ei << 6) | (uint32_t)lane;
+                if (lane == 0) this->se_first[ei] = n;
+                if (lane < BUCKET && ((m >> lane) & 1ull)) this->se_items[n + (uint32_t)__popcll(m & ((1ull << lane) - 1ull))] = ((uint32_t)ei << 6) | (uint32_t)lane;
                 n += (uint32_t)__popcll(m);
                 ei = nxt;
             }
         }
         WAVE_SYNC();
-        if (n < SE_HELP_MIN_ITEMS || n > se_spec_cap) { if (lane == 0) atomicExch(&se_slots[s].state, 0u); return; }
-        SEHelpSlot *slot = &se_slots[s];
-        SESpec *spec = se_spec + (size_t)s * se_spec_cap;
+        if (n < SE_HELP_MIN_ITEMS || n > this->se_spec_cap) { if (lane == 0) atomicExch(&this->se_slots[s].state, 0u); return; }
+        SEHelpSlot *slot = &this->se_slots[s];
+        SESpec *spec = this->se_spec + (size_t)s * this->se_spec_cap;
         for (uint32_t t = (uint32_t)lane; t < n; t += WAVE) spec[t].state = 0u;
         WAVE_SYNC();
         if (lane == 0) {
             const uint32_t w0 = atomicExch(&slot->next, SE_HELP_LOOKAHEAD), w1 = atomicExch(&slot->helpers, 0u);
             if ((w0 ^ w1) == 0xFFFFFFF5u) atomicExch(&slot->helpers, 0u);
-            XW::st(slot->read, cur_read); XW::st(slot->n, n); XW::st(slot->owner_pos, 0u);
+            XW::st(slot->read, this->cur_read); XW::st(slot->n, n); XW::st(slot->owner_pos, 0u);
             XW::st(slot->lim_alt, (int32_t)score_limit(true)); XW::st(slot->lim_non_alt, (int32_t)score_limit(false));
             XW::st(slot->best_all, (uint32_t)all().best_score);
-            XW::st(*(uint64_t *)&slot->items, (uint64_t)(uintptr_t)se_items); XW::st(*(uint64_t *)&slot->pool, (uint64_t)(uintptr_t)(Elem *)pool);
+            XW::st(*(uint64_t *)&slot->items, (uint64_t)(uintptr_t)this->se_items); XW::st(*(uint64_t *)&slot->pool, (uint64_t)(uintptr_t)(Elem *)pool);
             XW::st(*(uint64_t *)&slot->spec, (uint64_t)(uintptr_t)spec);
             XW::fence_release();
             atomicExch(&slot->state, 1u);
-            atomicAdd(&se_ctl[2], 1u);
-            if (se_diag) atomicAdd(&se_diag[1], 1ull << 32);
-        }
-        WAVE_SYNC();
-        se_slot = s; se_n = n; se_mine = spec;
+            atomicAdd(&this->se_ctl[2], 1u);
+            if (this->se_diag) atomicAdd(&this->se_diag[1], 1ull << 32);
+        }
+        WAVE_SYNC();
+        this->se_slot = s; this->se_n = n; this->se_mine = spec;
     }
 
     __device__ __forceinline__ bool se_take(uint16_t ei, int idx, uint64_t listed0, int limit_e, uint32_t e_lps, int64_t loc0, int cand_seed_offset, CandEval &ce) {
-        const uint32_t t0 = first_u32(se_first[ei]);
+        const uint32_t t0 = first_u32(this->se_first[ei]);
         if (t0 == 0xffffffffu) return false;
         const uint32_t t = t0 + (uint32_t)__popcll(listed0 & ((1ull << idx) - 1ull));
-        if (t >= se_n) return false;
-        SEHelpSlot *slot = &se_slots[se_slot];
-        SESpec *sp = &se_mine[t];
+        if (t >= this->se_n) return false;
+        SEHelpSlot *slot = &this->se_slots[this->se_slot];
+        SESpec *sp = &this->se_mine[t];
         if (lane == 0) XW::st(slot->owner_pos, t + 1u);
         const uint64_t t_w0 = wave_clock();
         for (;;) {
@@ -822,7 +796,7 @@
             if (st == 2u) break;
             XW::nap();
             if (wave_clock() - t_w0 > 1200000000ull) {
-                if (lane == 0 && se_diag) atomicAdd(&se_diag[0], 1ull);
+                if (lane == 0 && this->se_diag) atomicAdd(&this->se_diag[0], 1ull);
                 se_abandon();
                 return false;
             }
@@ -833,18 +807,18 @@
         uint32_t n_ag = XW::ld(sp->n_ag), stale = XW::ld(sp->stale);
         uint64_t bytes = XW::ld(sp->lv_ref_bytes);
         if (lim == limit_e) {
-            if (high && ((e_lps <= best_then) != (e_lps <= (uint32_t)all().best_score))) { if (lane == 0 && se_diag) atomicAdd(&se_diag[-1], 1ull << 16); return false; }
+            if (high && ((e_lps <= best_then) != (e_lps <= (uint32_t)all().best_score))) { if (lane == 0 && this->se_diag) atomicAdd(&this->se_diag[-1], 1ull << 16); return false; }
             ce.sc = XW::ld(sp->sc); ce.mp = XW::ld(sp->mp); ce.loc = XW::ld(sp->loc); ce.used_ag = XW::ld(sp->used_ag);
             ce.clip_before = XW::ld(sp->clip_before); ce.clip_after = XW::ld(sp->clip_after); ce.ag_score = XW::ld(sp->ag_score);
         } else {
-            if (lim < limit_e || n_lv == 0u) { if (lane == 0 && se_diag) atomicAdd(&se_diag[-1], 1ull); return false; }
+            if (lim < limit_e || n_lv == 0u) { if (lane == 0 && this->se_diag) atomicAdd(&this->se_diag[-1], 1ull); return false; }
             const int lv1 = XW::ld(sp->lv1), lv2 = XW::ld(sp->lv2);
             const int plen0 = read_len - (cand_seed_offset + (int)ix.seed_len), plen1 = cand_seed_offset;
             const bool half1_runs = lv1 >= 0 && lv1 <= limit_e;
             bytes = (uint64_t)plen0 + (uint64_t)(2 * (limit_e < 0 ? 0 : limit_e)) + (half1_runs ? (uint64_t)plen1 : 0ull);
             if (half1_runs && lv2 >= 0 && lv1 + lv2 <= limit_e) {
                 if (n_ag != 0u || (high && e_lps <= (uint32_t)all().best_score)) {
-                    if (lane == 0 && se_diag) atomicAdd(&se_diag[-1], 1ull << 16);
+                    if (lane == 0 && this->se_diag) atomicAdd(&this->se_diag[-1], 1ull << 16);
                     return false;
                 }
                 ce.sc = XW::ld(sp->sc); ce.mp = XW::ld(sp->mp); ce.loc = XW::ld(sp->loc); ce.used_ag = 0;
@@ -859,29 +833,29 @@
         cnt().lv += n_lv; cnt().ag += n_ag; cnt().lv_ref_bytes += bytes;
         ag_stale += stale; ag_replay += stale;
         if (n_ag) { ag_obj_used0 = 1; ag_obj_used1 = 1; ag_calls_unit += n_ag; }
-        if (lane == 0 && se_diag) atomicAdd(&se_diag[1], 1ull);
+        if (lane == 0 && this->se_diag) atomicAdd(&this->se_diag[1], 1ull);
         return true;
     }
 
     __device__ __forceinline__ void se_abandon() {
-        if (lane == 0) { atomicExch(&se_slots[se_slot].state, 4u); atomicSub(&se_ctl[2], 1u); }
-        se_slot = -1;
+        if (lane == 0) { atomicExch(&this->se_slots[this->se_slot].state, 4u); atomicSub(&this->se_ctl[2], 1u); }
+        this->se_slot = -1;
     }
 
     __device__ __forceinline__ void se_close() {
-        SEHelpSlot *slot = &se_slots[se_slot];
+        SEHelpSlot *slot = &this->se_slots[this->se_slot];
         uint32_t was = 0;
-        if (lane == 0) { was = atomicExch(&slot->state, 2u); atomicSub(&se_ctl[2], 1u); }
+        if (lane == 0) { was = atomicExch(&slot->state, 2u); atomicSub(&this->se_ctl[2], 1u); }
         was = first_u32(was);
         bool gave_up = was != 1u;
         const uint64_t t0 = wave_clock();
         while (!gave_up) {
             if (XW::aload(&slot->helpers) == 0u) break;
             XW::nap();
-            if (wave_clock() - t0 > 4800000000ull) { if (lane == 0 && se_diag) atomicAdd(&se_diag[0], 1ull << 16); gave_up = true; }
+            if (wave_clock() - t0 > 4800000000ull) { if (lane == 0 && this->se_diag) atomicAdd(&this->se_diag[0], 1ull << 16); gave_up = true; }
         }
         if (lane == 0) atomicExch(&slot->state, gave_up ? 4u : 0u);
-        se_slot = -1;
+        this->se_slot = -1;
     }
 
     __device__ __forceinline__ void se_help_slot(SEHelpSlot *slot) {
@@ -938,7 +912,7 @@
                     XW::st(sp->lv1, (int32_t)ce.lv1); XW::st(sp->lv2, (int32_t)ce.lv2);
                     XW::stores_done();
                     atomicExch(&sp->state, 2u);
-                    if (se_diag) atomicAdd(&se_diag[-1], 1ull << 32);
+                    if (this->se_diag) atomicAdd(&this->se_diag[-1], 1ull << 32);
 #if defined(SNAPGPU_WAVE_EMU)
                     if (getenv("SNAPGPU_DEBUG_SE_HELP")) fprintf(stderr, "HELPED read %u item %u limit %d sc %u n_ag %u\n", XW::ld(slot->read), t, rec_limit, ce.sc, d_ag);
 #endif
@@ -989,10 +963,10 @@
                 return false;
             }
 
-            if constexpr (!EXACT && !HAM) {
-                if (force_result && se_slots != nullptr && se_slot < 0) {
-                    if (se_tried & 0x80000000u) { se_tried = (se_tried & 0x7fffffffu) > 1u ? se_tried - 1u : 0u; }
-                    else if (!se_tried && se_wanted()) se_publish(wl);
+            if constexpr (HELP && !HAM) {
+                if (force_result && this->se_slots != nullptr && this->se_slot < 0) {
+                    if (this->se_tried & 0x80000000u) { this->se_tried = (this->se_tried & 0x7fffffffu) > 1u ? this->se_tried - 1u : 0u; }
+                    else if (!this->se_tried && se_wanted()) se_publish(wl);
                 }
             }
             uint16_t ei = get_next(sent(wl));
@@ -1031,7 +1005,7 @@
                     int cand_seed_offset = (int)((EW(20 + (idx >> 1)) >> (16 * (idx & 1))) & 0xffffu);
                     CandEval ce;
                     bool have = false;
-                    if constexpr (!EXACT && !HAM) { if (se_slot >= 0) have = se_take(ei, idx, listed0, limit_e, e_lps, loc, cand_seed_offset, ce); }
+                    if constexpr (HELP && !HAM) { if (this->se_slot >= 0) have = se_take(ei, idx, listed0, limit_e, e_lps, loc, cand_seed_offset, ce); }
                     if (!have) ce = eval_candidate<HAM>(loc, e_dir, e_lps, cand_seed_offset, limit_e, (uint32_t)all().best_score);
                     const uint32_t sc = ce.sc; const double mp = ce.mp; loc = ce.loc;
                     const int used_ag = ce.used_ag, clip_before = ce.clip_before, clip_after = ce.clip_after, ag_score = ce.ag_score;
@@ -1200,7 +1174,7 @@
         if (!cfg.alt_aware) non_alt().best_score = SNAPGPU_TooBigScoreValue;
         n_seeds_applied[0] = n_seeds_applied[1] = 0;
         popular_seeds_skipped = 0;
-        se_tried = 0;
+        if constexpr (HELP) this->se_tried = 0;
 
         while (true) {
             bool force = false, applied_either = false;
@@ -1259,7 +1233,7 @@
                 if (score<HAM>(force) || force) break;
             }
         }
-        if constexpr (!EXACT && !HAM) { if (se_slot >= 0) se_close(); }
+        if constexpr (HELP && !HAM) { if (this->se_slot >= 0) se_close(); }
         primary().score_prior_to_clipping = primary().score;
         primary().reserved = (ag_stale & 0x3fffffffu) | (ag_replay ? 0x40000000u : 0u);
         release_candidates();
diff --git a/snap_amd/csrc/kernel_common.h b/snap_amd/csrc/kernel_common.h
--- a/snap_amd/csrc/kernel_common.h
+++ b/snap_amd/csrc/kernel_common.h
@@ -50,11 +50,13 @@
 
 static __device__ __forceinline__ uint32_t align_up(uint32_t v, uint32_t a) { return (v + a - 1) & ~(a - 1); }
 
+#define SE_FRAME_BYTES 768u
+
 struct LdsLayout {
-    uint32_t rd0, rd1, ql0, ql1, gw, seed_used, wl_next, wl_prev, lv, ag, shared, rp, tp, lvp, total;
+    uint32_t rd0, rd1, ql0, ql1, gw, seed_used, wl_next, wl_prev, lv, ag, shared, rp, tp, lvp, frame, total;
 };
 
-static __host__ __device__ __forceinline__ LdsLayout lds_layout(uint32_t RL, uint32_t num_weight_lists, uint32_t kmax, uint32_t ag_lds) {
+static __host__ __device__ __forceinline__ LdsLayout lds_layout(uint32_t RL, uint32_t num_weight_lists, uint32_t kmax, uint32_t ag_lds, uint32_t frame_bytes = 0) {
     LdsLayout L; uint32_t o = 0;
     L.rd0 = o; o += RL; L.rd1 = o; o += RL; L.ql0 = o; o += RL; L.ql1 = o; o += RL;
     L.gw = o; o += (RL + 2 * WIN_PAD + 15) & ~15u;
@@ -67,6 +69,7 @@
     L.rp = o; o += (2 * 4 * read_plane_words(RL) * 8 + 15) & ~15u;
     L.tp = o; o += (3 * text_plane_blocks(RL, WIN_PAD) * 8 + 15) & ~15u;
     L.lvp = o; o += (lv_plane_work_words(RL) * 8 + 15) & ~15u;
+    L.frame = o; o += (frame_bytes + 15) & ~15u;
     L.total = o;
     return L;
 }
diff --git a/snap_amd/csrc/paired_dev.h b/snap_amd/csrc/paired_dev.h
--- a/snap_amd/csrc/paired_dev.h
+++ b/snap_amd/csrc/paired_dev.h
@@ -525,8 +525,6 @@
     al.agc_cap = a.single_agc_cap;
     al.cnt() = WaveCounters{0, 0, 0, 0, 0, 0, 0, 0, 0, 0, 0, 0};
     al.ag_calls_unit = 0;
-    al.se_slots = nullptr; al.se_n_slots = 0; al.se_spec = nullptr; al.se_spec_cap = 0; al.se_ctl = nullptr; al.se_eager = 0; al.se_diag = nullptr;
-    al.se_items = nullptr; al.se_first = nullptr; al.se_slot = -1; al.se_n = 0; al.se_tried = 0; al.cur_read = 0; al.se_mine = nullptr;
 
     if constexpr (SEC) {
         al.sec_cfg = a.ssec_cfg;
diff --git a/snap_amd/csrc/single_kernel.h b/snap_amd/csrc/single_kernel.h
--- a/snap_amd/csrc/single_kernel.h
+++ b/snap_amd/csrc/single_kernel.h
@@ -1,4 +1,5 @@
 #pragma once
+#include <new>
 #include "kernel_common.h"
 
 #ifndef SNAPGPU_WAVES_PER_SIMD
@@ -11,15 +12,13 @@
     const int lane = lane_id();
     const int wave_in_block = __builtin_amdgcn_readfirstlane((int)(threadIdx.x >> 6));
     const uint32_t wave_slot = blockIdx.x * (blockDim.x >> 6) + (uint32_t)wave_in_block;
-    const LdsLayout L = lds_layout(a.cfg.RL, a.cfg.num_weight_lists, a.cfg.kmax, a.cfg.ag_lds);
+    const LdsLayout L = lds_layout(a.cfg.RL, a.cfg.num_weight_lists, a.cfg.kmax, a.cfg.ag_lds, SE_FRAME_BYTES);
     uint8_t *my = lds + (size_t)wave_in_block * L.total;
 
     WaveShared *ws = (WaveShared *)(my + L.shared);
-#if !defined(SNAPGPU_REGDIR)
-    Aligner<AGC, SEC, EXACT, TIMED, PLANES> al(a.ix, a.tab, a.cfg, ws);
-#else
-    Aligner<AGC, SEC, EXACT, TIMED, PLANES, true> al(a.ix, a.tab, a.cfg, ws);
-#endif
+    typedef Aligner<AGC, SEC, EXACT, TIMED, PLANES, !EXACT> AL_T;
+    static_assert(sizeof(AL_T) <= SE_FRAME_BYTES, "the wave's frame does not fit SE_FRAME_BYTES");
+    AL_T &al = *new (my + L.frame) AL_T(a.ix, a.tab, a.cfg, ws);
     al.rd[0] = my + L.rd0; al.rd[1] = my + L.rd1;
     al.ql[0] = my + L.ql0; al.ql[1] = my + L.ql1;
     al.gw = my + L.gw;
@@ -50,10 +49,12 @@
     al.cnt() = WaveCounters{0, 0, 0, 0, 0, 0, 0, 0, 0, 0, 0, 0};
     uint64_t n_done = 0;
     const bool se_on = !EXACT && a.se_slots != nullptr && a.cfg.se_items_cap != 0;
-    al.se_slots = se_on ? a.se_slots : nullptr; al.se_n_slots = a.se_n_slots; al.se_spec = a.se_spec; al.se_spec_cap = a.se_spec_cap;
-    al.se_ctl = a.se_ctl; al.se_eager = a.se_eager; al.se_diag = a.counters + 14;
-    al.se_items = (uint32_t *)(sc + a.cfg.se_off); al.se_first = al.se_items + a.cfg.se_items_cap;
-    al.se_slot = -1; al.se_n = 0; al.se_tried = 0; al.cur_read = 0; al.se_mine = nullptr;
+    if constexpr (!EXACT) {
+        al.se_slots = se_on ? a.se_slots : nullptr; al.se_n_slots = a.se_n_slots; al.se_spec = a.se_spec; al.se_spec_cap = a.se_spec_cap;
+        al.se_ctl = a.se_ctl; al.se_eager = a.se_eager; al.se_diag = a.counters + 14;
+        al.se_items = (uint32_t *)(sc + a.cfg.se_off); al.se_first = al.se_items + a.cfg.se_items_cap;
+        al.se_slot = -1; al.se_n = 0; al.se_tried = 0; al.cur_read = 0; al.se_mine = nullptr;
+    }
 
     const uint32_t n_total = a.remap ? first_u32(*a.n_remap) : a.n_reads;
     unsigned long long dbg_worst = 0;
@@ -66,7 +67,7 @@
         if (a.remap) i = first_u32(a.remap[i]);
         else if (a.order) i = first_u32(a.order[i]);
         al.new_read_images();
-        al.cur_read = i;
+        if constexpr (!EXACT) al.cur_read = i;
         uint64_t b = first_u64(a.offsets[i]), e = first_u64(a.offsets[i + 1]);
         if (a.front_clip) {
             b += (uint64_t)first_u32((uint32_t)a.front_clip[i]); e = b + (uint64_t)first_u32((uint32_t)a.data_len[i]);
diff --git a/snap_amd/csrc/snapgpu.hip b/snap_amd/csrc/snapgpu.hip
--- a/snap_amd/csrc/snapgpu.hip
+++ b/snap_amd/csrc/snapgpu.hip
@@ -722,7 +722,7 @@
     c.se_off = ((size_t)c.ht_size * 2 + (size_t)c.pool_size * sizeof(Elem) + ag_bytes + 255) & ~(size_t)255;
     c.scratch_stride = (c.se_off + ((size_t)c.se_items_cap + (c.se_items_cap ? c.pool_size : 0u)) * 4 + 255) & ~(size_t)255;
     c.ag_lds = !c.ag_buffers ? 0u : (ctx->ag_variant == 3 ? ag_lds_bytes_reg(c.RL, 3) : ag_lds_bytes(c.RL));
-    LdsLayout L = lds_layout(c.RL, c.num_weight_lists, c.kmax, c.ag_lds);
+    LdsLayout L = lds_layout(c.RL, c.num_weight_lists, c.kmax, c.ag_lds, SE_FRAME_BYTES);
     c.lds_per_wave = L.total;
 
     int waves_per_cu = ctx->ag_variant == 3 ? 24 : 16;
@@ -731,6 +731,8 @@
     if ((size_t)4 * L.total > 160 * 1024) { snapgpu_destroy(ctx); return fail(nullptr, SNAPGPU_E_UNSUPPORTED, "per-read LDS state exceeds 40 KiB per wave (max_read_len / num_seeds / max_k too large)"); }
     ctx->n_wave_slots = (uint32_t)ctx->num_cus * (uint32_t)waves_per_cu;
     ctx->n_wave_slots = (ctx->n_wave_slots + 3) & ~3u;
+    if (getenv("SNAPGPU_VERBOSE")) fprintf(stderr, "snapgpu: single-end context: AGC %d RL %u weight_lists %u kmax %u ag_lds %u: lds_per_wave %u (%u without the wave's frame), %d waves per CU, %u wave slots\n",
+                                           ctx->ag_variant, c.RL, c.num_weight_lists, c.kmax, c.ag_lds, (unsigned)c.lds_per_wave, (unsigned)L.frame, waves_per_cu, ctx->n_wave_slots);
     size_t scratch_total = (size_t)ctx->n_wave_slots * c.scratch_stride;
     CRCHK(hipMalloc((void **)&ctx->d_scratch, scratch_total), SNAPGPU_E_NOMEM);
     CRCHK(hipMemsetAsync(ctx->d_scratch, 0, scratch_total, ctx->stream), SNAPGPU_E_NODEVICE);
```
